# kshedden/muscato

Hardware: AMD Instinct MI355X
Metric: reads/sec (100 bp, multi-map) at 1/2/4/8 MI355X; confirm-kernel HBM GB/s vs peak (higher is better)
Workload: dtype u32

## Files before the change

### include/muscato_hip.h

```cpp
#ifndef MUSCATO_HIP_H
#define MUSCATO_HIP_H

#include <stdint.h>

#ifdef __cplusplus
extern "C" {
#endif

#define MUSC_ABI_VERSION 3
#define MUSC_MAX_WINDOWS 16

typedef struct musc_ctx musc_ctx;

typedef struct {
  uint32_t read_idx;
  uint32_t gene_idx;
  uint32_t pos;
  uint32_t nmiss;
} musc_hit;

typedef struct {
  int32_t n_windows;
  int32_t windows[MUSC_MAX_WINDOWS];
  int32_t window_width;
  double pmatch;
  int32_t min_dinuc;
  int32_t max_read_length;
  int32_t max_matches;
  int32_t match_mode;
  int32_t mmtol;
  int32_t apply_mmtol;
  int32_t max_mismatch_p1;
  int32_t skip_block_check;
  int32_t n_shards;
  int32_t reserved[2];
} musc_params;

typedef struct {
  uint64_t n_reads;
  uint64_t n_read_windows;
  uint64_t n_candidates;
  uint64_t n_pairs;
  uint64_t n_accepted;
  uint64_t n_hits;
  uint64_t n_overflow_blocks;
  uint64_t confirm_bytes;
  uint32_t confirm_launches;
  uint32_t n_batches;
  float ms_screen;
  float ms_scan;
  uint32_t match_variant;
  float ms_confirm;
  float ms_select;
  float ms_total;
  float ms_index_build;
  float ms_read_prep;
  uint64_t n_descriptors;
  uint32_t index_kind;
  uint32_t match_launches;
  uint64_t n_overflow_entries;
  uint64_t match_bytes;
  uint64_t match_bytes_strict;
  uint64_t index_bytes;
} musc_stats;

int musc_abi_version(void);

int musc_init(int device_ordinal, musc_ctx** out);
void musc_destroy(musc_ctx* ctx);
const char* musc_last_error(musc_ctx* ctx);
int musc_reload_env(musc_ctx* ctx);

int musc_db_load_ascii(musc_ctx* ctx, const char* seqs, const uint64_t* offsets, uint32_t nseq,
                       int on_device);
int musc_db_load_packed(musc_ctx* ctx, const uint8_t* bases2bit, const uint8_t* nmask,
                        const uint64_t* seq_offsets, uint32_t nseq);
int musc_db_build_index(musc_ctx* ctx, int32_t window_width);
int musc_db_build_index_for(musc_ctx* ctx, const musc_params* params, int32_t max_read_len);

int musc_db_set_partition_bases(musc_ctx* ctx, uint64_t max_bases);
int musc_db_partitions(musc_ctx* ctx, uint32_t* first_target, uint32_t cap, uint32_t* n);

int musc_reads_load_ascii(musc_ctx* ctx, const char* seqs, const uint64_t* offsets,
                          uint64_t nreads, int on_device);
int musc_reads_load_packed(musc_ctx* ctx, const uint8_t* bases2bit, const uint8_t* nmask,
                           const uint64_t* read_offsets, uint64_t nreads);
int musc_reads_load_packed32(musc_ctx* ctx, const uint8_t* bases2bit, const uint8_t* nmask,
                             const uint32_t* lengths, uint32_t fixed_len, uint64_t nreads, int async);

int musc_reads_sort_unique(musc_ctx* ctx, const char* seqs, const uint64_t* offsets, uint64_t nreads,
                           int on_device, uint32_t** order, uint32_t** ustart, uint64_t* nunique);

int musc_match_device(musc_ctx* ctx, const musc_params* params, uint64_t* nhits);
int musc_hits_copy(musc_ctx* ctx, musc_hit* dst, uint64_t capacity, int dst_on_device);
int musc_hits_copy_packed(musc_ctx* ctx, uint64_t* dst, uint64_t capacity, int dst_on_device,
                          uint64_t read_base, const int32_t* bits);
int musc_hits_unpack(musc_ctx* ctx, const uint64_t* src, uint64_t n, int on_device, const int32_t* bits,
                     musc_hit* dst);
int musc_hits_copy_compact(musc_ctx* ctx, uint32_t* words, uint64_t words_capacity, uint8_t* counts,
                           uint64_t counts_capacity, int dst_on_device, const int32_t* bits);
int musc_match(musc_ctx* ctx, const musc_params* params, musc_hit** hits, uint64_t* nhits);
void musc_free_hits(musc_hit* hits);

int musc_get_stats(musc_ctx* ctx, musc_stats* out);

#define MUSC_INSTANCE_WORDS 4
#define MUSC_INST_MATCH_T 1u
#define MUSC_INST_MATCH_G 2u
#define MUSC_INST_SCREEN 3u
#define MUSC_INST_SCREEN_T 4u
#define MUSC_INST_CONFIRM 5u
int musc_last_instance(const musc_ctx* ctx, uint32_t* out);
int musc_instances(uint32_t* out, uint32_t capacity, uint32_t* n);

int musc_overflow_probes(musc_ctx* ctx, uint32_t** read_idx, uint32_t** window, uint64_t* n);
void musc_free_u32(uint32_t* p);

int musc_gather(musc_ctx* const* ctxs, int n, const uint64_t* read_base, musc_hit** hits,
                uint64_t* nhits);
int musc_gather_rccl(musc_ctx* const* ctxs, int n, const uint64_t* read_base, musc_hit** hits,
                     uint64_t* nhits);
int musc_rccl_probe(char* msg, uint64_t cap);

#ifdef __cplusplus
}
#endif
#endif
```

### muscato_amd/_lib.py

```python
from __future__ import annotations

import ctypes
import os

HERE = os.path.dirname(os.path.abspath(__file__))
LIB_PATH = os.environ.get("MUSC_LIB_PATH") or os.path.join(HERE, "libmuscato_hip.so")

MUSC_MAX_WINDOWS = 16


class MuscHit(ctypes.Structure):
    _fields_ = [("read_idx", ctypes.c_uint32), ("gene_idx", ctypes.c_uint32),
                ("pos", ctypes.c_uint32), ("nmiss", ctypes.c_uint32)]


class MuscParams(ctypes.Structure):
    _fields_ = [
        ("n_windows", ctypes.c_int32),
        ("windows", ctypes.c_int32 * MUSC_MAX_WINDOWS),
        ("window_width", ctypes.c_int32),
        ("pmatch", ctypes.c_double),
        ("min_dinuc", ctypes.c_int32),
        ("max_read_length", ctypes.c_int32),
        ("max_matches", ctypes.c_int32),
        ("match_mode", ctypes.c_int32),
        ("mmtol", ctypes.c_int32),
        ("apply_mmtol", ctypes.c_int32),
        ("max_mismatch_p1", ctypes.c_int32),
        ("skip_block_check", ctypes.c_int32),
        ("n_shards", ctypes.c_int32),
        ("reserved", ctypes.c_int32 * 2),
    ]


class MuscStats(ctypes.Structure):
    _fields_ = [
        ("n_reads", ctypes.c_uint64), ("n_read_windows", ctypes.c_uint64),
        ("n_candidates", ctypes.c_uint64), ("n_pairs", ctypes.c_uint64), ("n_accepted", ctypes.c_uint64),
        ("n_hits", ctypes.c_uint64), ("n_overflow_blocks", ctypes.c_uint64),
        ("confirm_bytes", ctypes.c_uint64),
        ("confirm_launches", ctypes.c_uint32), ("n_batches", ctypes.c_uint32),
        ("ms_screen", ctypes.c_float), ("ms_scan", ctypes.c_float), ("match_variant", ctypes.c_uint32),
        ("ms_confirm", ctypes.c_float), ("ms_select", ctypes.c_float), ("ms_total", ctypes.c_float),
        ("ms_index_build", ctypes.c_float), ("ms_read_prep", ctypes.c_float),
        ("n_descriptors", ctypes.c_uint64),
        ("index_kind", ctypes.c_uint32), ("match_launches", ctypes.c_uint32),
        ("n_overflow_entries", ctypes.c_uint64), ("match_bytes", ctypes.c_uint64),
        ("match_bytes_strict", ctypes.c_uint64), ("index_bytes", ctypes.c_uint64),
    ]


SYMBOLS = [
    "musc_abi_version", "musc_init", "musc_destroy", "musc_last_error", "musc_reload_env",
    "musc_db_load_ascii", "musc_db_load_packed", "musc_db_build_index", "musc_db_build_index_for",
    "musc_db_set_partition_bases", "musc_db_partitions",
    "musc_reads_load_ascii", "musc_reads_load_packed", "musc_reads_load_packed32", "musc_reads_sort_unique",
    "musc_match_device", "musc_hits_copy", "musc_hits_copy_packed", "musc_hits_copy_compact", "musc_hits_unpack", "musc_match", "musc_free_hits",
    "musc_get_stats", "musc_last_instance", "musc_instances", "musc_gather", "musc_gather_rccl", "musc_rccl_probe", "musc_overflow_probes", "musc_free_u32",
]

_lib = None


def load() -> ctypes.CDLL:
    global _lib
    if _lib is not None:
        return _lib
    if not os.path.exists(LIB_PATH):
        raise ImportError(
            "muscato_amd: %s is missing -- build it with `python -m muscato_amd.build` "
            "(hipcc, gfx950).  There is no CPU fallback." % LIB_PATH)
    import sys
    torch = sys.modules.get("torch")
    if torch is not None:
        try:
            if torch.cuda.is_available():
                torch.cuda.init()
        except Exception:
            pass
    lib = ctypes.CDLL(LIB_PATH)
    for s in SYMBOLS:
        if not hasattr(lib, s):
            raise ImportError("muscato_amd: %s does not export %s" % (LIB_PATH, s))
    vp, u64, i32 = ctypes.c_void_p, ctypes.c_uint64, ctypes.c_int32
    lib.musc_abi_version.restype = ctypes.c_int
    lib.musc_init.argtypes = [ctypes.c_int, ctypes.POINTER(vp)]
    lib.musc_destroy.argtypes = [vp]
    lib.musc_destroy.restype = None
    lib.musc_last_error.argtypes = [vp]
    lib.musc_last_error.restype = ctypes.c_char_p
    lib.musc_reload_env.argtypes = [vp]
    lib.musc_db_load_ascii.argtypes = [vp, vp, vp, ctypes.c_uint32, ctypes.c_int]
    lib.musc_db_load_packed.argtypes = [vp, vp, vp, vp, ctypes.c_uint32]
    lib.musc_db_build_index.argtypes = [vp, i32]
    lib.musc_db_build_index_for.argtypes = [vp, ctypes.POINTER(MuscParams), i32]
    lib.musc_db_set_partition_bases.argtypes = [vp, u64]
    lib.musc_db_partitions.argtypes = [vp, vp, ctypes.c_uint32, ctypes.POINTER(ctypes.c_uint32)]
    lib.musc_reads_load_ascii.argtypes = [vp, vp, vp, u64, ctypes.c_int]
    lib.musc_reads_load_packed.argtypes = [vp, vp, vp, vp, u64]
    lib.musc_reads_load_packed32.argtypes = [vp, vp, vp, vp, ctypes.c_uint32, u64, ctypes.c_int]
    lib.musc_reads_sort_unique.argtypes = [vp, vp, vp, u64, ctypes.c_int, ctypes.POINTER(vp), ctypes.POINTER(vp),
                                           ctypes.POINTER(u64)]
    lib.musc_match_device.argtypes = [vp, ctypes.POINTER(MuscParams), ctypes.POINTER(u64)]
    lib.musc_hits_copy.argtypes = [vp, vp, u64, ctypes.c_int]
    lib.musc_hits_copy_packed.argtypes = [vp, vp, u64, ctypes.c_int, u64, ctypes.POINTER(i32)]
    lib.musc_hits_copy_compact.argtypes = [vp, vp, u64, vp, u64, ctypes.c_int, ctypes.POINTER(i32)]
    lib.musc_hits_unpack.argtypes = [vp, vp, u64, ctypes.c_int, ctypes.POINTER(i32), vp]
    lib.musc_match.argtypes = [vp, ctypes.POINTER(MuscParams), ctypes.POINTER(vp), ctypes.POINTER(u64)]
    lib.musc_free_hits.argtypes = [vp]
    lib.musc_free_hits.restype = None
    lib.musc_get_stats.argtypes = [vp, ctypes.POINTER(MuscStats)]
    lib.musc_last_instance.argtypes = [vp, ctypes.POINTER(ctypes.c_uint32)]
    lib.musc_instances.argtypes = [ctypes.POINTER(ctypes.c_uint32), ctypes.c_uint32, ctypes.POINTER(ctypes.c_uint32)]
    lib.musc_overflow_probes.argtypes = [vp, ctypes.POINTER(vp), ctypes.POINTER(vp), ctypes.POINTER(u64)]
    lib.musc_overflow_probes.restype = ctypes.c_int
    lib.musc_free_u32.argtypes = [vp]
    lib.musc_free_u32.restype = None
    lib.musc_gather.argtypes = [ctypes.POINTER(vp), ctypes.c_int, ctypes.POINTER(u64),
                                ctypes.POINTER(vp), ctypes.POINTER(u64)]
    lib.musc_gather_rccl.argtypes = lib.musc_gather.argtypes
    lib.musc_rccl_probe.argtypes = [ctypes.c_char_p, ctypes.c_uint64]
    for name in ("musc_init", "musc_reload_env", "musc_db_load_ascii", "musc_db_load_packed", "musc_db_build_index", "musc_db_build_index_for", "musc_db_build_index_for",
                 "musc_db_set_partition_bases", "musc_db_partitions",
                 "musc_reads_load_ascii", "musc_reads_load_packed", "musc_reads_load_packed32", "musc_reads_sort_unique", "musc_match_device",
                 "musc_hits_copy", "musc_hits_copy_packed", "musc_hits_copy_compact", "musc_hits_unpack", "musc_match", "musc_get_stats", "musc_last_instance", "musc_instances",
                 "musc_gather", "musc_gather_rccl", "musc_rccl_probe"):
        getattr(lib, name).restype = ctypes.c_int
    _lib = lib
    return lib
```

### muscato_amd/api.py

```python
from __future__ import annotations

import ctypes
import json
from dataclasses import dataclass, field, asdict
from typing import List, Optional, Sequence, Tuple

import numpy as np

from . import _lib


class MuscatoError(RuntimeError):
    pass


@dataclass
class Config:
    ReadFileName: str = ""
    GeneFileName: str = ""
    GeneIdFileName: str = ""
    ResultsFileName: str = ""
    Windows: List[int] = field(default_factory=list)
    WindowWidth: int = 0
    BloomSize: int = 0
    NumHash: int = 0
    PMatch: float = 0.0
    MinDinuc: int = 0
    TempDir: str = ""
    LogDir: str = ""
    MinReadLength: int = 0
    MaxReadLength: int = 0
    MaxMatches: int = 0
    MaxConfirmProcs: int = 0
    MMTol: int = 0
    MatchMode: str = ""
    SortPar: int = 0
    SortTemp: str = ""
    SortMem: str = ""
    NoCleanTemp: bool = False
    CPUProfile: bool = False
    MaxMismatch: int = -1
    DbPartitionBases: int = 0

    @classmethod
    def from_json(cls, text) -> "Config":
        d = json.loads(text) if isinstance(text, (str, bytes)) else dict(text)
        c = cls()
        for k, v in d.items():
            if hasattr(c, k) and v is not None:
                setattr(c, k, v)
        return c

    def to_json(self) -> str:
        return json.dumps(asdict(self))

    def with_defaults(self) -> "Config":
        c = Config(**asdict(self))
        if not c.Windows:
            raise MuscatoError("Windows not provided")
        if c.WindowWidth == 0:
            raise MuscatoError("WindowWidth not provided")
        if c.MaxReadLength == 0:
            raise MuscatoError("MaxReadLength not provided")
        if c.BloomSize == 0:
            c.BloomSize = 4 * 1000 * 1000 * 1000
        if c.NumHash == 0:
            c.NumHash = 20
        if c.PMatch == 0:
            c.PMatch = 1.0
        if c.MaxMatches == 0:
            c.MaxMatches = 1000 * 1000
        if c.MaxConfirmProcs == 0:
            c.MaxConfirmProcs = 3
        if c.MatchMode == "":
            c.MatchMode = "best"
        if c.MatchMode not in ("best", "first"):
            raise MuscatoError("MatchMode must be 'first' or 'best'")
        if c.ResultsFileName == "":
            c.ResultsFileName = "results.txt"
        if c.DbPartitionBases < 0:
            raise MuscatoError("DbPartitionBases must be >= 0")
        return c

    def to_params(self, apply_mmtol: bool, skip_block_check: bool = False, n_shards: int = 1) -> _lib.MuscParams:
        c = self.with_defaults()
        if len(c.Windows) > _lib.MUSC_MAX_WINDOWS:
            raise MuscatoError("at most %d windows are supported" % _lib.MUSC_MAX_WINDOWS)
        p = _lib.MuscParams()
        p.n_windows = len(c.Windows)
        for i, w in enumerate(c.Windows):
            p.windows[i] = int(w)
        p.window_width = int(c.WindowWidth)
        p.pmatch = float(c.PMatch)
        p.min_dinuc = int(c.MinDinuc)
        p.max_read_length = int(c.MaxReadLength)
        p.max_matches = int(c.MaxMatches)
        p.match_mode = 1 if c.MatchMode == "first" else 0
        p.mmtol = int(c.MMTol)
        p.apply_mmtol = 1 if apply_mmtol else 0
        p.max_mismatch_p1 = c.MaxMismatch + 1 if c.MaxMismatch >= 0 else 0
        p.skip_block_check = 1 if skip_block_check else 0
        p.n_shards = max(1, int(n_shards))
        return p


def concat(seqs: Sequence[bytes]) -> Tuple[np.ndarray, np.ndarray]:
    off = np.zeros(len(seqs) + 1, dtype=np.uint64)
    if len(seqs):
        off[1:] = np.cumsum([len(s) for s in seqs], dtype=np.uint64)
    buf = np.frombuffer(b"".join(seqs) + b"\0" * 8, dtype=np.uint8).copy()
    return buf, off


_CODE = np.full(256, 255, dtype=np.uint8)
for _i, _c in enumerate(b"ACGT"):
    _CODE[_c] = _i


def pack_2bit(buf: np.ndarray, nbases: int) -> Tuple[np.ndarray, Optional[np.ndarray]]:
    codes = _CODE[buf[:nbases]]
    isx = codes == 255
    codes = np.where(isx, 0, codes).astype(np.uint8)
    pad = (-nbases) % 4
    c4 = np.concatenate([codes, np.zeros(pad, np.uint8)]).reshape(-1, 4)
    packed = (c4[:, 0] | (c4[:, 1] << 2) | (c4[:, 2] << 4) | (c4[:, 3] << 6)).astype(np.uint8)
    mask = np.packbits(isx, bitorder="little") if isx.any() else None
    return packed, mask


class Engine:

    def __init__(self, device: int = 0):
        self._lib = _lib.load()
        h = ctypes.c_void_p()
        rc = self._lib.musc_init(int(device), ctypes.byref(h))
        if rc != 0:
            raise MuscatoError("musc_init failed: %s" % self._lib.musc_last_error(None).decode())
        self._h = h
        self.device = device
        self.n_targets = 0
        self.n_reads = 0

    def close(self) -> None:
        if getattr(self, "_h", None):
            self._lib.musc_destroy(self._h)
            self._h = None

    def __del__(self):
        try:
            self.close()
        except Exception:
            pass

    def __enter__(self):
        return self

    def __exit__(self, *a):
        self.close()

    def _check(self, rc: int, what: str) -> None:
        if rc != 0:
            raise MuscatoError("%s failed (%d): %s" % (what, rc, self._lib.musc_last_error(self._h).decode()))

    def reload_env(self) -> None:
        self._check(self._lib.musc_reload_env(self._h), "musc_reload_env")

    def load_targets(self, seqs: Sequence[bytes]) -> None:
        buf, off = concat(seqs)
        self.load_targets_arrays(buf, off)

    def load_targets_arrays(self, buf: np.ndarray, off: np.ndarray) -> None:
        self._check(self._lib.musc_db_load_ascii(self._h, buf.ctypes.data, off.ctypes.data, len(off) - 1, 0),
                    "musc_db_load_ascii")
        self.n_targets = len(off) - 1

    def load_targets_device(self, seqs_ptr: int, off_ptr: int, nseq: int) -> None:
        self._check(self._lib.musc_db_load_ascii(self._h, seqs_ptr, off_ptr, nseq, 1), "musc_db_load_ascii")
        self.n_targets = nseq

    def load_targets_packed(self, seqs: Sequence[bytes]) -> None:
        buf, off = concat(seqs)
        packed, mask = pack_2bit(buf, int(off[-1]))
        packed = np.concatenate([packed, np.zeros(8, np.uint8)])
        mp = mask.ctypes.data if mask is not None else None
        self._check(self._lib.musc_db_load_packed(self._h, packed.ctypes.data, mp, off.ctypes.data, len(off) - 1),
                    "musc_db_load_packed")
        self.n_targets = len(off) - 1

    def build_index(self, window_width: int) -> None:
        self._check(self._lib.musc_db_build_index(self._h, int(window_width)), "musc_db_build_index")

    def build_index_for(self, cfg: "Config", max_read_len: int = 0) -> None:
        p = cfg.to_params(True)
        self._apply_partition_bases(cfg)
        self._check(self._lib.musc_db_build_index_for(self._h, ctypes.byref(p), int(max_read_len)),
                    "musc_db_build_index_for")

    def set_partition_bases(self, max_bases: int) -> None:
        if max_bases < 0:
            raise MuscatoError("partition bases must be >= 0")
        self._check(self._lib.musc_db_set_partition_bases(self._h, int(max_bases)), "musc_db_set_partition_bases")

    def partitions(self) -> List[int]:
        n = ctypes.c_uint32()
        self._check(self._lib.musc_db_partitions(self._h, None, 0, ctypes.byref(n)), "musc_db_partitions")
        if not n.value:
            return []
        out = (ctypes.c_uint32 * (n.value + 1))()
        self._check(self._lib.musc_db_partitions(self._h, out, n.value + 1, ctypes.byref(n)), "musc_db_partitions")
        return list(out)

    def _apply_partition_bases(self, cfg: "Config") -> None:
        if cfg.DbPartitionBases:
            self.set_partition_bases(int(cfg.DbPartitionBases))

    def load_reads(self, seqs: Sequence[bytes]) -> None:
        buf, off = concat(seqs)
        self.load_reads_arrays(buf, off)

    def load_reads_arrays(self, buf: np.ndarray, off: np.ndarray) -> None:
        self._check(self._lib.musc_reads_load_ascii(self._h, buf.ctypes.data, off.ctypes.data, len(off) - 1, 0),
                    "musc_reads_load_ascii")
        self.n_reads = len(off) - 1

    def load_reads_device(self, seqs_ptr: int, off_ptr: int, nreads: int) -> None:
        self._check(self._lib.musc_reads_load_ascii(self._h, seqs_ptr, off_ptr, nreads, 1), "musc_reads_load_ascii")
        self.n_reads = nreads

    def sort_unique_reads(self, seqs: Sequence[bytes]):
        buf, off = concat(seqs)
        return self.sort_unique_reads_arrays(buf.ctypes.data, off.ctypes.data, len(off) - 1, False)

    def sort_unique_reads_arrays(self, seqs_ptr: int, off_ptr: int, nreads: int, on_device: bool):
        po, pu, nu = ctypes.c_void_p(), ctypes.c_void_p(), ctypes.c_uint64()
        self._check(self._lib.musc_reads_sort_unique(self._h, seqs_ptr, off_ptr, nreads, 1 if on_device else 0,
                                                     ctypes.byref(po), ctypes.byref(pu), ctypes.byref(nu)),
                    "musc_reads_sort_unique")
        try:
            order = np.ctypeslib.as_array(ctypes.cast(po, ctypes.POINTER(ctypes.c_uint32)), shape=(max(nreads, 1),))[:nreads].copy()
            ustart = np.ctypeslib.as_array(ctypes.cast(pu, ctypes.POINTER(ctypes.c_uint32)), shape=(nu.value + 1,)).copy()
        finally:
            self._lib.musc_free_u32(po)
            self._lib.musc_free_u32(pu)
        self.n_reads = int(nu.value)
        return order, ustart

    def load_reads_packed(self, seqs: Sequence[bytes]) -> None:
        buf, off = concat(seqs)
        packed, mask = pack_2bit(buf, int(off[-1]))
        packed = np.concatenate([packed, np.zeros(8, np.uint8)])
        mp = mask.ctypes.data if mask is not None else None
        self._check(self._lib.musc_reads_load_packed(self._h, packed.ctypes.data, mp, off.ctypes.data, len(off) - 1),
                    "musc_reads_load_packed")
        self.n_reads = len(off) - 1

    def load_reads_packed_ptr(self, bases_ptr: int, mask_ptr: int, off_ptr: int, nreads: int) -> None:
        self._check(self._lib.musc_reads_load_packed(self._h, bases_ptr, mask_ptr or None, off_ptr, nreads),
                    "musc_reads_load_packed")
        self.n_reads = nreads

    def load_reads_packed32_ptr(self, bases_ptr: int, mask_ptr: int, lengths_ptr: int, fixed_len: int, nreads: int,
                                async_upload: bool = False) -> None:
        self._check(self._lib.musc_reads_load_packed32(self._h, bases_ptr, mask_ptr or None, lengths_ptr or None,
                                                       fixed_len, nreads, 1 if async_upload else 0),
                    "musc_reads_load_packed32")
        self.n_reads = nreads

    def match_device(self, cfg: Config, apply_mmtol: bool = True, skip_block_check: bool = False,
                     n_shards: int = 1) -> int:
        p = cfg.to_params(apply_mmtol, skip_block_check, n_shards)
        self._apply_partition_bases(cfg)
        n = ctypes.c_uint64()
        self._check(self._lib.musc_match_device(self._h, ctypes.byref(p), ctypes.byref(n)), "musc_match_device")
        return int(n.value)

    def hits_to(self, ptr: int, capacity: int, on_device: bool) -> None:
        self._check(self._lib.musc_hits_copy(self._h, ptr, capacity, 1 if on_device else 0), "musc_hits_copy")

    def hits_to_packed(self, ptr: int, capacity: int, on_device: bool, bits: Sequence[int], read_base: int = 0) -> None:
        b = (ctypes.c_int32 * 4)(*bits)
        self._check(self._lib.musc_hits_copy_packed(self._h, ptr, capacity, 1 if on_device else 0, read_base, b),
                    "musc_hits_copy_packed")

    def hits_to_compact(self, words_ptr: int, words_cap: int, counts_ptr: int, counts_cap: int, on_device: bool,
                        bits: Sequence[int]) -> None:
        b = (ctypes.c_int32 * 3)(*bits)
        self._check(self._lib.musc_hits_copy_compact(self._h, words_ptr, words_cap, counts_ptr, counts_cap,
                                                     1 if on_device else 0, b), "musc_hits_copy_compact")

    def unpack_hits(self, src_ptr: int, n: int, on_device: bool, bits: Sequence[int], dst_ptr: int) -> None:
        b = (ctypes.c_int32 * 4)(*bits)
        self._check(self._lib.musc_hits_unpack(self._h, src_ptr, n, 1 if on_device else 0, b, dst_ptr), "musc_hits_unpack")

    def match(self, cfg: Config, apply_mmtol: bool = True, n_shards: int = 1) -> np.ndarray:
        n = self.match_device(cfg, apply_mmtol, n_shards=n_shards)
        out = np.zeros((n, 4), dtype=np.uint32)
        if n:
            self.hits_to(out.ctypes.data, n, False)
        return out

    def overflow_probes(self) -> np.ndarray:
        pr, pw, n = ctypes.c_void_p(), ctypes.c_void_p(), ctypes.c_uint64()
        self._check(self._lib.musc_overflow_probes(self._h, ctypes.byref(pr), ctypes.byref(pw), ctypes.byref(n)),
                    "musc_overflow_probes")
        out = np.zeros((n.value, 2), dtype=np.uint32)
        if n.value:
            out[:, 0] = np.ctypeslib.as_array(ctypes.cast(pr, ctypes.POINTER(ctypes.c_uint32)), shape=(n.value,))
            out[:, 1] = np.ctypeslib.as_array(ctypes.cast(pw, ctypes.POINTER(ctypes.c_uint32)), shape=(n.value,))
        self._lib.musc_free_u32(pr)
        self._lib.musc_free_u32(pw)
        return out

    def last_instance(self) -> dict:
        w = (ctypes.c_uint32 * 4)()
        self._check(self._lib.musc_last_instance(self._h, w), "musc_last_instance")
        return {"path": "fused" if w[0] else "two-kernel" if w[1] else "none",
                "match": decode_instance(w[0]), "screen": decode_instance(w[1]), "confirm": decode_instance(w[2]),
                "block_mode": w[3] & 0xFF, "exact_rerun": bool(w[3] & 0x100)}

    def stats(self) -> dict:
        s = _lib.MuscStats()
        self._check(self._lib.musc_get_stats(self._h, ctypes.byref(s)), "musc_get_stats")
        return {k: getattr(s, k) for k, _ in s._fields_}


_INST_FIELDS = {1: ("k_match_t", ("W", "XM", "WIDE", "SG")), 2: ("k_match_g", (None, None, None, "SG")),
                3: ("k_screen", ("mask", "one", "lines")), 4: ("k_screen_t", ()), 5: ("k_confirm", ("mask", "w2"))}


def decode_instance(word: int) -> Optional[dict]:
    if not word:
        return None
    name, fields = _INST_FIELDS[word & 0xFF]
    d = {"kernel": name, "RW": (word >> 8) & 0xFF}
    for i, f in enumerate(fields):
        if f:
            d[f] = (word >> (16 + 4 * i)) & 0xF
    return d


def instance_name(d: Optional[dict]) -> str:
    return "none" if d is None else "%s<%s>" % (d["kernel"], ", ".join(str(v) for k, v in d.items() if k != "kernel"))


def instances() -> List[dict]:
    lib = _lib.load()
    n = ctypes.c_uint32()
    if lib.musc_instances(None, 0, ctypes.byref(n)):
        raise RuntimeError("musc_instances failed")
    buf = (ctypes.c_uint32 * max(1, n.value))()
    lib.musc_instances(buf, n.value, ctypes.byref(n))
    return [decode_instance(w) for w in buf[:n.value]]


def gather(engines: Sequence["Engine"], read_bases: Sequence[int], rccl: bool = False) -> np.ndarray:
    lib = engines[0]._lib
    n = len(engines)
    arr = (ctypes.c_void_p * n)(*[e._h for e in engines])
    bases = (ctypes.c_uint64 * n)(*[int(b) for b in read_bases])
    ph, cnt = ctypes.c_void_p(), ctypes.c_uint64()
    rc = lib.musc_gather_rccl(arr, n, bases, ctypes.byref(ph), ctypes.byref(cnt)) if rccl else 1
    if rccl and rc == 2:
        raise MuscatoError("musc_gather_rccl failed (%d): %s" % (rc, lib.musc_last_error(engines[0]._h).decode()))
    if rc != 0:
        rc = lib.musc_gather(arr, n, bases, ctypes.byref(ph), ctypes.byref(cnt))
    if rc != 0:
        raise MuscatoError("musc_gather failed (%d): %s" % (rc, lib.musc_last_error(engines[0]._h).decode()))
    out = np.zeros((cnt.value, 4), dtype=np.uint32)
    if cnt.value:
        ctypes.memmove(out.ctypes.data, ph, cnt.value * 16)
    lib.musc_free_hits(ph)
    return out


def sorted_hits(a: np.ndarray) -> np.ndarray:
    if len(a) == 0:
        return a.reshape(0, 4)
    idx = np.lexsort((a[:, 3], a[:, 2], a[:, 1], a[:, 0]))
    return a[idx]
```

### muscato_amd/csrc/kernels_confirm.hpp

```cpp
#pragma once

template <int RW, bool MASK>
struct PairRegs {
  uint4 ds;
  uint32_t exact;
  uint32_t r[RW ? RW : 1], t[RW ? RW : 1], rm[(RW && MASK) ? RW : 1], tm[(RW && MASK) ? RW : 1];
};

template <int RW, bool MASK>
DEV void pair_issue(PairRegs<RW, MASK>& P, const uint4 ds, const uint32_t* __restrict__ rd,
                    const uint32_t* __restrict__ rdm, const uint32_t* __restrict__ db2,
                    const uint32_t* __restrict__ dbm2, const uint32_t* __restrict__ dbx, uint64_t r0,
                    const uint32_t* __restrict__ rvalid) {
  static_assert(RW != 0, "static stride only");
  P.ds = ds;
  const uint32_t ri = ds.x & 0xFFFFFFu;
  const uint64_t gpos = (uint64_t)ds.y | ((uint64_t)(ds.x >> 24) << 32);
  const uint32_t* __restrict__ rec = rd + (r0 + ri) * (uint64_t)RW;
  const uint64_t widx = gpos >> 4;
  P.exact = rvalid[ri];
  bool rx = false, tx = false;
  if constexpr (MASK) {
    rx = (ds.z & DESC_RX) != 0;
    tx = db_span_has_x(dbx, gpos, RW * 16);
  }
#pragma unroll
  for (int q = 0; q < RW / 4; q++) {
    const u32x4_v a = __builtin_nontemporal_load(reinterpret_cast<const u32x4_v*>(rec) + q);
    P.r[4 * q] = a.x; P.r[4 * q + 1] = a.y; P.r[4 * q + 2] = a.z; P.r[4 * q + 3] = a.w;
    const u32x4_u b = *reinterpret_cast<const u32x4_u*>(db2 + widx + 4 * q);
    P.t[4 * q] = b.x; P.t[4 * q + 1] = b.y; P.t[4 * q + 2] = b.z; P.t[4 * q + 3] = b.w;
    if constexpr (MASK) {
      uint4 c = make_uint4(0, 0, 0, 0);
      if (rx) c = *reinterpret_cast<const uint4*>(rdm + (r0 + ri) * (uint64_t)RW + 4 * q);
      P.rm[4 * q] = c.x; P.rm[4 * q + 1] = c.y; P.rm[4 * q + 2] = c.z; P.rm[4 * q + 3] = c.w;
      u32x4_u d = {0, 0, 0, 0};
      if (tx) d = *reinterpret_cast<const u32x4_u*>(dbm2 + widx + 4 * q);
      P.tm[4 * q] = d.x; P.tm[4 * q + 1] = d.y; P.tm[4 * q + 2] = d.z; P.tm[4 * q + 3] = d.w;
    }
  }
}

DEV uint32_t pair_code(const uint4 ds, uint32_t nx, uint32_t budget, uint32_t exact) {
  const uint32_t ri = ds.x & 0xFFFFFFu, k = ds.z & 15u;
  const bool within = nx <= budget;
  const bool a0 = within && ((exact >> k) & 1u);
  const bool a1 = within && (ds.z & DESC_TWO) && ((exact >> (k + 1)) & 1u);
  if (!(a0 || a1)) return NX_REJECT;
  const uint32_t kmin = (uint32_t)(__ffs(exact) - 1);
  const bool first = (a0 && kmin == k) || (a1 && kmin == k + 1);
  return (first ? nx : (nx | NX_DUP)) | (a0 ? NX_ACC0 : 0u) | (a1 ? NX_ACC1 : 0u) | (k << 20) | ((ri & (TILE - 1)) << 24);
}

template <int RW, bool MASK, bool W2, class BudgetOf>
DEV uint32_t pair_finish(const PairRegs<RW, MASK>& P, const PathParams& pp, BudgetOf budget_of) {
  const uint64_t gpos = (uint64_t)P.ds.y | ((uint64_t)(P.ds.x >> 24) << 32);
  const uint32_t sh = ((uint32_t)gpos & 15u) * 2u;
  uint32_t exact = P.exact;
  if ((P.ds.z >> 4) & 1u) exact &= ~pp.q1zero_mask;
  const uint32_t len = P.r[RW - 1] & 0xFFFFu;
  const int len2 = 2 * (int)len;
  uint32_t nx = 0;
#pragma unroll
  for (int j = 0; j < RW - 1; j++) {
    const uint32_t tj = __funnelshift_r(P.t[j], P.t[j + 1], sh);
    const uint32_t x = P.r[j] ^ tj;
    uint32_t d = (x | (x >> 1)) & 0x55555555u;
    if constexpr (MASK) d |= (P.rm[j] ^ __funnelshift_r(P.tm[j], P.tm[j + 1], sh)) & 0x55555555u;
    const int rem = len2 - 32 * j;
    d &= rem >= 32 ? 0xFFFFFFFFu : (rem <= 0 ? 0u : ((1u << rem) - 1u));
    nx += __popc(d);
    if constexpr (W2) {
#pragma unroll
      for (int kk = 0; kk < 2; kk++)
        if (kk < pp.W && (d & window_word_mask(pp.win[kk], pp.ww, j))) exact &= ~(1u << kk);
    } else {
      for (int kk = 0; kk < pp.W; kk++)
        if (d & window_word_mask(pp.win[kk], pp.ww, j)) exact &= ~(1u << kk);
    }
  }
  return pair_code(P.ds, nx, budget_of(len), exact);
}

template <int RW, bool MASK, bool W2, class BudgetOf>
DEV uint32_t confirm_pair(const uint4 ds, const uint32_t* __restrict__ rd, const uint32_t* __restrict__ rdm,
                          const uint32_t* __restrict__ db2, const uint32_t* __restrict__ dbm2,
                          const uint32_t* __restrict__ dbx, uint64_t r0, int rw_rt, const PathParams& pp,
                          BudgetOf budget_of, const uint32_t* __restrict__ rvalid) {
  if constexpr (RW != 0) {
    PairRegs<RW, MASK> P;
    pair_issue<RW, MASK>(P, ds, rd, rdm, db2, dbm2, dbx, r0, rvalid);
    return pair_finish<RW, MASK, W2>(P, pp, budget_of);
  } else {
    const uint32_t ri = ds.x & 0xFFFFFFu;
    const int rw = rw_rt;
    const uint64_t gpos = (uint64_t)ds.y | ((uint64_t)(ds.x >> 24) << 32);
    const uint32_t* __restrict__ rec = rd + (r0 + ri) * (uint64_t)rw;
    const uint64_t widx = gpos >> 4;
    const uint32_t sh = ((uint32_t)gpos & 15u) * 2u;
    uint32_t exact = rvalid[ri];
    if ((ds.z >> 4) & 1u) exact &= ~pp.q1zero_mask;
    uint32_t nx = 0;
    const uint32_t len = rec[rw - 1] & 0xFFFFu;
    const int len2 = 2 * (int)len;
    const uint32_t* __restrict__ recm = MASK ? rdm + (r0 + ri) * (uint64_t)rw : nullptr;
    uint32_t tlo = db2[widx], tmlo = MASK ? dbm2[widx] : 0u;
    for (int j = 0; j < rw - 1; j++) {
      const uint32_t thi = db2[widx + j + 1];
      const uint32_t x = rec[j] ^ __funnelshift_r(tlo, thi, sh);
      tlo = thi;
      uint32_t d = (x | (x >> 1)) & 0x55555555u;
      if (MASK) {
        const uint32_t tmhi = dbm2[widx + j + 1];
        d |= (recm[j] ^ __funnelshift_r(tmlo, tmhi, sh)) & 0x55555555u;
        tmlo = tmhi;
      }
      const int rem = len2 - 32 * j;
      d &= rem >= 32 ? 0xFFFFFFFFu : (rem <= 0 ? 0u : ((1u << rem) - 1u));
      nx += __popc(d);
      for (int kk = 0; kk < pp.W; kk++)
        if (d & window_word_mask(pp.win[kk], pp.ww, j)) exact &= ~(1u << kk);
    }
    return pair_code(ds, nx, budget_of(len), exact);
  }
}

#define BLOCK_LDS_BITS 11
#define CONF_TILES 32


#define CODE_CAP 1024

template <int RW, bool MASK, bool W2>
__global__ __launch_bounds__(TILE, (RW <= 8 && !(RW == 8 && MASK)) ? 8 : 4) void k_confirm(
    const uint32_t* __restrict__ rd, const uint32_t* __restrict__ rdm,
    const uint32_t* __restrict__ db2, const uint32_t* __restrict__ dbm2, const uint32_t* __restrict__ dbx,
    uint64_t r0, uint32_t n, int rw_rt,
    const PathParams* __restrict__ ppp, const uint16_t* __restrict__ nmiss_tab, const uint4* __restrict__ cdesc,
    const uint32_t* __restrict__ rvalid, uint32_t* __restrict__ p_nx,
    const uint32_t* __restrict__ tbase, const uint32_t* __restrict__ tcount,
    const uint32_t* __restrict__ wb, int block_mode, uint32_t block_thr, uint32_t* __restrict__ block_table,
    const uint64_t* __restrict__ seq_off, uint4* __restrict__ stage, uint32_t* __restrict__ tcount2,
    unsigned long long* __restrict__ counters) {
  const PathParams& pp = *ppp;
  extern __shared__ uint32_t s_wcnt[];
  __shared__ uint32_t s_best[TILE], s_cnt[TILE], s_base[TILE];
  __shared__ uint32_t s_code[CODE_CAP];
  __shared__ uint32_t s_sketch[1 << BLOCK_LDS_BITS];
  __shared__ uint32_t s_wsum[TILE / 64];
  __shared__ uint16_t s_nm[CONF_NM];
  __shared__ uint32_t s_tb[CONF_TILES], s_tn[CONF_TILES];
  const uint32_t ntiles = (n + TILE - 1) / TILE;
  const int lane = threadIdx.x & 63, wid = threadIdx.x >> 6;
  if (block_mode == 1)
    for (uint32_t t = threadIdx.x; t < (1u << BLOCK_LDS_BITS); t += TILE) s_sketch[t] = 0;
  for (uint32_t t = threadIdx.x; t < CONF_NM; t += TILE) s_nm[t] = t <= (uint32_t)pp.max_len ? nmiss_tab[t] : (uint16_t)0;
  const uint32_t my_tiles = blockIdx.x < ntiles ? (ntiles - 1 - blockIdx.x) / gridDim.x + 1 : 0;
  for (uint32_t j = threadIdx.x; j < my_tiles && j < CONF_TILES; j += TILE) {
    s_tb[j] = tbase[blockIdx.x + j * gridDim.x];
    s_tn[j] = tcount[blockIdx.x + j * gridDim.x];
  }
  if (blockIdx.x == 0 && threadIdx.x == 0) tcount2[ntiles] = 0;
  unsigned long long acc = 0;
  auto budget_of = [&](uint32_t len) -> uint32_t { return len < CONF_NM ? s_nm[len] : nmiss_tab[len]; };
  __syncthreads();

  for (uint32_t j = 0; j < my_tiles; j++) {
    const uint32_t tile = blockIdx.x + j * gridDim.x;
    lds_barrier();
    s_best[threadIdx.x] = 0xFFFFFFFFu;
    s_cnt[threadIdx.x] = 0;
    if (block_mode)
      for (uint32_t t = threadIdx.x; t < TILE * (uint32_t)pp.W; t += TILE) s_wcnt[t] = 0;
    lds_barrier();
    const uint32_t tn = s_tn[j];
    const uint64_t tb = s_tb[j];
    auto tally = [&](uint32_t w) {
      if (w == NX_REJECT) return;
      const uint32_t rl = w >> 24;
      if (block_mode) {
        const uint32_t k = (w >> 20) & 15u;
        if (w & NX_ACC0) atomicAdd(&s_wcnt[rl * pp.W + k], 1u);
        if (w & NX_ACC1) atomicAdd(&s_wcnt[rl * pp.W + k + 1], 1u);
      }
      if (w & NX_DUP) return;
      atomicMin(&s_best[rl], w & 0xFFFFu);
      acc++;
    };
    auto confirm_at = [&](uint32_t tj, uint32_t* gene, uint32_t* zword) -> uint32_t {
      const u32x4_v dsv = __builtin_nontemporal_load(reinterpret_cast<const u32x4_v*>(cdesc) + tb + tj);
      *gene = dsv.w;
      *zword = dsv.z;
      return confirm_pair<RW, MASK, W2>(make_uint4(dsv.x, dsv.y, dsv.z, dsv.w), rd, rdm, db2, dbm2, dbx, r0, rw_rt, pp,
                                    budget_of, rvalid);
    };
    uint32_t w0 = NX_REJECT, gene0 = 0, z0 = 0;
    if (threadIdx.x < tn) w0 = confirm_at(threadIdx.x, &gene0, &z0);
    tally(w0);
    for (uint32_t tj = threadIdx.x + TILE; tj < tn; tj += TILE) {
      uint32_t g, z;
      const uint32_t w = confirm_at(tj, &g, &z);
      if (tj - TILE < CODE_CAP) s_code[tj - TILE] = w; else p_nx[tb + tj] = w;
      tally(w);
    }
    lds_barrier();
    auto count = [&](uint32_t w) {
      if (w == NX_REJECT || (w & NX_DUP)) return;
      const uint32_t rl = w >> 24;
      const uint32_t thr = pp.apply_mmtol ? s_best[rl] + (uint32_t)pp.mmtol : 0xFFFFu;
      if ((w & 0xFFFFu) <= thr) atomicAdd(&s_cnt[rl], 1u);
    };
    count(w0);
    for (uint32_t tj = threadIdx.x + TILE; tj < tn; tj += TILE)
      count(tj - TILE < CODE_CAP ? s_code[tj - TILE] : p_nx[tb + tj]);
    if (block_mode) {
      for (uint32_t t = threadIdx.x; t < TILE * (uint32_t)pp.W; t += TILE) {
        const uint32_t cw = s_wcnt[t];
        if (!cw) continue;
        const uint32_t rl = t / pp.W, k = t % pp.W;
        const uint32_t h = block_hash32((uint32_t)k, wb[((uint64_t)tile * TILE + rl) * pp.W + k]);
        if (block_mode == 1) atomicAdd(&s_sketch[h >> (32 - BLOCK_LDS_BITS)], cw);
        else atomicAdd(&block_table[h >> (32 - BLOCK_TABLE_BITS)], cw);
      }
    }
    lds_barrier();
    const uint32_t c = s_cnt[threadIdx.x];
    uint32_t inc = c;
#pragma unroll
    for (int d = 1; d < 64; d <<= 1) {
      const uint32_t o = __shfl_up(inc, d);
      if (lane >= d) inc += o;
    }
    if (lane == 63) s_wsum[wid] = inc;
    lds_barrier();
    uint32_t woff = 0, total = 0;
#pragma unroll
    for (int q = 0; q < TILE / 64; q++) {
      if (q < wid) woff += s_wsum[q];
      total += s_wsum[q];
    }
    s_base[threadIdx.x] = woff + inc - c;
    s_cnt[threadIdx.x] = 0;
    if (threadIdx.x == 0) tcount2[tile] = total;
    lds_barrier();
    if (total == 0) continue;
    auto emit = [&](uint32_t w, uint32_t tj, uint32_t gene, uint32_t zword) {
      if (w == NX_REJECT || (w & NX_DUP)) return;
      const uint32_t rl = w >> 24, v = w & 0xFFFFu;
      const uint32_t thr = pp.apply_mmtol ? s_best[rl] + (uint32_t)pp.mmtol : 0xFFFFu;
      if (v > thr) return;
      const uint32_t ord = atomicAdd(&s_cnt[rl], 1u);
      uint32_t pos = (zword >> 6) & 0xFFFFu;
      if (!((zword >> 5) & 1u)) {
        const uint4 ds = cdesc[tb + tj];
        pos = (uint32_t)(((uint64_t)ds.y | ((uint64_t)(ds.x >> 24) << 32)) - seq_off[gene]);
      }
      stage[tb + s_base[rl] + ord] = make_uint4((uint32_t)(r0 + tile * TILE + rl), gene, pos, v);
    };
    emit(w0, threadIdx.x, gene0, z0);
    for (uint32_t tj = threadIdx.x + TILE; tj < tn; tj += TILE) {
      const uint32_t w = tj - TILE < CODE_CAP ? s_code[tj - TILE] : p_nx[tb + tj];
      if (w == NX_REJECT || (w & NX_DUP)) continue;
      const uint4 ds = cdesc[tb + tj];
      emit(w, tj, ds.w, ds.z);
    }
  }
  block_add_u64(acc, &counters[1]);
  if (block_mode == 1) {
    lds_barrier();
    uint32_t hot = 0;
    for (uint32_t t = threadIdx.x; t < (1u << BLOCK_LDS_BITS); t += TILE) hot |= s_sketch[t] >= block_thr;
    if (__any(hot) && (threadIdx.x & 63) == 0) atomicOr(&counters[6], 1ull);
  }
}

MUSC_KERNEL __launch_bounds__(256) void k_compact(uint32_t ntiles, const uint32_t* __restrict__ tbase,
                                                 const uint32_t* __restrict__ tcount2,
                                                 const uint32_t* __restrict__ tpre,
                                                 const uint4* __restrict__ stage, uint4* __restrict__ hits,
                                                 uint64_t hits_cap, unsigned long long* __restrict__ counters) {
  const unsigned long long base = counters[2];
  if (base + tpre[ntiles] > hits_cap) {
    if (blockIdx.x == 0 && threadIdx.x == 0) atomicOr(&counters[3], 2ull);
    return;
  }
  for (uint32_t tile = blockIdx.x; tile < ntiles; tile += gridDim.x) {
    const uint32_t m = tcount2[tile];
    const uint4* __restrict__ src = stage + tbase[tile];
    uint4* __restrict__ dst = hits + base + tpre[tile];
    for (uint32_t j = threadIdx.x; j < m; j += blockDim.x) dst[j] = src[j];
  }
}

template <int RW>
__global__ __launch_bounds__(256) void k_hot_probes(const uint32_t* __restrict__ rd,
                                                    const uint32_t* __restrict__ rdm, uint64_t nreads,
                                                    int rw_rt, const PathParams* __restrict__ ppp,
                                                    const uint32_t* __restrict__ block_table,
                                                    uint32_t max_matches, uint2* __restrict__ out,
                                                    uint64_t cap, unsigned long long* __restrict__ cursor) {
  const PathParams& pp = *ppp;
  const int rw = RW ? RW : rw_rt;
  const bool has_m = rdm != nullptr;
  for (uint64_t i = (uint64_t)blockIdx.x * blockDim.x + threadIdx.x; i < nreads; i += (uint64_t)gridDim.x * blockDim.x) {
    Rec<RW> rec;
    rec.load(rd + i * (uint64_t)rw, rw);
    Rec<RW> recm = rec;
    if (has_m) recm.load(rdm + i * (uint64_t)rw, rw);
    const uint32_t len = rec.len();
    for (int k = 0; k < pp.W; k++) {
      const uint32_t q1 = (uint32_t)pp.win[k], q2 = q1 + (uint32_t)pp.ww;
      if (len < q2) continue;
      if (pp.min_dinuc > 0 && rec_count_dinuc(rec, recm, has_m, q1, pp.ww) < pp.min_dinuc) continue;
      const uint32_t b = rec_bucket(rec, recm, has_m, q1, pp.ww, pp.bits, pp.direct);
      const uint32_t h = block_hash32((uint32_t)k, b);
      if (block_table[h >> (32 - BLOCK_TABLE_BITS)] > max_matches) {
        const unsigned long long slot = atomicAdd(cursor, 1ull);
        if (slot < cap) out[slot] = make_uint2((uint32_t)i, (uint32_t)k);
      }
    }
  }
}

MUSC_KERNEL void k_advance(const uint32_t* __restrict__ tpre, uint32_t ntiles, unsigned long long* counters) {
  if (threadIdx.x == 0 && blockIdx.x == 0) counters[2] += tpre[ntiles];
}

MUSC_KERNEL void k_block_overflow(const uint32_t* __restrict__ block_table, uint32_t max_matches,
                                 unsigned long long* __restrict__ counters) {
  unsigned long long c = 0;
  for (uint32_t i = blockIdx.x * blockDim.x + threadIdx.x; i < (1u << BLOCK_TABLE_BITS); i += gridDim.x * blockDim.x)
    c += block_table[i] > max_matches;
  block_add_u64(c, &counters[5]);
}

struct PackBits {
  int32_t read, gene, pos, nmiss;
};

MUSC_KERNEL __launch_bounds__(256) void k_pack_hits(const uint4* __restrict__ hits, uint64_t n, uint64_t read_base,
                                                   PackBits b, uint64_t* __restrict__ out, uint32_t* __restrict__ bad) {
  for (uint64_t i = (uint64_t)blockIdx.x * blockDim.x + threadIdx.x; i < n; i += (uint64_t)gridDim.x * blockDim.x) {
    const uint4 h = hits[i];
    const uint64_t r = (uint64_t)h.x + read_base;
    if ((b.read < 64 && (r >> b.read)) || ((uint64_t)h.y >> b.gene) || ((uint64_t)h.z >> b.pos) || ((uint64_t)h.w >> b.nmiss))
      atomicOr(bad, 1u);
    out[i] = (((((r << b.gene) | h.y) << b.pos) | h.z) << b.nmiss) | h.w;
  }
}

MUSC_KERNEL __launch_bounds__(256) void k_unpack_hits(const uint64_t* __restrict__ in, uint64_t n, PackBits b,
                                                     uint4* __restrict__ hits) {
  for (uint64_t i = (uint64_t)blockIdx.x * blockDim.x + threadIdx.x; i < n; i += (uint64_t)gridDim.x * blockDim.x) {
    uint64_t v = in[i];
    const uint32_t nm = (uint32_t)(v & ((1ull << b.nmiss) - 1ull));
    v >>= b.nmiss;
    const uint32_t pos = (uint32_t)(v & ((1ull << b.pos) - 1ull));
    v >>= b.pos;
    const uint32_t gene = (uint32_t)(v & ((1ull << b.gene) - 1ull));
    v >>= b.gene;
    hits[i] = make_uint4((uint32_t)v, gene, pos, nm);
  }
}

MUSC_KERNEL __launch_bounds__(256) void k_pack_compact(const uint4* __restrict__ hits, uint64_t n, PackBits b,
                                                      uint32_t* __restrict__ words, uint8_t* __restrict__ counts,
                                                      uint32_t* __restrict__ bad) {
  for (uint64_t i = (uint64_t)blockIdx.x * blockDim.x + threadIdx.x; i < n; i += (uint64_t)gridDim.x * blockDim.x) {
    const uint4 h = hits[i];
    if (((uint64_t)h.y >> b.gene) || ((uint64_t)h.z >> b.pos) || ((uint64_t)h.w >> b.nmiss)) atomicOr(bad, 1u);
    words[i] = (((h.y << b.pos) | h.z) << b.nmiss) | h.w;
    const uint32_t prev = i ? hits[i - 1].x : 0xFFFFFFFFu;
    if (i && prev > h.x) atomicOr(bad, 4u);
    if (i == 0 || prev != h.x) {
      uint32_t cnt = 1;
      while (i + cnt < n && cnt < 256 && hits[i + cnt].x == h.x) cnt++;
      if (cnt > 255) atomicOr(bad, 2u);
      counts[h.x] = (uint8_t)cnt;
    }
  }
}
```

### muscato_amd/csrc/muscato_hip.hip

```cpp

#include <hip/hip_runtime.h>
#include <rccl/rccl.h>
#include <dlfcn.h>

#include <algorithm>
#include <cstdarg>
#include <cstdio>
#include <cstdlib>
#include <cstring>
#include <map>
#include <mutex>
#include <string>
#include <type_traits>
#include <vector>

#include "../../include/muscato_hip.h"

#include "kernels_common.hpp"
#include "kernels_index.hpp"
#include "kernels_screen.hpp"
#include "kernels_confirm.hpp"
#include "kernels_match.hpp"
#include "kernels_match_lane_inst.hpp"
#include "kernels_screen_lane.hpp"
#include "kernels_partition.hpp"
MUSC_LANE_INSTANCES_4(extern)
MUSC_LANE_INSTANCES_8(extern)
MUSC_LANE_INSTANCES_12(extern)
MUSC_LANE_INSTANCES_8W(extern)
MUSC_LANE_INSTANCES_12W(extern)
MUSC_LANE_INSTANCES_16W(extern)
MUSC_LANE_INSTANCES_SPEC(extern)
MUSC_DMA_INSTANCES(extern)


namespace {

thread_local std::string g_init_error;

template <class T>
struct DevBuf {
  T* p = nullptr;
  uint64_t cap = 0;
  void release() {
    if (p) (void)hipFree(p);
    p = nullptr;
    cap = 0;
  }
};

struct Roctx {
  int (*push)(const char*) = nullptr;
  int (*pop)() = nullptr;
  Roctx() {
    for (const char* name : {"librocprofiler-sdk-roctx.so.1", "librocprofiler-sdk-roctx.so", "libroctx64.so.4", "libroctx64.so"}) {
      if (void* h = dlopen(name, RTLD_NOW | RTLD_LOCAL)) {
        push = reinterpret_cast<int (*)(const char*)>(dlsym(h, "roctxRangePushA"));
        pop = reinterpret_cast<int (*)()>(dlsym(h, "roctxRangePop"));
        if (push && pop) return;
        push = nullptr;
        pop = nullptr;
      }
    }
  }
};
const Roctx& roctx() {
  static const Roctx r;
  return r;
}
struct Range {
  bool on;
  explicit Range(const char* name) : on(roctx().push != nullptr) {
    if (on) (void)roctx().push(name);
  }
  ~Range() {
    if (on) (void)roctx().pop();
  }
};

struct CaptureGuard {
  hipStream_t st = nullptr;
  bool active = false;
  hipError_t begin(hipStream_t s) {
    const hipError_t e = hipStreamBeginCapture(s, hipStreamCaptureModeThreadLocal);
    if (e == hipSuccess) {
      st = s;
      active = true;
    }
    return e;
  }
  hipError_t end(hipGraph_t* g) {
    active = false;
    return hipStreamEndCapture(st, g);
  }
  ~CaptureGuard() {
    if (!active) return;
    hipGraph_t g = nullptr;
    (void)hipStreamEndCapture(st, &g);
    if (g) (void)hipGraphDestroy(g);
    (void)hipGetLastError();
  }
};

struct TmpBufs {
  void* p[16] = {};
  int n = 0;
  template <class T>
  hipError_t alloc(T** out, size_t bytes) {
    void* q = nullptr;
    *out = nullptr;
    if (n >= 16) return hipErrorOutOfMemory;
    const hipError_t e = hipMalloc(&q, bytes ? bytes : 16);
    if (e == hipSuccess) p[n++] = q;
    *out = (T*)q;
    return e;
  }
  void release() {
    for (int i = 0; i < n; i++) (void)hipFree(p[i]);
    n = 0;
  }
  ~TmpBufs() { release(); }
};

}

struct EnvKnobs {
  enum { IDX_AUTO = 0, IDX_CLASSIC, IDX_LINES, IDX_CLASSIC64 };
  int index = IDX_AUTO;
  bool match_dma = false;
  bool screen_wg = false;
  int context = 0;
  bool no_x_context = false;
  bool force_wide = false;
  int index_bits = 0;
  bool ctx_direct = false;
  int debug_grid = 0;
  bool debug_sync = false;
  int graph = -1;
  bool pipeline = false;
  bool no_spec = false;
  long batch_reads = 0;
  long index_budget_mb = 0;
  void read() {
    *this = EnvKnobs();
    auto is = [](const char* v, const char* w) { return v && !strcmp(v, w); };
    const char* e = getenv("MUSC_INDEX");
    index = is(e, "classic") ? IDX_CLASSIC : is(e, "lines") ? IDX_LINES : is(e, "classic64") ? IDX_CLASSIC64 : IDX_AUTO;
    e = getenv("MUSC_MATCH");
    match_dma = is(e, "dma");
    screen_wg = is(getenv("MUSC_SCREEN"), "wg");
    e = getenv("MUSC_CONTEXT");
    context = is(e, "narrow") ? 1 : is(e, "wide") ? 2 : 0;
    no_x_context = getenv("MUSC_NO_X_CONTEXT") != nullptr;
    force_wide = getenv("MUSC_DEBUG_FORCE_WIDE") != nullptr;
    if ((e = getenv("MUSC_DEBUG_INDEX_BITS"))) index_bits = atoi(e);
    ctx_direct = (e = getenv("MUSC_DEBUG_CTX_DIRECT")) && atoi(e) > 0;
    if ((e = getenv("MUSC_DEBUG_GRID"))) debug_grid = atoi(e);
    debug_sync = getenv("MUSC_DEBUG_SYNC") != nullptr;
    if ((e = getenv("MUSC_GRAPH"))) graph = atoi(e);
    if ((e = getenv("MUSC_PIPELINE"))) pipeline = atoi(e) > 0;
    no_spec = getenv("MUSC_NO_SPEC") != nullptr;
    if ((e = getenv("MUSC_BATCH_READS"))) batch_reads = atol(e);
    if ((e = getenv("MUSC_DEBUG_INDEX_BUDGET_MB"))) index_budget_mb = atol(e);
  }
};

struct musc_ctx {
  int device = 0;
  hipStream_t stream = nullptr;
  std::string err;
  EnvKnobs env;

  uint32_t* db2 = nullptr;
  uint32_t* dbm2 = nullptr;
  bool db_has_x = false;
  bool reads_have_x = false;
  DevBuf<uint32_t> rdx;
  uint64_t rdx_epoch = ~0ull;
  int rdx_wide = -1;
  uint64_t xok_epoch = ~0ull;
  double xok_pmatch = -1.0;
  int32_t xok_mmp1 = -1;
  bool xok = false;
  uint32_t* dbx = nullptr;
  uint64_t max_tlen = 0;
  uint64_t xokdb_epoch = ~0ull;
  int32_t xokdb_key[CTX_MAX_W + 3] = {0};
  bool xokdb = false;
  uint64_t* seq_off = nullptr;
  uint32_t nseq = 0;
  uint64_t nbases = 0;
  uint64_t db_words = 0;
  std::vector<uint64_t> h_seq_off;

  uint64_t part_bases = 0;
  std::vector<uint32_t> part_first;
  int part_kind = 0;
  uint64_t part_size = 0;
  uint32_t cur_part = 0;
  DevBuf<musc_hit> pacc;
  DevBuf<uint32_t> pbest;
  DevBuf<uint64_t> pcnt, padj;
  DevBuf<uint32_t> pflags, pflags_tmp;
  DevBuf<uint32_t> block_acc;

  int idx_ww = 0, idx_bits = 0, idx_direct = 0;
  uint32_t idx_g0 = 0, idx_g1 = 0;
  int wide = 0;
  Bucket* idx_T = nullptr;
  uint4* idx_E = nullptr;
  bool idx_lines = false;
  unsigned scrt_resident = 0;
  int scrt_rw = 0;
  uint64_t idx_T_bytes = 0, idx_E_cap = 0;
  uint64_t idx_n = 0;
  uint64_t idx_novf = 0;
  int idx_kind = 0;
  int idx_wide = 0;
  int idx_CL = 0;
  CtxBucket* ctx_T = nullptr;
  CtxEntry* ctx_E = nullptr;
  uint64_t ctx_T_cap = 0, ctx_E_cap = 0;
  PathParams* d_pp = nullptr;
  PathParams h_pp;
  bool h_pp_valid = false;
  MatchParams* d_mp = nullptr;
  MatchParams h_mp;
  bool h_mp_valid = false;
  int spec_geom = 0;
  DevBuf<uint4> spill;

  uint32_t* rd = nullptr;
  uint32_t* rdm = nullptr;
  uint64_t nreads = 0;
  int rw = 0;
  uint32_t max_len = 0;

  struct Upload {
    uint32_t* stage = nullptr;
    uint64_t stage_words = 0;
    hipStream_t s_up = nullptr;
    std::vector<hipEvent_t> ev;
    uint64_t piece = 0, n_pieces = 0;
    uint64_t packed_upto = 0;
    uint32_t L = 0;
    bool active = false;
  } up;

  struct BatchSet {
    DevBuf<uint32_t> wb, rvalid, tbase, tcount;
    DevBuf<uint4> cdesc;
  } bs[2];
  int cur = 0;
  hipStream_t stream2 = nullptr;
  hipStream_t s_confirm = nullptr;
  hipEvent_t ev_ready[2] = {nullptr, nullptr}, ev_free[2] = {nullptr, nullptr}, ev_join = nullptr;
  DevBuf<uint32_t> scan_tmp, tcount2, tpre;
  DevBuf<uint4> stage;
  DevBuf<uint32_t> p_nx;
  DevBuf<uint16_t> nmiss_tab;
  DevBuf<uint32_t> block_table;
  bool force_exact_blocks = false;
  uint64_t exact_epoch = 0;
  musc_params exact_params;
  int cur_block_mode = 0;
  uint32_t cur_block_thr = 0;
  PathParams last_pp;
  uint32_t last_max_matches = 0;
  uint32_t last_inst[MUSC_INSTANCE_WORDS] = {0, 0, 0, 0};
  bool last_exact_blocks = false;
  unsigned long long* counters = nullptr;
  uint64_t* h_pinned = nullptr;

  DevBuf<musc_hit> hits;
  uint64_t nhits = 0;
  DevBuf<uint64_t> packed;
  DevBuf<musc_hit> gathered;
  uint32_t* d_flag = nullptr;

  uint32_t batch_reads = 16u << 20;
  uint64_t data_epoch = 1;
  uint64_t sized_epoch = 0;
  musc_params sized_params;
  bool sized_exact_blocks = false;
  uint32_t sized_bsz = 0;
  musc_stats stats;
  hipGraphExec_t graph_exec = nullptr;
  bool graph_failed = false;
  uint64_t graph_epoch = 0;
  musc_params graph_params;
  int graph_block_mode = -1;
  uint32_t graph_batches = 0;
  std::vector<hipEvent_t> ev_pool;
  size_t ev_used = 0;
  double nm_pmatch = -1.0;
  int32_t nm_mmp1 = -1;
  uint32_t nm_maxlen = 0xFFFFFFFFu;
};

namespace {

int fail(musc_ctx* c, int code, const char* fmt, ...) {
  char buf[512];
  va_list ap;
  va_start(ap, fmt);
  vsnprintf(buf, sizeof buf, fmt, ap);
  va_end(ap);
  if (c) c->err = buf; else g_init_error = buf;
  return code;
}

#define HIPCHK(c, expr)                                                                 \
  do {                                                                                  \
    hipError_t e_ = (expr);                                                             \
    if (e_ != hipSuccess) {                                                             \
      (void)hipGetLastError();                                                          \
      return fail((c), 10, "%s failed: %s (%s:%d)", #expr, hipGetErrorString(e_), __FILE__, __LINE__); \
    }                                                                                   \
  } while (0)

template <class T>
int ensure(musc_ctx* c, DevBuf<T>& b, uint64_t n, bool keep = false) {
  if (n <= b.cap && b.p) return 0;
  uint64_t ncap = std::max<uint64_t>(n, b.cap + b.cap / 2);
  ncap = std::max<uint64_t>(ncap, 1024);
  T* np = nullptr;
  HIPCHK(c, hipMalloc((void**)&np, ncap * sizeof(T) + 64));
  if (keep && b.p && b.cap) {
    hipError_t e = hipMemcpyAsync(np, b.p, b.cap * sizeof(T), hipMemcpyDeviceToDevice, c->stream);
    if (e == hipSuccess) e = hipStreamSynchronize(c->stream);
    if (e != hipSuccess) {
      (void)hipFree(np);
      return fail(c, 10, "hit buffer grow failed: %s", hipGetErrorString(e));
    }
  }
  b.release();
  b.p = np;
  b.cap = ncap;
  return 0;
}

inline unsigned nblk(uint64_t n, unsigned b) { return (unsigned)((n + b - 1) / b); }

uint64_t scan_tmp_elems(uint64_t n) {
  uint64_t t = 0;
  while (n > SCAN_TILE) {
    n = (n + SCAN_TILE - 1) / SCAN_TILE;
    t += (n + 8 + 3) & ~3ull;
  }
  return t + 8;
}

int scan_u32(musc_ctx* c, const uint32_t* in, uint32_t* out, uint64_t n, bool inclusive, uint32_t* tmp,
             hipStream_t st = nullptr) {
  if (!st) st = c->stream;
  const uint64_t nb = (n + SCAN_TILE - 1) / SCAN_TILE;
  if (nb > 0x7FFFFFFFull) return fail(c, 11, "scan too large");
  if (nb <= 1) {
    if (inclusive) hipLaunchKernelGGL(k_scan_block<true>, dim3(1), dim3(SCAN_BLOCK), 0, st, in, out, (uint32_t*)nullptr, n);
    else hipLaunchKernelGGL(k_scan_block<false>, dim3(1), dim3(SCAN_BLOCK), 0, st, in, out, (uint32_t*)nullptr, n);
    HIPCHK(c, hipGetLastError());
    return 0;
  }
  uint32_t* sums = tmp;
  if (inclusive) hipLaunchKernelGGL(k_scan_block<true>, dim3((unsigned)nb), dim3(SCAN_BLOCK), 0, st, in, out, sums, n);
  else hipLaunchKernelGGL(k_scan_block<false>, dim3((unsigned)nb), dim3(SCAN_BLOCK), 0, st, in, out, sums, n);
  HIPCHK(c, hipGetLastError());
  int rc = scan_u32(c, sums, sums, nb, false, tmp + ((nb + 8 + 3) & ~3ull), st);
  if (rc) return rc;
  hipLaunchKernelGGL(k_scan_add, dim3((unsigned)nb), dim3(SCAN_BLOCK), 0, st, out, sums, n);
  HIPCHK(c, hipGetLastError());
  return 0;
}

int scan_u64(musc_ctx* c, const uint64_t* in, uint64_t* out, uint64_t n, uint64_t* tmp) {
  const uint64_t nb = (n + SCAN_TILE - 1) / SCAN_TILE;
  if (nb > 0x7FFFFFFFull) return fail(c, 11, "scan too large");
  if (nb <= 1) {
    hipLaunchKernelGGL(k_scan64_block, dim3(1), dim3(SCAN_BLOCK), 0, c->stream, in, out, (uint64_t*)nullptr, n);
    HIPCHK(c, hipGetLastError());
    return 0;
  }
  hipLaunchKernelGGL(k_scan64_block, dim3((unsigned)nb), dim3(SCAN_BLOCK), 0, c->stream, in, out, tmp, n);
  HIPCHK(c, hipGetLastError());
  int rc = scan_u64(c, tmp, tmp, nb, tmp + ((nb + 8 + 3) & ~3ull));
  if (rc) return rc;
  hipLaunchKernelGGL(k_scan64_add, dim3((unsigned)nb), dim3(SCAN_BLOCK), 0, c->stream, out, tmp, n);
  HIPCHK(c, hipGetLastError());
  return 0;
}

void free_index(musc_ctx* c) {
  c->idx_ww = 0;
  c->idx_n = 0;
  c->data_epoch++;
}

void drop_ctx_index(musc_ctx* c) {
  if (c->ctx_T) (void)hipFree(c->ctx_T);
  if (c->ctx_E) (void)hipFree(c->ctx_E);
  c->ctx_T = nullptr;
  c->ctx_E = nullptr;
  c->ctx_T_cap = c->ctx_E_cap = 0;
}

void free_db(musc_ctx* c) {
  free_index(c);
  if (c->db2) (void)hipFree(c->db2);
  if (c->dbm2) (void)hipFree(c->dbm2);
  if (c->dbx) (void)hipFree(c->dbx);
  if (c->seq_off) (void)hipFree(c->seq_off);
  c->db2 = c->dbm2 = c->dbx = nullptr;
  c->db_has_x = false;
  c->seq_off = nullptr;
  c->nseq = 0;
  c->nbases = 0;
  c->h_seq_off.clear();
  c->part_first.clear();
  c->data_epoch++;
}

void free_reads(musc_ctx* c) {
  if (c->up.active) {
    (void)hipStreamSynchronize(c->up.s_up);
    c->up.active = false;
  }
  if (c->rd) (void)hipFree(c->rd);
  if (c->rdm) (void)hipFree(c->rdm);
  c->rd = c->rdm = nullptr;
  c->reads_have_x = false;
  c->nreads = 0;
  c->rw = 0;
  c->data_epoch++;
}

struct EvPair {
  hipEvent_t a, b;
};

hipEvent_t pool_event(musc_ctx* c) {
  if (c->ev_used == c->ev_pool.size()) {
    hipEvent_t e = nullptr;
    if (hipEventCreate(&e) != hipSuccess) return nullptr;
    c->ev_pool.push_back(e);
  }
  return c->ev_pool[c->ev_used++];
}

struct Timer {
  musc_ctx* c;
  bool off = false;
  std::vector<EvPair> ev[5];
  explicit Timer(musc_ctx* ctx) : c(ctx) { c->ev_used = 0; }
  int begin(int fam, hipStream_t s = nullptr) {
    if (off) return 0;
    EvPair p;
    p.a = pool_event(c);
    p.b = pool_event(c);
    if (!p.a || !p.b) return 1;
    (void)hipEventRecord(p.a, s ? s : c->stream);
    ev[fam].push_back(p);
    return 0;
  }
  void end(int fam, hipStream_t s = nullptr) {
    if (!off && !ev[fam].empty()) (void)hipEventRecord(ev[fam].back().b, s ? s : c->stream);
  }
  float total(int fam) {
    float t = 0;
    for (auto& p : ev[fam]) {
      float ms = 0;
      if (hipEventElapsedTime(&ms, p.a, p.b) == hipSuccess) t += ms;
    }
    return t;
  }
};

int check_params(musc_ctx* c, const musc_params* P) {
  if (!P) return fail(c, 2, "params is NULL");
  if (P->n_windows < 1 || P->n_windows > MUSC_MAX_WINDOWS)
    return fail(c, 2, "n_windows=%d outside 1..%d", P->n_windows, MUSC_MAX_WINDOWS);
  if (P->window_width < 1 || P->window_width > 4096) return fail(c, 2, "bad window_width=%d", P->window_width);
  for (int k = 0; k < P->n_windows; k++)
    if (P->windows[k] < 0 || P->windows[k] > 60000) return fail(c, 2, "bad window start %d", P->windows[k]);
  if (!(P->pmatch >= 0.0 && P->pmatch <= 1.0)) return fail(c, 2, "PMatch=%g outside [0,1]", P->pmatch);
  if (P->match_mode != 0 && P->match_mode != 1) return fail(c, 2, "match_mode must be 0 (best) or 1 (first)");
  if (P->mmtol < 0) return fail(c, 2, "MMTol < 0");
  if (P->max_mismatch_p1 < 0) return fail(c, 2, "max_mismatch_p1 < 0");
  return 0;
}

bool screen_lane(const musc_ctx* c, bool mask) {
  return c->idx_lines && !mask && !c->rdm && (c->rw == 4 || c->rw == 8 || c->rw == 12 || c->rw == 16) && !c->env.screen_wg;
}

template <class F>
auto by_rw(int rw, F&& f) {
  switch (rw) {
    case 4: return f(std::integral_constant<int, 4>{});
    case 8: return f(std::integral_constant<int, 8>{});
    case 12: return f(std::integral_constant<int, 12>{});
    case 16: return f(std::integral_constant<int, 16>{});
    default: return f(std::integral_constant<int, 0>{});
  }
}

typedef decltype(&k_screen_t<8>) screen_t_fn;
typedef decltype(&k_screen<0, false, false, false>) screen_fn;
typedef decltype(&k_confirm<0, false, false>) confirm_fn;
template <class Fn>
struct Inst {
  Fn fn;
  uint32_t id;
};
constexpr uint32_t inst_id(uint32_t family, int rw, int a = 0, int b = 0, int c = 0, int d = 0) {
  return family | (uint32_t)rw << 8 | (uint32_t)a << 16 | (uint32_t)b << 20 | (uint32_t)c << 24 | (uint32_t)d << 28;
}
#define INST_SCREEN_T(RW) Inst<screen_t_fn>{k_screen_t<RW>, inst_id(MUSC_INST_SCREEN_T, RW)}
#define INST_SCREEN(RW, M, ONE, LN) Inst<screen_fn>{k_screen<RW, M, ONE, LN>, inst_id(MUSC_INST_SCREEN, RW, M, ONE, LN)}
#define INST_CONFIRM(RW, M, W2) Inst<confirm_fn>{k_confirm<RW, M, W2>, inst_id(MUSC_INST_CONFIRM, RW, M, W2)}

Inst<screen_t_fn> screen_t_instance(int rw) {
  return by_rw(rw, [](auto r) -> Inst<screen_t_fn> {
    if constexpr (decltype(r)::value != 0) return INST_SCREEN_T(decltype(r)::value);
    else return Inst<screen_t_fn>{nullptr, 0};
  });
}

Inst<screen_fn> screen_instance(int rw, bool mask, int W, bool lines) {
  const int m = mask, one = W <= 2, ln = lines;
  return by_rw(rw, [&](auto r) -> Inst<screen_fn> {
    constexpr int RW = decltype(r)::value;
    static const Inst<screen_fn> k[2][2][2] = {
        {{INST_SCREEN(RW, false, false, false), INST_SCREEN(RW, false, false, true)}, {INST_SCREEN(RW, false, true, false), INST_SCREEN(RW, false, true, true)}},
        {{INST_SCREEN(RW, true, false, false), INST_SCREEN(RW, true, false, true)}, {INST_SCREEN(RW, true, true, false), INST_SCREEN(RW, true, true, true)}}};
    return k[m][one][ln];
  });
}

Inst<confirm_fn> confirm_instance(int rw, bool mask, int W) {
  const int m = mask, w2 = W <= 2;
  return by_rw(rw, [&](auto r) -> Inst<confirm_fn> {
    constexpr int RW = decltype(r)::value;
    static const Inst<confirm_fn> k[2][2] = {{INST_CONFIRM(RW, false, false), INST_CONFIRM(RW, false, true)}, {INST_CONFIRM(RW, true, false), INST_CONFIRM(RW, true, true)}};
    return k[m][w2];
  });
}

Inst<screen_t_fn> screen_t_kernel(const musc_ctx* c) { return screen_t_instance(c->rw); }
Inst<screen_fn> screen_kernel(const musc_ctx* c, int W) { return screen_instance(c->rw, c->rdm != nullptr, W, c->idx_lines); }
Inst<confirm_fn> confirm_kernel(const musc_ctx* c, bool mask, int W) { return confirm_instance(c->rw, mask, W); }

unsigned screen_grid(musc_ctx* c, uint32_t n, bool mask) {
  unsigned g = std::min(nblk(n, TILE), MAX_GRID);
  if (screen_lane(c, mask)) {
    if (!c->scrt_resident) {
      int per_cu = 0, ncu = 0;
      const void* fn = reinterpret_cast<const void*>(screen_t_kernel(c).fn);
      if (hipOccupancyMaxActiveBlocksPerMultiprocessor(&per_cu, fn, 64, 0) != hipSuccess || per_cu < 1) { (void)hipGetLastError(); per_cu = 8; }
      if (hipDeviceGetAttribute(&ncu, hipDeviceAttributeMultiprocessorCount, c->device) != hipSuccess || ncu < 1) ncu = 256;
      c->scrt_resident = (unsigned)per_cu * (unsigned)ncu;
      c->scrt_rw = c->rw;
    }
    if (c->scrt_rw != c->rw) { c->scrt_resident = 0; return screen_grid(c, n, mask); }
    g = std::min(g, std::min(c->scrt_resident, MAX_GRID));
  }
  return g;
}

void launch_screen(musc_ctx* c, bool mask, uint64_t r0, uint32_t n, const PathParams& pp) {
  const dim3 sgrid(screen_grid(c, n, mask));
  auto& b = c->bs[c->cur];
  if (screen_lane(c, mask)) {
    const auto k = screen_t_kernel(c);
    c->last_inst[1] = k.id;
    hipLaunchKernelGGL(k.fn, sgrid, dim3(64), 0, c->stream, c->rd, r0, n, c->d_pp, c->nmiss_tab.p,
                       reinterpret_cast<const LineBucket*>(c->idx_T), c->idx_E, b.cdesc.p, b.cdesc.cap, b.rvalid.p, b.wb.p,
                       b.tbase.p, b.tcount.p, c->counters + 8, c->counters + 3);
  } else {
    const auto k = screen_kernel(c, pp.W);
    c->last_inst[1] = k.id;
    hipLaunchKernelGGL(k.fn, sgrid, dim3(TILE), 0, c->stream, c->rd, c->rdm, r0, n, c->rw, c->d_pp,
                       c->nmiss_tab.p, c->idx_T, c->idx_E, b.cdesc.p, b.cdesc.cap, b.rvalid.p, b.wb.p, b.tbase.p, b.tcount.p,
                       c->counters + 8, c->counters + 3);
  }
}

void launch_confirm(musc_ctx* c, bool mask, uint64_t r0, uint32_t n, const PathParams& pp) {
  const dim3 grid(std::min(nblk(n, TILE), MAX_GRID));
  static_assert((1u << 24) / TILE / MAX_GRID <= CONF_TILES, "a k_confirm workgroup keeps its tile list in LDS");
  const size_t lds = c->cur_block_mode ? (size_t)TILE * pp.W * 4 : 0;
  auto& b = c->bs[c->cur];
  const auto k = confirm_kernel(c, mask, pp.W);
  c->last_inst[2] = k.id;
  hipLaunchKernelGGL(k.fn, grid, dim3(TILE), lds, c->s_confirm, c->rd, c->rdm, c->db2, c->dbm2,
                     c->dbx, r0, n, c->rw, c->d_pp, c->nmiss_tab.p, b.cdesc.p, b.rvalid.p, c->p_nx.p, b.tbase.p, b.tcount.p,
                     b.wb.p, c->cur_block_mode, c->cur_block_thr, c->block_table.p, c->seq_off, c->stage.p, c->tcount2.p,
                     c->counters);
}

}

extern "C" {

int musc_abi_version(void) { return MUSC_ABI_VERSION; }

const char* musc_last_error(musc_ctx* ctx) { return ctx ? ctx->err.c_str() : g_init_error.c_str(); }

int musc_init(int device_ordinal, musc_ctx** out) {
  if (!out) return fail(nullptr, 2, "musc_init: out is NULL");
  *out = nullptr;
  int ndev = 0;
  hipError_t e = hipGetDeviceCount(&ndev);
  if (e != hipSuccess || ndev == 0)
    return fail(nullptr, 3, "musc_init: no HIP device (%s); this library has no CPU fallback",
                e == hipSuccess ? "device count 0" : hipGetErrorString(e));
  if (device_ordinal < 0 || device_ordinal >= ndev)
    return fail(nullptr, 2, "musc_init: device %d outside 0..%d", device_ordinal, ndev - 1);
  hipDeviceProp_t prop;
  if ((e = hipGetDeviceProperties(&prop, device_ordinal)) != hipSuccess)
    return fail(nullptr, 3, "musc_init: hipGetDeviceProperties: %s", hipGetErrorString(e));
  if (strncmp(prop.gcnArchName, "gfx950", 6) != 0)
    return fail(nullptr, 3, "musc_init: device %d is %s; this library is built for gfx950 only",
                device_ordinal, prop.gcnArchName);
  if ((e = hipSetDevice(device_ordinal)) != hipSuccess)
    return fail(nullptr, 3, "musc_init: hipSetDevice: %s", hipGetErrorString(e));
  musc_ctx* c = new musc_ctx();
  c->device = device_ordinal;
  memset(&c->stats, 0, sizeof c->stats);
  if ((e = hipStreamCreateWithFlags(&c->stream, hipStreamNonBlocking)) != hipSuccess ||
      (e = hipStreamCreateWithFlags(&c->stream2, hipStreamNonBlocking)) != hipSuccess ||
      (e = hipEventCreateWithFlags(&c->ev_ready[0], hipEventDisableTiming)) != hipSuccess ||
      (e = hipEventCreateWithFlags(&c->ev_ready[1], hipEventDisableTiming)) != hipSuccess ||
      (e = hipEventCreateWithFlags(&c->ev_free[0], hipEventDisableTiming)) != hipSuccess ||
      (e = hipEventCreateWithFlags(&c->ev_free[1], hipEventDisableTiming)) != hipSuccess ||
      (e = hipEventCreateWithFlags(&c->ev_join, hipEventDisableTiming)) != hipSuccess ||
      (e = hipMalloc((void**)&c->counters, 16 * sizeof(unsigned long long))) != hipSuccess ||
      (e = hipMalloc((void**)&c->d_flag, 4)) != hipSuccess ||
      (e = hipMalloc((void**)&c->d_mp, sizeof(MatchParams))) != hipSuccess ||
      (e = hipMalloc((void**)&c->d_pp, sizeof(PathParams))) != hipSuccess ||
      (e = hipHostMalloc((void**)&c->h_pinned, 16 * sizeof(uint64_t))) != hipSuccess) {
    fail(nullptr, 3, "musc_init: %s", hipGetErrorString(e));
    musc_destroy(c);
    return 3;
  }
  c->env.read();
  if (c->env.batch_reads >= 1 && c->env.batch_reads <= (16l << 20)) c->batch_reads = (uint32_t)c->env.batch_reads;
  *out = c;
  return 0;
}

int musc_reload_env(musc_ctx* c) {
  if (!c) return 1;
  c->env.read();
  c->sized_epoch = 0;
  return 0;
}

void musc_destroy(musc_ctx* c) {
  if (!c) return;
  (void)hipSetDevice(c->device);
  if (c->stream) (void)hipStreamSynchronize(c->stream);
  if (c->stream2) (void)hipStreamSynchronize(c->stream2);
  free_db(c);
  free_reads(c);
  if (c->idx_T) (void)hipFree(c->idx_T);
  if (c->idx_E) (void)hipFree(c->idx_E);
  if (c->ctx_T) (void)hipFree(c->ctx_T);
  if (c->ctx_E) (void)hipFree(c->ctx_E);
  if (c->d_mp) (void)hipFree(c->d_mp);
  if (c->d_pp) (void)hipFree(c->d_pp);
  c->spill.release();
  for (int i = 0; i < 2; i++) {
    c->bs[i].wb.release(); c->bs[i].tbase.release(); c->bs[i].rvalid.release(); c->bs[i].tcount.release();
    c->bs[i].cdesc.release();
  }
  c->scan_tmp.release(); c->tcount2.release(); c->tpre.release(); c->stage.release(); c->rdx.release();
  c->p_nx.release();
  c->nmiss_tab.release();
  c->block_table.release();
  c->pacc.release(); c->pbest.release(); c->pcnt.release(); c->padj.release(); c->pflags.release(); c->pflags_tmp.release();
  c->block_acc.release();
  c->hits.release();
  c->packed.release();
  c->gathered.release();
  if (c->d_flag) (void)hipFree(c->d_flag);
  if (c->counters) (void)hipFree(c->counters);
  if (c->h_pinned) (void)hipHostFree(c->h_pinned);
  for (hipEvent_t ev : {c->ev_ready[0], c->ev_ready[1], c->ev_free[0], c->ev_free[1], c->ev_join})
    if (ev) (void)hipEventDestroy(ev);
  for (hipEvent_t ev : c->ev_pool) (void)hipEventDestroy(ev);
  if (c->graph_exec) (void)hipGraphExecDestroy(c->graph_exec);
  for (hipEvent_t ev : c->up.ev) (void)hipEventDestroy(ev);
  if (c->up.stage) (void)hipFree(c->up.stage);
  if (c->up.s_up) (void)hipStreamDestroy(c->up.s_up);
  if (c->stream2) (void)hipStreamDestroy(c->stream2);
  if (c->stream) (void)hipStreamDestroy(c->stream);
  delete c;
}


static int db_xblocks(musc_ctx* c) {
  const uint64_t nblk64 = (c->db_words + 64 + 3) / 4;
  const uint64_t nw = nblk64 / 32 + 4;
  if (c->dbx) (void)hipFree(c->dbx);
  c->dbx = nullptr;
  HIPCHK(c, hipMalloc((void**)&c->dbx, nw * 4));
  HIPCHK(c, hipMemsetAsync(c->dbx, 0, nw * 4, c->stream));
  hipLaunchKernelGGL(k_db_xblocks, dim3(nblk(nblk64, 256)), dim3(256), 0, c->stream, c->dbm2, c->db_words, c->dbx);
  HIPCHK(c, hipGetLastError());
  HIPCHK(c, hipStreamSynchronize(c->stream));
  return 0;
}

static int db_finish(musc_ctx* c) {
  uint32_t hasx = 0;
  HIPCHK(c, hipMemcpyAsync(&hasx, c->d_flag, 4, hipMemcpyDeviceToHost, c->stream));
  unsigned long long tl = 0;
  HIPCHK(c, hipMemsetAsync(c->counters + 4, 0, 8, c->stream));
  hipLaunchKernelGGL(k_max_len, dim3(std::min(nblk(c->nseq, 256), MAX_GRID)), dim3(256), 0, c->stream, c->seq_off, (uint64_t)c->nseq, c->counters + 4);
  HIPCHK(c, hipGetLastError());
  HIPCHK(c, hipMemcpyAsync(&tl, c->counters + 4, 8, hipMemcpyDeviceToHost, c->stream));
  HIPCHK(c, hipStreamSynchronize(c->stream));
  c->max_tlen = tl;
  c->db_has_x = hasx != 0;
  if (!hasx) {
    (void)hipFree(c->dbm2);
    c->dbm2 = nullptr;
    return 0;
  }
  return db_xblocks(c);
}

static int db_alloc(musc_ctx* c, const uint64_t* offsets, uint32_t nseq, int on_device) {
  HIPCHK(c, hipSetDevice(c->device));
  free_db(c);
  if (nseq == 0) return fail(c, 2, "database has no sequences");
  uint64_t first = 0, last = 0;
  if (on_device) {
    HIPCHK(c, hipMemcpy(&first, offsets, 8, hipMemcpyDeviceToHost));
    HIPCHK(c, hipMemcpy(&last, offsets + nseq, 8, hipMemcpyDeviceToHost));
  } else {
    first = offsets[0];
    last = offsets[nseq];
  }
  if (first != 0) return fail(c, 2, "offsets[0] must be 0");
  if (last >= (1ull << 36)) return fail(c, 2, "database larger than 2^36 bases");
  c->nseq = nseq;
  c->nbases = last;
  c->db_words = (last + 15) / 16;
  c->h_seq_off.resize((size_t)nseq + 1);
  if (on_device) HIPCHK(c, hipMemcpy(c->h_seq_off.data(), offsets, ((uint64_t)nseq + 1) * 8, hipMemcpyDeviceToHost));
  else memcpy(c->h_seq_off.data(), offsets, ((uint64_t)nseq + 1) * 8);
  const uint64_t alloc_words = c->db_words + 64;
  HIPCHK(c, hipMalloc((void**)&c->db2, alloc_words * 4));
  HIPCHK(c, hipMalloc((void**)&c->dbm2, alloc_words * 4));
  HIPCHK(c, hipMemsetAsync(c->db2, 0, alloc_words * 4, c->stream));
  HIPCHK(c, hipMemsetAsync(c->dbm2, 0, alloc_words * 4, c->stream));
  HIPCHK(c, hipMalloc((void**)&c->seq_off, ((uint64_t)nseq + 1) * 8));
  HIPCHK(c, hipMemcpyAsync(c->seq_off, offsets, ((uint64_t)nseq + 1) * 8,
                           on_device ? hipMemcpyDeviceToDevice : hipMemcpyHostToDevice, c->stream));
  HIPCHK(c, hipMemsetAsync(c->d_flag, 0, 4, c->stream));
  return 0;
}

int musc_db_load_ascii(musc_ctx* c, const char* seqs, const uint64_t* offsets, uint32_t nseq, int on_device) {
  if (!c) return 1;
  if (!seqs || !offsets) return fail(c, 2, "musc_db_load_ascii: NULL input");
  int rc = db_alloc(c, offsets, nseq, on_device);
  if (rc) return rc;
  const unsigned char* src = (const unsigned char*)seqs;
  TmpBufs B;
  unsigned char* tmp = nullptr;
  if (!on_device && c->nbases) {
    HIPCHK(c, B.alloc(&tmp, c->nbases));
    HIPCHK(c, hipMemcpyAsync(tmp, seqs, c->nbases, hipMemcpyHostToDevice, c->stream));
    src = tmp;
  }
  if (c->db_words) {
    hipLaunchKernelGGL(k_pack_db_ascii, dim3(nblk(c->db_words, 256)), dim3(256), 0, c->stream, src, c->nbases,
                       c->db2, c->dbm2, c->db_words, c->d_flag);
    HIPCHK(c, hipGetLastError());
  }
  return db_finish(c);
}

int musc_db_load_packed(musc_ctx* c, const uint8_t* bases2bit, const uint8_t* nmask, const uint64_t* seq_offsets,
                        uint32_t nseq) {
  if (!c) return 1;
  if (!bases2bit || !seq_offsets) return fail(c, 2, "musc_db_load_packed: NULL input");
  int rc = db_alloc(c, seq_offsets, nseq, 0);
  if (rc) return rc;
  TmpBufs B;
  uint32_t* t2 = nullptr;
  uint16_t* tm = nullptr;
  const uint64_t w = c->db_words;
  if (w) {
    HIPCHK(c, B.alloc(&t2, w * 4));
    HIPCHK(c, hipMemsetAsync(t2, 0, w * 4, c->stream));
    HIPCHK(c, hipMemcpyAsync(t2, bases2bit, (c->nbases + 3) / 4, hipMemcpyHostToDevice, c->stream));
    if (nmask) {
      HIPCHK(c, B.alloc(&tm, w * 2));
      HIPCHK(c, hipMemsetAsync(tm, 0, w * 2, c->stream));
      HIPCHK(c, hipMemcpyAsync(tm, nmask, (c->nbases + 7) / 8, hipMemcpyHostToDevice, c->stream));
    }
    hipLaunchKernelGGL(k_pack_db_packed, dim3(nblk(w, 256)), dim3(256), 0, c->stream, t2, tm, c->db2, c->dbm2, w,
                       c->d_flag);
    HIPCHK(c, hipGetLastError());
  }
  return db_finish(c);
}

extern "C++" {
struct IdxRange {
  uint32_t g0, g1;
  uint64_t b0, b1, size;
};
static IdxRange whole_db(const musc_ctx* c) { return IdxRange{0, c->nseq, 0, c->nbases, c->nbases}; }

static uint64_t index_room(musc_ctx* c, uint64_t reserve) {
  size_t mfree = 0, mtotal = 0;
  if (hipMemGetInfo(&mfree, &mtotal) != hipSuccess) {
    (void)hipGetLastError();
    return 0;
  }
  const uint64_t have = (uint64_t)mfree + c->idx_T_bytes + c->idx_E_cap * sizeof(uint4) +
                        (c->ctx_T ? c->ctx_T_cap * sizeof(CtxBucket) : 0) + (c->ctx_E ? c->ctx_E_cap * sizeof(CtxEntry) : 0);
  uint64_t room = have > reserve ? have - reserve : 0;
  if (c->env.index_budget_mb > 0) room = std::min<uint64_t>(room, (uint64_t)c->env.index_budget_mb << 20);
  return room;
}

static uint64_t lines_need(uint64_t nb, uint64_t bases) {
  return (nb + 1) * (sizeof(LineBucket) + 8) + (bases > 7 * nb ? (bases - 7 * nb) * 16 : 0) + nb * 64;
}
static uint64_t classic64_need(uint64_t nb, uint64_t bases) { return (nb + 1) * (sizeof(Bucket) + 16) + bases * sizeof(uint4); }
static const uint64_t LINES_RESERVE = 12ull << 30, CLASSIC_RESERVE = 4ull << 30, CTX_RESERVE = 4ull << 30;

static bool want_line_buckets(musc_ctx* c, int32_t ww, int bits, int direct, uint64_t bases) {
  if (c->env.index == EnvKnobs::IDX_LINES) return true;
  if (c->env.index == EnvKnobs::IDX_CLASSIC64) return false;
  if (!direct) return false;
  (void)ww;
  const uint64_t nb = 1ull << bits;
  if (bases < 4 * nb) return false;
  return lines_need(nb, bases) <= index_room(c, LINES_RESERVE);
}

static void classic_table(const musc_ctx* c, int32_t ww, uint64_t bases, int* bits, int* direct) {
  *direct = 0;
  const uint64_t floor_bases = std::max<uint64_t>(bases, 1ull << 19);
  if (2 * ww <= 30 && (1ull << (2 * ww)) <= 32 * floor_bases) {
    *bits = 2 * ww;
    *direct = 1;
  } else {
    *bits = 10;
    while (*bits < 31 && (1ull << *bits) < bases) (*bits)++;
  }
  if (c->env.index_bits >= 8 && c->env.index_bits <= 31) { *bits = c->env.index_bits; *direct = 0; }
}

static void ctx_table(const musc_ctx* c, int32_t ww, uint64_t bases, int* bits, int* direct) {
  *direct = 0;
  const uint64_t floor_bases = std::max<uint64_t>(bases, 1ull << 9);
  if (2 * ww <= 30 && ((1ull << (2 * ww)) <= 2 * floor_bases || c->env.ctx_direct)) {
    *bits = 2 * ww;
    *direct = 1;
  } else {
    *bits = 10;
    while (*bits < 30 && (1ull << *bits) < bases) (*bits)++;
  }
  if (c->env.index_bits >= 8 && c->env.index_bits <= 30) { *bits = c->env.index_bits; *direct = 0; }
}
static uint64_t ctx_need(int bits, int wide, uint64_t bases) {
  const uint64_t esz = wide ? sizeof(CtxEntryW) : sizeof(CtxEntry);
  return ((1ull << bits) + 1) * (sizeof(CtxBucket) + 12) + bases / (wide ? 2 : 3) * esz;
}

template <class BT>
static int build_index_buckets(musc_ctx* c, int32_t ww, int bits, int direct, const IdxRange& R) {
  const uint64_t nb = 1ull << bits;
  c->ev_used = 0;
  hipEvent_t e0 = pool_event(c), e1 = pool_event(c), e2 = pool_event(c), e3 = pool_event(c);
  if (!e0 || !e1 || !e2 || !e3) return fail(c, 10, "hipEventCreate failed");
  if (c->idx_T_bytes < (nb + 1) * sizeof(BT)) {
    if (c->idx_T) (void)hipFree(c->idx_T);
    c->idx_T = nullptr;
    c->idx_T_bytes = 0;
    HIPCHK(c, hipMalloc((void**)&c->idx_T, (nb + 1) * sizeof(BT)));
    c->idx_T_bytes = (nb + 1) * sizeof(BT);
  }
  BT* const T = reinterpret_cast<BT*>(c->idx_T);
  TmpBufs B;
  uint64_t *tmp = nullptr, *stmp = nullptr;
  HIPCHK(c, B.alloc(&tmp, (nb + 1 + 16) * 8));
  HIPCHK(c, B.alloc(&stmp, scan_tmp_elems(nb + 1) * 8));
  HIPCHK(c, hipEventRecord(e0, c->stream));
  HIPCHK(c, hipMemsetAsync(T, 0, (nb + 1) * sizeof(BT), c->stream));
  const unsigned blocks = (unsigned)std::min<uint64_t>((R.b1 - R.b0 + 255) / 256, 1u << 22);
  if (R.b1 > R.b0) {
    hipLaunchKernelGGL((k_index<false, BT>), dim3(blocks), dim3(256), 0, c->stream, c->db2, c->dbm2, c->seq_off, c->nseq,
                       R.b0, R.b1, ww, bits, direct, c->wide, T, (uint4*)nullptr);
    HIPCHK(c, hipGetLastError());
  }
  hipLaunchKernelGGL((k_index_ovf_count<BT>), dim3(nblk(nb + 1, 256)), dim3(256), 0, c->stream, T, nb, tmp);
  HIPCHK(c, hipGetLastError());
  int rc = scan_u64(c, tmp, tmp, nb + 1, stmp);
  if (rc) return rc;
  uint64_t novf = 0;
  HIPCHK(c, hipMemcpyAsync(&novf, tmp + nb, 8, hipMemcpyDeviceToHost, c->stream));
  hipLaunchKernelGGL((k_index_ovf_set<BT>), dim3(nblk(nb, 256)), dim3(256), 0, c->stream, T, nb, tmp);
  HIPCHK(c, hipGetLastError());
  HIPCHK(c, hipEventRecord(e2, c->stream));
  HIPCHK(c, hipStreamSynchronize(c->stream));
  B.release();
  if (std::is_same<BT, LineBucket>::value) {
    if (novf >= 0xFFFFFFF0ull) return fail(c, 5, "internal: %llu overflow lines do not fit 32-bit numbers", (unsigned long long)novf);
    novf *= 8;
  }
  c->idx_novf = novf;
  if (c->idx_E_cap < novf + 16) {
    if (c->idx_E) (void)hipFree(c->idx_E);
    c->idx_E = nullptr;
    c->idx_E_cap = 0;
    HIPCHK(c, hipMalloc((void**)&c->idx_E, ((uint64_t)novf + 16) * sizeof(uint4)));
    c->idx_E_cap = novf + 16;
  }
  HIPCHK(c, hipEventRecord(e3, c->stream));
  if (R.b1 > R.b0) {
    hipLaunchKernelGGL((k_index<true, BT>), dim3(blocks), dim3(256), 0, c->stream, c->db2, c->dbm2, c->seq_off, c->nseq,
                       R.b0, R.b1, ww, bits, direct, c->wide, T, c->idx_E);
    HIPCHK(c, hipGetLastError());
  }
  HIPCHK(c, hipEventRecord(e1, c->stream));
  HIPCHK(c, hipStreamSynchronize(c->stream));
  float ms = 0, ms2 = 0;
  (void)hipEventElapsedTime(&ms, e0, e2);
  (void)hipEventElapsedTime(&ms2, e3, e1);
  c->stats.ms_index_build = ms + ms2;
  return 0;
}
}

static int build_index_classic(musc_ctx* c, int32_t ww, const IdxRange& R, int lines_kind) {
  c->wide = c->nbases >= 0xFFFFFFF0ull || c->env.force_wide;
  if (c->wide && c->nseq >= (1u << 24))
    return fail(c, 5, "a database of 2^32 bases or more may hold at most 2^24 targets (has %u)", c->nseq);
  int bits, direct;
  classic_table(c, ww, R.size, &bits, &direct);
  if (c->idx_ww == ww && c->idx_kind == 0 && c->idx_T && c->idx_bits == bits && c->idx_direct == direct &&
      c->idx_g0 == R.g0 && c->idx_g1 == R.g1 && (lines_kind < 0 || c->idx_lines == (lines_kind == 1)) &&
      !(c->env.index == EnvKnobs::IDX_LINES && !c->idx_lines) && !(c->env.index == EnvKnobs::IDX_CLASSIC64 && c->idx_lines))
    return 0;
  const bool lines = lines_kind >= 0 ? lines_kind == 1 : want_line_buckets(c, ww, bits, direct, R.size) && bits <= 30;
  free_index(c);
  drop_ctx_index(c);
  c->idx_kind = 0;
  c->idx_lines = lines;
  const int rc = lines ? build_index_buckets<LineBucket>(c, ww, bits, direct, R) : build_index_buckets<Bucket>(c, ww, bits, direct, R);
  if (rc) return rc;
  c->idx_ww = ww;
  c->idx_bits = bits;
  c->idx_direct = direct;
  c->idx_g0 = R.g0;
  c->idx_g1 = R.g1;
  return 0;
}

int musc_db_build_index(musc_ctx* c, int32_t ww) {
  if (!c) return 1;
  if (!c->db2) return fail(c, 4, "no database loaded");
  if (ww < 1 || ww > 4096) return fail(c, 2, "bad window width %d", ww);
  HIPCHK(c, hipSetDevice(c->device));
  return build_index_classic(c, ww, whole_db(c), -1);
}

static int build_index_ctx(musc_ctx* c, int32_t ww, int32_t CL, int wide, const IdxRange& R) {
  int bits, direct;
  ctx_table(c, ww, R.size, &bits, &direct);
  if (c->idx_kind == 1 && c->idx_ww == ww && c->idx_CL == CL && c->idx_wide == wide && c->idx_bits == bits &&
      c->idx_direct == direct && c->idx_g0 == R.g0 && c->idx_g1 == R.g1 && c->ctx_T)
    return 0;
  free_index(c);
  c->wide = 0;
  const uint64_t nb = 1ull << bits;
  if (ctx_need(bits, wide, R.size) > index_room(c, CTX_RESERVE)) return 100;
  if (c->idx_T) (void)hipFree(c->idx_T);
  if (c->idx_E) (void)hipFree(c->idx_E);
  c->idx_T = nullptr;
  c->idx_E = nullptr;
  c->idx_T_bytes = c->idx_E_cap = 0;
  c->ev_used = 0;
  hipEvent_t e0 = pool_event(c), e1 = pool_event(c), e2 = pool_event(c), e3 = pool_event(c);
  if (!e0 || !e1 || !e2 || !e3) return fail(c, 10, "hipEventCreate failed");
  if (c->ctx_T_cap < nb + 1) {
    if (c->ctx_T) (void)hipFree(c->ctx_T);
    c->ctx_T = nullptr;
    c->ctx_T_cap = 0;
    if (hipMalloc((void**)&c->ctx_T, (nb + 1) * sizeof(CtxBucket)) != hipSuccess) {
      (void)hipGetLastError();
      c->ctx_T = nullptr;
      return 100;
    }
    c->ctx_T_cap = nb + 1;
  }
  TmpBufs B;
  uint64_t *tmp = nullptr, *stmp = nullptr;
  uint32_t* cursor = nullptr;
  if (B.alloc(&tmp, (nb + 1 + 16) * 8) != hipSuccess || B.alloc(&stmp, scan_tmp_elems(nb + 1) * 8) != hipSuccess ||
      B.alloc(&cursor, (nb + 1) * 4) != hipSuccess) {
    (void)hipGetLastError();
    return 100;
  }
  HIPCHK(c, hipEventRecord(e0, c->stream));
  HIPCHK(c, hipMemsetAsync(c->ctx_T, 0, (nb + 1) * sizeof(CtxBucket), c->stream));
  HIPCHK(c, hipMemsetAsync(cursor, 0, (nb + 1) * 4, c->stream));
  const unsigned blocks = (unsigned)std::min<uint64_t>((R.b1 - R.b0 + 255) / 256, 1u << 22);
  const uint32_t* const xm2 = c->db_has_x ? c->dbm2 : nullptr;
  const uint32_t* const xbl = c->db_has_x ? c->dbx : nullptr;
  if (R.b1 > R.b0) {
    hipLaunchKernelGGL((k_index_ctx<false, false>), dim3(blocks), dim3(256), 0, c->stream, c->db2, xm2, xbl, c->seq_off, c->nseq, c->nbases,
                       R.b0, R.b1, ww, bits, direct, CL, c->ctx_T, (void*)nullptr, cursor);
    HIPCHK(c, hipGetLastError());
  }
  hipLaunchKernelGGL(k_ctx_ovf_count, dim3(nblk(nb + 1, 256)), dim3(256), 0, c->stream, c->ctx_T, nb,
                     (uint32_t)(wide ? CTXW_INLINE : CTX_INLINE), tmp);
  HIPCHK(c, hipGetLastError());
  int rc = scan_u64(c, tmp, tmp, nb + 1, stmp);
  if (rc) return rc;
  uint64_t novf = 0;
  HIPCHK(c, hipMemcpyAsync(&novf, tmp + nb, 8, hipMemcpyDeviceToHost, c->stream));
  hipLaunchKernelGGL(k_ctx_ovf_set, dim3(nblk(nb, 256)), dim3(256), 0, c->stream, c->ctx_T, nb, tmp);
  HIPCHK(c, hipGetLastError());
  HIPCHK(c, hipEventRecord(e2, c->stream));
  HIPCHK(c, hipStreamSynchronize(c->stream));
  if (novf >= 0xFFFFFFF0ull) return fail(c, 5, "internal: %llu overflow entries do not fit 32-bit offsets", (unsigned long long)novf);
  c->idx_novf = novf;
  const uint64_t ecap = (ctx_entries_bytes(novf + 16, wide) + sizeof(CtxEntry) - 1) / sizeof(CtxEntry);
  if (c->ctx_E_cap < ecap) {
    if (c->ctx_E) (void)hipFree(c->ctx_E);
    c->ctx_E = nullptr;
    c->ctx_E_cap = 0;
    if (hipMalloc((void**)&c->ctx_E, ecap * sizeof(CtxEntry)) != hipSuccess) {
      (void)hipGetLastError();
      c->ctx_E = nullptr;
      return 100;
    }
    c->ctx_E_cap = ecap;
  }
  HIPCHK(c, hipEventRecord(e3, c->stream));
  if (R.b1 > R.b0) {
    if (wide)
      hipLaunchKernelGGL((k_index_ctx<true, true>), dim3(blocks), dim3(256), 0, c->stream, c->db2, xm2, xbl, c->seq_off, c->nseq, c->nbases,
                         R.b0, R.b1, ww, bits, direct, CL, c->ctx_T, (void*)c->ctx_E, cursor);
    else
      hipLaunchKernelGGL((k_index_ctx<true, false>), dim3(blocks), dim3(256), 0, c->stream, c->db2, xm2, xbl, c->seq_off, c->nseq, c->nbases,
                         R.b0, R.b1, ww, bits, direct, CL, c->ctx_T, (void*)c->ctx_E, cursor);
    HIPCHK(c, hipGetLastError());
  }
  HIPCHK(c, hipEventRecord(e1, c->stream));
  HIPCHK(c, hipStreamSynchronize(c->stream));
  float ms = 0, ms2 = 0;
  (void)hipEventElapsedTime(&ms, e0, e2);
  (void)hipEventElapsedTime(&ms2, e3, e1);
  c->stats.ms_index_build = ms + ms2;
  c->idx_kind = 1;
  c->idx_wide = wide;
  c->idx_ww = ww;
  c->idx_CL = CL;
  c->idx_bits = bits;
  c->idx_direct = direct;
  c->idx_g0 = R.g0;
  c->idx_g1 = R.g1;
  return 0;
}

enum MatchKind { MK_LANE = 2, MK_DMA = 3 };
static int match_kind(const musc_ctx* c, int W) {
  if (c->env.match_dma && W == 2 && c->rw == 8 && c->idx_kind == 1 && !c->idx_wide && !c->db_has_x && !c->reads_have_x) return MK_DMA;
  return MK_LANE;
}

static bool reads_xpos(musc_ctx* c, int wide) {
  if (c->rdx_epoch == c->data_epoch && c->rdx_wide == wide) return true;
  if (ensure(c, c->rdx, c->nreads)) return false;
  if (wide)
    hipLaunchKernelGGL(k_read_xpos<true>, dim3(nblk(c->nreads, 256)), dim3(256), 0, c->stream, c->rd, c->rdm, c->nreads, c->rw, c->rdx.p);
  else
    hipLaunchKernelGGL(k_read_xpos<false>, dim3(nblk(c->nreads, 256)), dim3(256), 0, c->stream, c->rd, c->rdm, c->nreads, c->rw, c->rdx.p);
  if (hipGetLastError() != hipSuccess) return false;
  c->rdx_epoch = c->data_epoch;
  c->rdx_wide = wide;
  c->xok_epoch = ~0ull;
  c->xokdb_epoch = ~0ull;
  return true;
}

static bool reads_x_fit(musc_ctx* c, const musc_params* P, uint32_t max_len, int wide) {
  if (!c->rdm || !c->rd || !c->nreads) return false;
  if (c->env.no_x_context) return false;
  if (!reads_xpos(c, wide)) return false;
  max_len = std::max(max_len, c->max_len);
  if (c->xok_epoch == c->data_epoch && c->xok_pmatch == P->pmatch && c->xok_mmp1 == P->max_mismatch_p1) return c->xok;
  std::vector<uint16_t> tab((size_t)max_len + 2);
  for (uint32_t L = 0; L < tab.size(); L++) {
    volatile double a = 1.0 - P->pmatch;
    volatile double b = a * (double)L;
    long long v = (long long)b;
    if (P->max_mismatch_p1 > 0) v = P->max_mismatch_p1 - 1;
    if (v < 0) v = 0;
    if (v > 0xFFFE) v = 0xFFFE;
    tab[L] = (uint16_t)v;
  }
  TmpBufs B;
  uint16_t* d_tab = nullptr;
  uint32_t bad = 1;
  if (B.alloc(&d_tab, tab.size() * 2) != hipSuccess) return false;
  if (hipMemcpyAsync(d_tab, tab.data(), tab.size() * 2, hipMemcpyHostToDevice, c->stream) != hipSuccess) return false;
  if (hipMemsetAsync(c->d_flag, 0, 4, c->stream) != hipSuccess) return false;
  hipLaunchKernelGGL(k_xpos_check, dim3(nblk(c->nreads, 256)), dim3(256), 0, c->stream, c->rd, c->rdx.p, c->nreads, c->rw, d_tab,
                     max_len, wide ? XPos<true>::MAX : XPos<false>::MAX, c->d_flag);
  if (hipMemcpyAsync(&bad, c->d_flag, 4, hipMemcpyDeviceToHost, c->stream) != hipSuccess) return false;
  if (hipStreamSynchronize(c->stream) != hipSuccess) return false;
  c->xok = bad == 0;
  c->xok_epoch = c->data_epoch;
  c->xok_pmatch = P->pmatch;
  c->xok_mmp1 = P->max_mismatch_p1;
  return c->xok;
}

static bool reads_x_fit_db(musc_ctx* c, const musc_params* P, int wide) {
  if (!c->rdm || !c->rd || !c->nreads) return false;
  if (!reads_xpos(c, wide)) return false;
  int32_t key[CTX_MAX_W + 3] = {P->n_windows, P->window_width, wide};
  XWins wn;
  memset(&wn, 0, sizeof wn);
  wn.n = P->n_windows;
  wn.ww = P->window_width;
  for (int k = 0; k < P->n_windows && k < CTX_MAX_W; k++) key[3 + k] = wn.q1[k] = P->windows[k];
  if (c->xokdb_epoch == c->data_epoch && memcmp(key, c->xokdb_key, sizeof key) == 0) return c->xokdb;
  uint32_t bad = 1;
  if (hipMemsetAsync(c->d_flag, 0, 4, c->stream) != hipSuccess) return false;
  if (wide) hipLaunchKernelGGL(k_xpos_check_db<true>, dim3(nblk(c->nreads, 256)), dim3(256), 0, c->stream, c->rdx.p, c->nreads, wn, c->d_flag);
  else hipLaunchKernelGGL(k_xpos_check_db<false>, dim3(nblk(c->nreads, 256)), dim3(256), 0, c->stream, c->rdx.p, c->nreads, wn, c->d_flag);
  if (hipMemcpyAsync(&bad, c->d_flag, 4, hipMemcpyDeviceToHost, c->stream) != hipSuccess) return false;
  if (hipStreamSynchronize(c->stream) != hipSuccess) return false;
  c->xokdb = bad == 0;
  c->xokdb_epoch = c->data_epoch;
  memcpy(c->xokdb_key, key, sizeof key);
  return c->xokdb;
}

static bool ctx_eligible(musc_ctx* c, const musc_params* P, uint32_t max_len, int* CL, int* wide) {
  if (c->env.index != EnvKnobs::IDX_AUTO) return false;
  if (c->db_has_x && (c->max_tlen >= 0x80000000ull || c->nseq > (1u << 24) || c->env.no_x_context)) return false;
  if (c->nbases >= 0xFFFFFFF0ull || c->env.force_wide) return false;
  if (P->n_windows > CTX_MAX_W) return false;
  int q1min = P->windows[0], q1max = P->windows[0];
  for (int k = 1; k < P->n_windows; k++) {
    q1min = std::min(q1min, P->windows[k]);
    q1max = std::max(q1max, P->windows[k]);
  }
  const int64_t span = (int64_t)q1max - q1min + (int64_t)max_len;
  const int wenv = c->env.context;
  *CL = q1max;
  *wide = 0;
  if (span > CTX_BASES || q1max > CTX_BASES || wenv == 2) {
    if (wenv == 1) return false;
    if (span > CTXW_BASES || q1max > CTXW_BASES) return false;
    *wide = 1;
  }
  if (c->reads_have_x && !(c->db_has_x ? reads_x_fit_db(c, P, *wide) : reads_x_fit(c, P, max_len, *wide))) return false;
  return true;
}

enum { PK_CTX = 1, PK_LINES = 2, PK_CLASSIC64 = 3 };
static const uint32_t MAX_PARTITIONS = 4096;

static int index_kind_for(musc_ctx* c, int32_t ww, bool ctx_ok, int wide, uint64_t bases, bool fit, uint64_t extra) {
  int bits, direct;
  if (ctx_ok) {
    ctx_table(c, ww, bases, &bits, &direct);
    if (ctx_need(bits, wide, bases) <= index_room(c, CTX_RESERVE + extra)) return PK_CTX;
  }
  classic_table(c, ww, bases, &bits, &direct);
  const uint64_t nb = 1ull << bits;
  const bool lines = bits <= 30 && (c->env.index == EnvKnobs::IDX_LINES ||
                                    (c->env.index != EnvKnobs::IDX_CLASSIC64 && direct && bases >= 4 * nb &&
                                     lines_need(nb, bases) <= index_room(c, LINES_RESERVE + extra)));
  if (lines) return !fit || lines_need(nb, bases) <= index_room(c, LINES_RESERVE + extra) ? PK_LINES : 0;
  return !fit || classic64_need(nb, bases) <= index_room(c, CLASSIC_RESERVE + extra) ? PK_CLASSIC64 : 0;
}

static uint64_t merge_reserve(const musc_ctx* c) {
  const uint64_t tuples = std::max<uint64_t>(c->hits.cap, c->nreads);
  return 20 * (c->nreads + 1) + (4ull << BLOCK_TABLE_BITS) + 20 * tuples;
}

static bool cut_targets(const musc_ctx* c, uint64_t limit, std::vector<uint32_t>* first, uint64_t* largest) {
  const std::vector<uint64_t>& off = c->h_seq_off;
  limit = std::min(limit, c->nbases);
  first->assign(1, 0u);
  *largest = 0;
  uint32_t g = 0;
  while (g < c->nseq) {
    uint32_t g1 = (uint32_t)(std::upper_bound(off.begin() + g + 1, off.begin() + c->nseq + 1, off[g] + limit) - off.begin()) - 1;
    if (g1 <= g) g1 = g + 1;
    *largest = std::max<uint64_t>(*largest, off[g1] - off[g]);
    first->push_back(g1);
    if (first->size() > MAX_PARTITIONS + 1) return false;
    g = g1;
  }
  return true;
}

static int plan_partitions(musc_ctx* c, const musc_params* P, uint32_t max_len) {
  const int32_t ww = P->window_width;
  const std::vector<uint32_t> one = {0u, c->nseq};
  if (!c->part_bases && c->idx_ww == ww && c->idx_g0 == 0 && c->idx_g1 == c->nseq && c->nseq) {
    c->part_first = one;
    return 0;
  }
  int CL = 0, wide = 0;
  const bool ctx_ok = ctx_eligible(c, P, max_len, &CL, &wide);
  std::vector<uint32_t> first;
  uint64_t largest = 0;
  int kind = 0;
  if (c->part_bases) {
    if (!cut_targets(c, c->part_bases, &first, &largest))
      return fail(c, 5, "DbPartitionBases %llu cuts the database into more than %u partitions",
                  (unsigned long long)c->part_bases, MAX_PARTITIONS);
    const uint64_t extra = first.size() > 2 ? merge_reserve(c) : 0;
    kind = index_kind_for(c, ww, ctx_ok, wide, largest, true, extra);
    if (!kind) kind = index_kind_for(c, ww, false, wide, largest, false, 0);
  } else if (index_kind_for(c, ww, ctx_ok, wide, c->nbases, true, 0)) {
    first = one;
  } else {
    uint32_t lo = 2, hi = MAX_PARTITIONS;
    bool found = false;
    while (lo <= hi) {
      const uint32_t n = lo + (hi - lo) / 2;
      std::vector<uint32_t> f;
      uint64_t lg = 0;
      const bool ok = cut_targets(c, (c->nbases + n - 1) / n, &f, &lg);
      const int k = ok ? index_kind_for(c, ww, ctx_ok, wide, lg, true, merge_reserve(c)) : 0;
      if (k) {
        first.swap(f);
        largest = lg;
        kind = k;
        found = true;
        hi = n - 1;
      } else {
        lo = n + 1;
      }
    }
    if (!found)
      return fail(c, 5, "the index of this database does not fit the device even in %u partitions", MAX_PARTITIONS);
  }
  c->part_first = first;
  c->part_kind = first.size() > 2 ? kind : 0;
  c->part_size = first.size() > 2 ? largest : c->nbases;
  return 0;
}

static int ensure_index(musc_ctx* c, const musc_params* P, uint32_t max_len) {
  int CL = 0, wide = 0;
  if (c->part_first.size() > 2) {
    const uint32_t p = c->cur_part;
    const uint32_t g0 = c->part_first[p], g1 = c->part_first[p + 1];
    const IdxRange R{g0, g1, c->h_seq_off[g0], c->h_seq_off[g1], c->part_size};
    if (c->part_kind == PK_CTX) {
      if (!ctx_eligible(c, P, max_len, &CL, &wide)) return fail(c, 12, "internal: a partition lost context-bucket eligibility");
      const int rc = build_index_ctx(c, P->window_width, CL, wide, R);
      if (rc == 100)
        return fail(c, 5, "the context index of partition %u (%llu bases) does not fit the device", p,
                    (unsigned long long)(R.b1 - R.b0));
      return rc;
    }
    return build_index_classic(c, P->window_width, R, c->part_kind == PK_LINES ? 1 : 0);
  }
  if (ctx_eligible(c, P, max_len, &CL, &wide)) {
    const int rc = build_index_ctx(c, P->window_width, CL, wide, whole_db(c));
    if (rc != 100) return rc;
  }
  return musc_db_build_index(c, P->window_width);
}

int musc_db_build_index_for(musc_ctx* c, const musc_params* P, int32_t max_read_len) {
  if (!c) return 1;
  int rc = check_params(c, P);
  if (rc) return rc;
  if (!c->db2) return fail(c, 4, "no database loaded");
  HIPCHK(c, hipSetDevice(c->device));
  const uint32_t ml = max_read_len > 0 ? (uint32_t)max_read_len
                                       : (P->max_read_length > 0 ? (uint32_t)P->max_read_length : c->max_len);
  if ((rc = plan_partitions(c, P, ml))) return rc;
  c->cur_part = 0;
  return ensure_index(c, P, ml);
}

int musc_db_set_partition_bases(musc_ctx* c, uint64_t max_bases) {
  if (!c) return 1;
  c->part_bases = max_bases;
  return 0;
}

int musc_db_partitions(musc_ctx* c, uint32_t* first_target, uint32_t cap, uint32_t* n) {
  if (!c) return 1;
  if (!n) return fail(c, 2, "musc_db_partitions: n is NULL");
  *n = c->part_first.empty() ? 0u : (uint32_t)c->part_first.size() - 1;
  if (!first_target || !*n) return 0;
  if (cap < *n + 1) return fail(c, 2, "musc_db_partitions: room for %u boundaries < %u", cap, *n + 1);
  memcpy(first_target, c->part_first.data(), (*n + 1) * sizeof(uint32_t));
  return 0;
}


static int upload_prepare(musc_ctx* c, uint64_t r0, uint64_t n, hipStream_t st) {
  musc_ctx::Upload& u = c->up;
  if (!u.active) return 0;
  const uint64_t want = std::min<uint64_t>(r0 + n, c->nreads);
  while (u.packed_upto < want) {
    const uint64_t i = u.packed_upto / u.piece;
    const uint64_t first = i * u.piece, cnt = std::min<uint64_t>(u.piece, c->nreads - first);
    HIPCHK(c, hipStreamWaitEvent(st, u.ev[i], 0));
    hipLaunchKernelGGL(k_pack_reads_fixed, dim3(nblk(cnt * (uint64_t)c->rw, 256)), dim3(256), 0, st, u.stage, first, cnt, u.L, c->rw, c->rd);
    HIPCHK(c, hipGetLastError());
    u.packed_upto = first + cnt;
  }
  if (u.packed_upto >= c->nreads) u.active = false;
  return 0;
}

static int reads_load(musc_ctx* c, const unsigned char* ascii, const uint8_t* bases2bit, const uint8_t* nmask,
                      const uint64_t* offsets, uint64_t nreads, int on_device, bool packed) {
  HIPCHK(c, hipSetDevice(c->device));
  free_reads(c);
  if (nreads >= 0xFFFFFFF0ull) return fail(c, 2, "too many reads for 32-bit read_idx");
  c->nreads = nreads;
  if (nreads == 0) {
    c->rw = 4;
    return 0;
  }
  TmpBufs B;
  uint64_t* d_off = nullptr;
  const uint64_t* offp = offsets;
  if (!on_device) {
    HIPCHK(c, B.alloc(&d_off, (nreads + 1) * 8));
    HIPCHK(c, hipMemcpyAsync(d_off, offsets, (nreads + 1) * 8, hipMemcpyHostToDevice, c->stream));
    offp = d_off;
  }
  HIPCHK(c, hipMemsetAsync(c->counters + 4, 0, 8, c->stream));
  hipLaunchKernelGGL(k_max_len, dim3(std::min(nblk(nreads, 256), MAX_GRID)), dim3(256), 0, c->stream, offp, nreads, c->counters + 4);
  HIPCHK(c, hipGetLastError());
  HIPCHK(c, hipMemcpyAsync(c->h_pinned, c->counters + 4, 8, hipMemcpyDeviceToHost, c->stream));
  uint64_t first = 0, total = 0;
  HIPCHK(c, hipMemcpyAsync(&first, offp, 8, hipMemcpyDeviceToHost, c->stream));
  HIPCHK(c, hipMemcpyAsync(&total, offp + nreads, 8, hipMemcpyDeviceToHost, c->stream));
  HIPCHK(c, hipStreamSynchronize(c->stream));
  const uint64_t maxlen = c->h_pinned[0];
  if (first != 0) return fail(c, 2, "read offsets[0] must be 0");
  if (maxlen > 65535) return fail(c, 2, "read of %llu bases exceeds the 65535-base record limit", (unsigned long long)maxlen);
  c->max_len = (uint32_t)maxlen;
  int rw = (int)((2 * maxlen + 31) / 32) + 1;
  rw = (rw + 3) & ~3;
  if (rw < 4) rw = 4;
  c->rw = rw;
  const uint64_t words = nreads * (uint64_t)rw;
  if (words >= (1ull << 32)) return fail(c, 2, "too many read words for one dispatch (reads x record words >= 2^32)");
  HIPCHK(c, hipMalloc((void**)&c->rd, words * 4 + 256));
  HIPCHK(c, hipMemsetAsync(c->rd + words, 0, 256, c->stream));
  const bool may_have_x = !packed || nmask != nullptr;
  if (may_have_x) {
    HIPCHK(c, hipMalloc((void**)&c->rdm, words * 4 + 256));
    HIPCHK(c, hipMemsetAsync(c->rdm + words, 0, 256, c->stream));
  }
  uint32_t* d_hasx = c->d_flag;
  HIPCHK(c, hipMemsetAsync(d_hasx, 0, 4, c->stream));
  unsigned char *t1 = nullptr, *t2 = nullptr;
  if (!packed) {
    const unsigned char* src = ascii;
    if (!on_device && total) {
      HIPCHK(c, B.alloc(&t1, total));
      HIPCHK(c, hipMemcpyAsync(t1, ascii, total, hipMemcpyHostToDevice, c->stream));
      src = t1;
    }
    hipLaunchKernelGGL(k_pack_reads<false>, dim3(nblk(words, 256)), dim3(256), 0, c->stream, src,
                       (const uint32_t*)nullptr, (const uint32_t*)nullptr, offp, nreads, rw, c->rd, c->rdm, d_hasx);
  } else {
    const uint64_t b2 = ((total + 3) / 4 + 7) & ~3ull, bm = ((total + 7) / 8 + 7) & ~3ull;
    HIPCHK(c, B.alloc(&t1, b2 + 16));
    HIPCHK(c, hipMemsetAsync(t1, 0, b2 + 16, c->stream));
    HIPCHK(c, hipMemcpyAsync(t1, bases2bit, (total + 3) / 4, hipMemcpyHostToDevice, c->stream));
    if (nmask) {
      HIPCHK(c, B.alloc(&t2, bm + 16));
      HIPCHK(c, hipMemsetAsync(t2, 0, bm + 16, c->stream));
      HIPCHK(c, hipMemcpyAsync(t2, nmask, (total + 7) / 8, hipMemcpyHostToDevice, c->stream));
    }
    hipLaunchKernelGGL(k_pack_reads<true>, dim3(nblk(words, 256)), dim3(256), 0, c->stream,
                       (const unsigned char*)nullptr, (const uint32_t*)t1, (const uint32_t*)t2, offp, nreads, rw,
                       c->rd, c->rdm, d_hasx);
  }
  HIPCHK(c, hipGetLastError());
  uint32_t hasx = 0;
  HIPCHK(c, hipMemcpyAsync(&hasx, d_hasx, 4, hipMemcpyDeviceToHost, c->stream));
  HIPCHK(c, hipStreamSynchronize(c->stream));
  c->reads_have_x = hasx != 0;
  if (!hasx && c->rdm) {
    (void)hipFree(c->rdm);
    c->rdm = nullptr;
  }
  return 0;
}

static int reads_load_fixed(musc_ctx* c, const uint8_t* bases2bit, uint32_t L, uint64_t nreads, int async) {
  HIPCHK(c, hipSetDevice(c->device));
  free_reads(c);
  if (nreads >= 0xFFFFFFF0ull) return fail(c, 2, "too many reads for 32-bit read_idx");
  if (L > 65535) return fail(c, 2, "read of %u bases exceeds the 65535-base record limit", L);
  c->nreads = nreads;
  if (nreads == 0) {
    c->rw = 4;
    return 0;
  }
  c->max_len = L;
  int rw = (int)((2ull * L + 31) / 32) + 1;
  rw = (rw + 3) & ~3;
  if (rw < 4) rw = 4;
  c->rw = rw;
  const uint64_t words = nreads * (uint64_t)rw;
  if (words >= (1ull << 32)) return fail(c, 2, "too many read words for one dispatch (reads x record words >= 2^32)");
  HIPCHK(c, hipMalloc((void**)&c->rd, words * 4 + 256));
  HIPCHK(c, hipMemsetAsync(c->rd + words, 0, 256, c->stream));
  c->reads_have_x = false;
  musc_ctx::Upload& u = c->up;
  const uint64_t total_bytes = (nreads * (uint64_t)L + 3) / 4;
  const uint64_t need_words = (total_bytes + 3) / 4 + 4;
  if (u.stage_words < need_words) {
    if (u.stage) (void)hipFree(u.stage);
    u.stage = nullptr;
    u.stage_words = 0;
    HIPCHK(c, hipMalloc((void**)&u.stage, need_words * 4));
    u.stage_words = need_words;
  }
  if (!u.s_up) HIPCHK(c, hipStreamCreateWithFlags(&u.s_up, hipStreamNonBlocking));
  uint64_t piece = std::max<uint64_t>(c->batch_reads / 4, 64);
  piece = (piece + 63) & ~63ull;
  u.piece = piece;
  u.n_pieces = (nreads + piece - 1) / piece;
  u.L = L;
  u.packed_upto = 0;
  while (u.ev.size() < u.n_pieces) {
    hipEvent_t e = nullptr;
    HIPCHK(c, hipEventCreateWithFlags(&e, hipEventDisableTiming));
    u.ev.push_back(e);
  }
  HIPCHK(c, hipMemsetAsync(u.stage + (need_words - 4), 0, 16, u.s_up));
  for (uint64_t i = 0; i < u.n_pieces; i++) {
    const uint64_t b0 = i * piece * (uint64_t)L / 4;
    const uint64_t b1 = std::min<uint64_t>(((i + 1) * piece * (uint64_t)L + 3) / 4, total_bytes);
    HIPCHK(c, hipMemcpyAsync(reinterpret_cast<uint8_t*>(u.stage) + b0, bases2bit + b0, b1 - b0, hipMemcpyHostToDevice, u.s_up));
    HIPCHK(c, hipEventRecord(u.ev[i], u.s_up));
  }
  u.active = true;
  if (!async) {
    int rc = upload_prepare(c, 0, nreads, c->stream);
    if (rc) return rc;
    HIPCHK(c, hipStreamSynchronize(c->stream));
  }
  return 0;
}

int musc_reads_load_packed32(musc_ctx* c, const uint8_t* bases2bit, const uint8_t* nmask, const uint32_t* lengths,
                             uint32_t fixed_len, uint64_t nreads, int async) {
  if (!c) return 1;
  if (!bases2bit && nreads) return fail(c, 2, "musc_reads_load_packed32: NULL input");
  if (!lengths && !nmask) return reads_load_fixed(c, bases2bit, fixed_len, nreads, async);
  HIPCHK(c, hipSetDevice(c->device));
  TmpBufs B;
  uint64_t *d_off = nullptr, *stmp = nullptr;
  uint32_t* d_len = nullptr;
  HIPCHK(c, B.alloc(&d_off, (nreads + 2) * 8));
  if (lengths) {
    HIPCHK(c, B.alloc(&d_len, (nreads + 1) * 4));
    HIPCHK(c, B.alloc(&stmp, scan_tmp_elems(nreads + 1) * 8));
    HIPCHK(c, hipMemcpyAsync(d_len, lengths, nreads * 4, hipMemcpyHostToDevice, c->stream));
    hipLaunchKernelGGL(k_widen_u32, dim3(nblk(nreads + 1, 256)), dim3(256), 0, c->stream, d_len, nreads, d_off);
    HIPCHK(c, hipGetLastError());
    int rc = scan_u64(c, d_off, d_off, nreads + 1, stmp);
    if (rc) return rc;
  } else {
    hipLaunchKernelGGL(k_iota_mul, dim3(nblk(nreads + 1, 256)), dim3(256), 0, c->stream, d_off, nreads, (uint64_t)fixed_len);
    HIPCHK(c, hipGetLastError());
  }
  return reads_load(c, nullptr, bases2bit, nmask, d_off, nreads, 1, true);
}

int musc_reads_load_ascii(musc_ctx* c, const char* seqs, const uint64_t* offsets, uint64_t nreads, int on_device) {
  if (!c) return 1;
  if ((!seqs || !offsets) && nreads) return fail(c, 2, "musc_reads_load_ascii: NULL input");
  return reads_load(c, (const unsigned char*)seqs, nullptr, nullptr, offsets, nreads, on_device, false);
}

int musc_reads_load_packed(musc_ctx* c, const uint8_t* bases2bit, const uint8_t* nmask, const uint64_t* read_offsets,
                           uint64_t nreads) {
  if (!c) return 1;
  if ((!bases2bit || !read_offsets) && nreads) return fail(c, 2, "musc_reads_load_packed: NULL input");
  return reads_load(c, nullptr, bases2bit, nmask, read_offsets, nreads, 0, true);
}


extern "C++" {
static size_t match_dyn_lds(int kind, int W, int block_mode) {
  if (kind == MK_DMA) return block_mode == 1 ? (size_t)(4u << MATCHG_SKETCH_BITS) : 0u;
  const size_t wcnt = (size_t)TILE * W * 4 * (kind == MK_LANE ? 2 : 1);
  return block_mode ? wcnt + (block_mode == 1 ? (4u << MATCH_SKETCH_BITS) : 0u) : 0u;
}

typedef Inst<match_kernel_t> MatchInst;
#define INST_T(RW, W, XM, WD, SG) MatchInst{k_match_t<RW, W, XM, WD, SG>, inst_id(MUSC_INST_MATCH_T, RW, W, XM, WD, SG)}
#define INST_G(RW, SG) MatchInst{k_match_g<RW, SG>, inst_id(MUSC_INST_MATCH_G, RW, 0, 0, 0, SG)}
template <int RW, bool WD>
static MatchInst lane_instance(int W, int xm) {
  static const MatchInst k[4][3] = {
      {INST_T(RW, 1, 0, WD, 0), INST_T(RW, 1, 1, WD, 0), INST_T(RW, 1, 2, WD, 0)},
      {INST_T(RW, 2, 0, WD, 0), INST_T(RW, 2, 1, WD, 0), INST_T(RW, 2, 2, WD, 0)},
      {INST_T(RW, 3, 0, WD, 0), INST_T(RW, 3, 1, WD, 0), INST_T(RW, 3, 2, WD, 0)},
      {INST_T(RW, 4, 0, WD, 0), INST_T(RW, 4, 1, WD, 0), INST_T(RW, 4, 2, WD, 0)}};
  return k[(W >= 1 && W <= 3 ? W : 4) - 1][xm];
}

static MatchInst match_instance(int kind, int spec_geom, int rw, bool wide, int W, int xm) {
  if (kind == MK_DMA) return spec_geom == 1 ? INST_G(8, 1) : INST_G(8, 0);
  if (spec_geom == 1) return INST_T(8, 2, 0, false, 1);
  return by_rw(rw, [&](auto r) -> MatchInst {
    constexpr int RW = decltype(r)::value;
    if constexpr (RW == 0) return MatchInst{nullptr, 0};
    else if (wide) return lane_instance<RW, true>(W, xm);
    else if constexpr (RW <= 12) return lane_instance<RW, false>(W, xm);
    else return MatchInst{nullptr, 0};
  });
}

static MatchInst match_kernel(const musc_ctx* c, int W) {
  const int xm = c->db_has_x ? 2 : c->reads_have_x ? 1 : 0;
  return match_instance(match_kind(c, W), c->spec_geom, c->rw, c->idx_wide != 0, W, xm);
}

static unsigned match_resident(musc_ctx* c, match_kernel_t kern, int W, int block_mode) {
  int per_cu = 0, ncu = 0;
  const size_t lds = match_dyn_lds(match_kind(c, W), W, block_mode);
  const void* fn = reinterpret_cast<const void*>(kern);
  hipError_t e = hipOccupancyMaxActiveBlocksPerMultiprocessor(&per_cu, fn, TILE, lds);
  if (e != hipSuccess || per_cu < 1) { (void)hipGetLastError(); per_cu = 2; }
  {
    hipFuncAttributes fa;
    if (hipFuncGetAttributes(&fa, fn) == hipSuccess) {
      const size_t total = ((size_t)fa.sharedSizeBytes + lds + 2047) / 2048 * 2048;
      const int fit = total ? (int)((160u << 10) / total) : per_cu;
      if (fit >= 1 && fit < per_cu) per_cu = fit;
    } else {
      (void)hipGetLastError();
    }
  }
  if (hipDeviceGetAttribute(&ncu, hipDeviceAttributeMultiprocessorCount, c->device) != hipSuccess || ncu < 1) ncu = 256;
  unsigned resident = (unsigned)per_cu * (unsigned)ncu;
  if (c->env.debug_grid >= 1 && (unsigned)c->env.debug_grid < resident) resident = (unsigned)c->env.debug_grid;
  return resident;
}

static void launch_match(musc_ctx* c, match_kernel_t kern, uint64_t r0, uint32_t n, int W, int block_mode, uint32_t block_thr,
                         unsigned ngrid) {
  const size_t lds = match_dyn_lds(match_kind(c, W), W, block_mode);
  const uint32_t* const rdx = c->reads_have_x ? (const uint32_t*)c->rdx.p : (const uint32_t*)nullptr;
  hipLaunchKernelGGL(kern, dim3(ngrid), dim3(TILE), lds, c->stream, c->rd, r0, n, c->d_mp, c->nmiss_tab.p, c->ctx_T,
                     c->ctx_E, c->stage.p, c->stage.cap, c->spill.p, c->spill.cap, c->bs[0].tbase.p, c->tcount2.p,
                     block_mode, block_thr, c->block_table.p, c->counters, rdx);
}
}

static int match_device_impl(musc_ctx* c, const musc_params* P, uint64_t* nhits);
static int match_index_pass(musc_ctx* c, const musc_params* P, uint64_t* nhits);

extern "C++" {
template <int SG>
static bool spec_geom_equals(const MatchParams& mp) {
  typedef SpecGeom<SG> G;
  if (mp.W != G::nwin || mp.ww != G::ww || mp.CL != G::CL || mp.min_dinuc != G::min_dinuc || mp.direct != 1 || mp.bits != 2 * G::ww) return false;
  for (int k = 0; k < G::nwin; k++)
    if (mp.win[k] != G::win[k] || mp.need[k] != (1u << k) - 1u) return false;
  return true;
}
}
static int spec_geom_matches(const musc_ctx* c, const MatchParams& mp) {
  if (c->env.no_spec) return 0;
  if (c->rw != 8 || c->idx_wide || c->db_has_x || c->reads_have_x) return 0;
  if (spec_geom_equals<1>(mp)) return 1;
  return 0;
}

static int match_ctx_pass(musc_ctx* c, const musc_params* P, const PathParams& pp, int block_mode, uint64_t max_matches, uint64_t planned_batches, uint64_t* nhits) {
  int rc = 0;
  if (c->rw != 4 && c->rw != 8 && c->rw != 12 && !(c->rw == 16 && c->idx_wide))
    return fail(c, 12, "internal: record stride %d on the context path", c->rw);
  {
    static thread_local MatchParams mp;
    memset(&mp, 0, sizeof mp);
    mp.W = pp.W; mp.ww = pp.ww; mp.min_dinuc = pp.min_dinuc; mp.bits = pp.bits; mp.direct = pp.direct;
    mp.mmtol = pp.mmtol; mp.apply_mmtol = pp.apply_mmtol; mp.max_len = pp.max_len; mp.CL = c->idx_CL;
    mp.q1zero_mask = pp.q1zero_mask;
    mp.seq_off = c->db_has_x ? c->seq_off : nullptr;
    mp.dbm2 = c->db_has_x ? c->dbm2 : nullptr;
    for (int k = 0; k < pp.W && k < CTX_MAX_W; k++) mp.win[k] = pp.win[k];
    match_tables(mp);
    c->spec_geom = spec_geom_matches(c, mp);
    c->stats.match_variant = (match_kind(c, pp.W) == MK_DMA ? 4u : 2u) + (c->spec_geom ? 1u : 0u);
    if (!c->h_mp_valid || memcmp(&mp, &c->h_mp, sizeof mp) != 0) {
      c->h_mp = mp;
      HIPCHK(c, hipMemcpyAsync(c->d_mp, &c->h_mp, sizeof mp, hipMemcpyHostToDevice, c->stream));
      HIPCHK(c, hipStreamSynchronize(c->stream));
      c->h_mp_valid = true;
    }
  }
  const MatchInst inst = match_kernel(c, pp.W);
  const match_kernel_t kern = inst.fn;
  c->last_inst[0] = inst.id;
  if (!kern) return fail(c, 12, "internal: no fused kernel instance for record stride %d, %d windows", c->rw, pp.W);
  const unsigned resident = match_resident(c, kern, pp.W, block_mode);
  uint32_t block_thr = (uint32_t)std::min<uint64_t>(max_matches / (planned_batches * resident), 0x7FFFFFFFull);
  if (block_mode == 1 && block_thr < 2) block_mode = 2;
  c->last_inst[3] = (uint32_t)block_mode | (c->force_exact_blocks ? 0x100u : 0u);
  if (block_mode == 2 && !c->block_table.p) {
    if ((rc = ensure(c, c->block_table, 1ull << BLOCK_TABLE_BITS))) return rc;
  }
  const bool check_blocks = block_mode != 0;
  const bool sized = c->sized_epoch == c->data_epoch && c->sized_exact_blocks == (block_mode == 2) &&
                     memcmp(&c->sized_params, P, sizeof *P) == 0 && !c->env.debug_sync;
  uint32_t bsz = sized ? c->sized_bsz : c->batch_reads;
  const uint64_t L = c->max_len;
  const bool use_graph = sized && c->env.graph > 0 && !c->graph_failed;
  if (!sized && c->graph_exec) {
    (void)hipGraphExecDestroy(c->graph_exec);
    c->graph_exec = nullptr;
  }
  for (int attempt = 0;; attempt++) {
    if (attempt > 40) return fail(c, 12, "internal: the context pass did not converge on buffer sizes");
    Timer tm(c);
    hipEvent_t ev0 = pool_event(c), ev1 = pool_event(c);
    if (!ev0 || !ev1) return fail(c, 10, "hipEventCreate failed");
    const bool replay = use_graph && c->graph_exec && c->graph_epoch == c->data_epoch && c->graph_block_mode == block_mode &&
                        memcmp(&c->graph_params, P, sizeof *P) == 0;
    const bool capture = use_graph && !replay;
    if (capture && c->graph_exec) {
      (void)hipGraphExecDestroy(c->graph_exec);
      c->graph_exec = nullptr;
    }
    tm.off = capture || replay;
    CaptureGuard cap;
    if (!replay) {
      if (capture) {
        if (cap.begin(c->stream) != hipSuccess) {
          (void)hipGetLastError();
          c->graph_failed = true;
          return match_index_pass(c, P, nhits);
        }
      } else {
        HIPCHK(c, hipEventRecord(ev0, c->stream));
      }
    }
    uint64_t n_cand = 0, n_cmp = 0, n_windows = 0, n_ovf = 0, r0 = 0;
    c->stats.n_batches = 0;
    c->stats.match_launches = 0;
    bool again = false;
    if (!replay) {
      HIPCHK(c, hipMemsetAsync(c->counters, 0, 16 * sizeof(unsigned long long), c->stream));
      if (block_mode == 2) HIPCHK(c, hipMemsetAsync(c->block_table.p, 0, (1ull << BLOCK_TABLE_BITS) * 4, c->stream));
    }
    while (!replay && r0 < c->nreads) {
      const uint32_t n = (uint32_t)std::min<uint64_t>(bsz, c->nreads - r0);
      const uint32_t ntiles = nblk(n, WT);
      const uint64_t sgrid = std::min<uint64_t>(nblk(n, TILE), resident);
      const uint64_t swaves = sgrid * (TILE / 64);
      if (!sized) {
        if ((rc = ensure(c, c->bs[0].tbase, (uint64_t)ntiles + 1))) return rc;
        if ((rc = ensure(c, c->scan_tmp, scan_tmp_elems((uint64_t)ntiles + 1)))) return rc;
        if ((rc = ensure(c, c->tcount2, (uint64_t)ntiles + 1))) return rc;
        if ((rc = ensure(c, c->tpre, (uint64_t)ntiles + 1))) return rc;
        if ((rc = ensure(c, c->stage, std::max<uint64_t>(2ull * n, swaves * 64)))) return rc;
        if ((rc = ensure(c, c->spill, swaves * 32))) return rc;
        HIPCHK(c, hipMemsetAsync(c->counters + 8, 0, 8 * sizeof(unsigned long long), c->stream));
      }
      if ((rc = upload_prepare(c, r0, n, c->stream))) return rc;
      tm.begin(0);
      {
        Range rg("k_match");
        launch_match(c, kern, r0, n, pp.W, block_mode, block_thr, (unsigned)sgrid);
      }
      HIPCHK(c, hipGetLastError());
      tm.end(0);
      c->stats.match_launches++;
      c->stats.n_batches++;
      if (!sized) {
        HIPCHK(c, hipMemcpyAsync(&c->h_pinned[0], c->counters, 16 * 8, hipMemcpyDeviceToHost, c->stream));
        HIPCHK(c, hipStreamSynchronize(c->stream));
        const uint64_t need_stage = c->h_pinned[8 + 7] * swaves, need_spill = 2 * c->h_pinned[8 + 5] * swaves;
        if (need_stage > (1ull << 31)) {
          if (n == 1) return fail(c, 6, "one read has %llu tuples (> 2^31)", (unsigned long long)c->h_pinned[8 + 7]);
          bsz = n / 2;
          again = true;
          break;
        }
        if (c->h_pinned[3] & 8ull)
          return fail(c, 12, "internal: the kernel instance specialised for geometry %d refused this run's parameters", c->spec_geom);
        if (c->h_pinned[3] || need_stage > c->stage.cap || need_spill > c->spill.cap) {
          if (need_stage > c->stage.cap && (rc = ensure(c, c->stage, need_stage + need_stage / 4 + swaves))) return rc;
          if (need_spill > c->spill.cap && (rc = ensure(c, c->spill, need_spill + need_spill / 4 + swaves))) return rc;
          again = true;
          break;
        }
        n_windows += c->h_pinned[8 + 0];
        n_cmp += c->h_pinned[8 + 1];
        n_cand += c->h_pinned[8 + 3];
        n_ovf += c->h_pinned[8 + 4];
        if ((rc = ensure(c, c->hits, c->h_pinned[2] + c->h_pinned[8 + 6], true))) return rc;
      }
      Range rgc("scan + k_compact_w");
      tm.begin(4);
      tm.begin(1);
      rc = scan_u32(c, c->tcount2.p, c->tpre.p, (uint64_t)ntiles + 1, false, c->scan_tmp.p, c->stream);
      if (rc) return rc;
      tm.end(1);
      hipLaunchKernelGGL(k_compact_w, dim3(std::min(nblk(ntiles, 4), 4u * MAX_GRID)), dim3(256), 0, c->stream, ntiles,
                         c->bs[0].tbase.p, c->tcount2.p, c->tpre.p, c->stage.p, reinterpret_cast<uint4*>(c->hits.p),
                         c->hits.cap, c->counters);
      HIPCHK(c, hipGetLastError());
      hipLaunchKernelGGL(k_advance, dim3(1), dim3(64), 0, c->stream, c->tpre.p, ntiles, c->counters);
      HIPCHK(c, hipGetLastError());
      tm.end(4);
      r0 += n;
    }
    if (again) continue;
    c->last_pp = pp;
    c->last_max_matches = (uint32_t)max_matches;
    c->last_exact_blocks = block_mode == 2;
    if (!replay) {
      if (block_mode == 2) {
        hipLaunchKernelGGL(k_block_overflow, dim3(1024), dim3(256), 0, c->stream, c->block_table.p, (uint32_t)max_matches,
                           c->counters);
        HIPCHK(c, hipGetLastError());
      }
      if (!capture) HIPCHK(c, hipEventRecord(ev1, c->stream));
      HIPCHK(c, hipMemcpyAsync(c->h_pinned, c->counters, 16 * 8, hipMemcpyDeviceToHost, c->stream));
    }
    if (capture) {
      hipGraph_t g = nullptr;
      hipError_t ge = cap.end(&g);
      if (ge == hipSuccess) ge = hipGraphInstantiate(&c->graph_exec, g, nullptr, nullptr, 0);
      if (g) (void)hipGraphDestroy(g);
      if (ge != hipSuccess) {
        (void)hipGetLastError();
        c->graph_exec = nullptr;
        c->graph_failed = true;
        return match_index_pass(c, P, nhits);
      }
      c->graph_epoch = c->data_epoch;
      c->graph_params = *P;
      c->graph_block_mode = block_mode;
      c->graph_batches = c->stats.n_batches;
    }
    if (capture || replay) {
      c->stats.n_batches = c->stats.match_launches = c->graph_batches;
      HIPCHK(c, hipEventRecord(ev0, c->stream));
      HIPCHK(c, hipGraphLaunch(c->graph_exec, c->stream));
      HIPCHK(c, hipEventRecord(ev1, c->stream));
    }
    HIPCHK(c, hipStreamSynchronize(c->stream));
    if (c->h_pinned[3] & 8ull)
      return fail(c, 12, "internal: the kernel instance specialised for geometry %d refused this run's parameters", c->spec_geom);
    if (c->h_pinned[3]) {
      if (!sized) return fail(c, 12, "internal: a capacity guard fired although every batch was sized (flags %llu)",
                              (unsigned long long)c->h_pinned[3]);
      c->sized_epoch = 0;
      return match_index_pass(c, P, nhits);
    }
    if (sized) {
      n_windows = c->h_pinned[8 + 0];
      n_cmp = c->h_pinned[8 + 1];
      n_cand = c->h_pinned[8 + 3];
      n_ovf = c->h_pinned[8 + 4];
    }
    c->stats.n_read_windows = n_windows;
    c->stats.n_candidates = n_cand;
    c->stats.n_pairs = n_cmp;
    c->stats.n_descriptors = 0;
    c->stats.n_overflow_entries = n_ovf;
    c->stats.n_accepted = c->h_pinned[1];
    c->stats.n_hits = c->nhits = c->h_pinned[2];
    c->stats.n_overflow_blocks = check_blocks ? c->h_pinned[5] : ~0ull;
    if (block_mode == 1 && (c->h_pinned[6] || c->stats.n_batches > planned_batches)) {
      c->force_exact_blocks = true;
      c->exact_epoch = c->data_epoch;
      c->exact_params = *P;
      rc = match_index_pass(c, P, nhits);
      c->force_exact_blocks = false;
      return rc;
    }
    c->stats.ms_screen = tm.total(0);
    c->stats.ms_scan = tm.total(1);
    c->stats.ms_select = tm.total(4);
    (void)hipEventElapsedTime(&c->stats.ms_total, ev0, ev1);
    const uint64_t rec_b = (2 * L + 7) / 8;
    const uint64_t ent_b = c->idx_wide ? sizeof(CtxEntryW) : sizeof(CtxEntry);
    c->stats.match_bytes = c->nreads * rec_b + n_windows * sizeof(CtxBucket) + n_ovf * ent_b + 16 * c->stats.n_hits;
    c->stats.match_bytes_strict = c->nreads * rec_b + n_windows * 8 + n_cand * ent_b + 16 * c->stats.n_hits;
    if (nhits) *nhits = c->nhits;
    c->sized_epoch = c->data_epoch;
    c->sized_params = *P;
    c->sized_exact_blocks = block_mode == 2;
    c->sized_bsz = bsz;
    return 0;
  }
}

int musc_match_device(musc_ctx* c, const musc_params* P, uint64_t* nhits) {
  if (!c) return 1;
  const int rc = match_device_impl(c, P, nhits);
  if (rc != 0 && c->up.active && c->up.s_up) (void)hipStreamSynchronize(c->up.s_up);
  return rc;
}

static int match_partitioned(musc_ctx* c, const musc_params* P, uint64_t* nhits);

static int match_device_impl(musc_ctx* c, const musc_params* P, uint64_t* nhits) {
  Range rg_pass("musc_match_device");
  int rc = check_params(c, P);
  if (rc) return rc;
  if (!c->db2) return fail(c, 4, "no database loaded");
  if (!c->rd && c->nreads) return fail(c, 4, "no reads loaded");
  HIPCHK(c, hipSetDevice(c->device));
  if ((rc = plan_partitions(c, P, c->max_len))) return rc;
  c->cur_part = 0;
  if (c->part_first.size() > 2) return match_partitioned(c, P, nhits);
  return match_index_pass(c, P, nhits);
}

static int match_index_pass(musc_ctx* c, const musc_params* P, uint64_t* nhits) {
  int rc = ensure_index(c, P, c->max_len);
  if (rc) return rc;

  const float keep_index_ms = c->stats.ms_index_build;
  memset(&c->stats, 0, sizeof c->stats);
  c->stats.ms_index_build = keep_index_ms;
  c->stats.n_reads = c->nreads;
  c->nhits = 0;
  if (nhits) *nhits = 0;

  PathParams pp;
  memset(&pp, 0, sizeof pp);
  pp.W = P->n_windows;
  pp.ww = P->window_width;
  pp.min_dinuc = P->min_dinuc;
  pp.bits = c->idx_bits;
  pp.direct = c->idx_direct;
  pp.mmtol = P->mmtol > 0xFFFF ? 0xFFFF : P->mmtol;
  pp.apply_mmtol = P->apply_mmtol;
  pp.wide = c->wide;
  pp.max_len = (int32_t)c->max_len;
  for (int k = 0; k < pp.W; k++) {
    pp.win[k] = P->windows[k];
    if (P->windows[k] == 0) pp.q1zero_mask |= 1u << k;
  }

  if (c->nm_pmatch != P->pmatch || c->nm_mmp1 != P->max_mismatch_p1 || c->nm_maxlen != c->max_len || !c->nmiss_tab.p) {
    std::vector<uint16_t> tab((size_t)c->max_len + 2);
    for (uint32_t L = 0; L < tab.size(); L++) {
      volatile double a = 1.0 - P->pmatch;
      volatile double b = a * (double)L;
      long long v = (long long)b;
      if (P->max_mismatch_p1 > 0) v = P->max_mismatch_p1 - 1;
      if (v < 0) v = 0;
      if (v > 0xFFFE) v = 0xFFFE;
      tab[L] = (uint16_t)v;
    }
    rc = ensure(c, c->nmiss_tab, tab.size());
    if (rc) return rc;
    HIPCHK(c, hipMemcpyAsync(c->nmiss_tab.p, tab.data(), tab.size() * 2, hipMemcpyHostToDevice, c->stream));
    HIPCHK(c, hipStreamSynchronize(c->stream));
    c->nm_pmatch = P->pmatch;
    c->nm_mmp1 = P->max_mismatch_p1;
    c->nm_maxlen = c->max_len;
  }

  HIPCHK(c, hipMemsetAsync(c->counters, 0, 8 * sizeof(unsigned long long), c->stream));
  const uint64_t planned_batches = (c->nreads + c->batch_reads - 1) / c->batch_reads + 1;
  uint64_t max_matches = P->max_matches > 0 ? (uint64_t)P->max_matches : 0x7FFFFFFFull;
  if (P->n_shards > 1) max_matches /= (uint64_t)P->n_shards;
  const uint32_t block_thr = (uint32_t)std::min<uint64_t>(max_matches / (planned_batches * MAX_GRID), 0x7FFFFFFFull);
  const bool known_exact = c->exact_epoch == c->data_epoch && memcmp(&c->exact_params, P, sizeof *P) == 0;
  int block_mode = P->skip_block_check ? 0 : (c->force_exact_blocks || known_exact || block_thr < 2 ? 2 : 1);
  const bool check_blocks = block_mode != 0;
  c->cur_block_mode = block_mode;
  c->cur_block_thr = block_thr;
  if (block_mode == 2) {
    if ((rc = ensure(c, c->block_table, 1ull << BLOCK_TABLE_BITS))) return rc;
    HIPCHK(c, hipMemsetAsync(c->block_table.p, 0, (1ull << BLOCK_TABLE_BITS) * 4, c->stream));
  }
  if (!c->h_pp_valid || memcmp(&pp, &c->h_pp, sizeof pp) != 0) {
    c->h_pp = pp;
    HIPCHK(c, hipMemcpyAsync(c->d_pp, &c->h_pp, sizeof pp, hipMemcpyHostToDevice, c->stream));
    HIPCHK(c, hipStreamSynchronize(c->stream));
    c->h_pp_valid = true;
  }
  c->stats.index_kind = c->idx_kind == 1 ? (c->idx_wide ? 2u : 1u) : (c->idx_lines ? 3u : 0u);
  c->stats.match_variant = 0;
  c->last_inst[0] = c->last_inst[1] = c->last_inst[2] = 0;
  c->last_inst[3] = (uint32_t)block_mode | (c->force_exact_blocks ? 0x100u : 0u);
  c->stats.index_bytes = c->idx_kind == 1
                             ? ((1ull << c->idx_bits) + 1) * sizeof(CtxBucket) + ctx_entries_bytes(c->idx_novf + 16, c->idx_wide)
                             : ((1ull << c->idx_bits) + 1) * (c->idx_lines ? sizeof(LineBucket) : sizeof(Bucket)) + (c->idx_novf + 16) * sizeof(uint4);
  if (c->idx_kind == 1)
    return match_ctx_pass(c, P, pp, block_mode, max_matches, planned_batches, nhits);

  Timer tm(c);
  hipEvent_t ev0 = pool_event(c), ev1 = pool_event(c);
  if (!ev0 || !ev1) return fail(c, 10, "hipEventCreate failed");
  HIPCHK(c, hipEventRecord(ev0, c->stream));

  const bool mask = c->reads_have_x || c->db_has_x;
  if (mask && !c->rdm && c->nreads) {
    const uint64_t words = c->nreads * (uint64_t)c->rw;
    HIPCHK(c, hipMalloc((void**)&c->rdm, words * 4 + 256));
    HIPCHK(c, hipMemsetAsync(c->rdm, 0, words * 4 + 256, c->stream));
  }
  if (mask && !c->dbm2) {
    HIPCHK(c, hipMalloc((void**)&c->dbm2, (c->db_words + 64) * 4));
    HIPCHK(c, hipMemsetAsync(c->dbm2, 0, (c->db_words + 64) * 4, c->stream));
    if ((rc = db_xblocks(c))) return rc;
  }

  const bool sized = c->sized_epoch == c->data_epoch && c->sized_exact_blocks == (block_mode == 2) &&
                     memcmp(&c->sized_params, P, sizeof *P) == 0 && !c->env.debug_sync;
  uint64_t n_cand = 0, n_pairs = 0, n_windows = 0, n_two = 0;
  const uint64_t PAIR_CAP = 1ull << 31;
  uint64_t r0 = 0;
  uint32_t bsz = sized ? c->sized_bsz : c->batch_reads;
  if (sized) HIPCHK(c, hipMemsetAsync(c->counters + 8, 0, 8 * sizeof(unsigned long long), c->stream));
  const bool want_pipe = c->env.pipeline;
  const bool piped = sized && want_pipe && c->nreads > bsz && c->bs[1].cdesc.cap >= c->bs[0].cdesc.cap;
  hipStream_t sA = c->stream, sB = piped ? c->stream2 : c->stream;
  c->s_confirm = sB;
  c->cur = 0;
  if (piped) {
    HIPCHK(c, hipEventRecord(c->ev_join, sA));
    HIPCHK(c, hipStreamWaitEvent(sB, c->ev_join, 0));
  }
  uint32_t batch_no = 0;
  while (r0 < c->nreads) {
    const uint32_t n = (uint32_t)std::min<uint64_t>(bsz, c->nreads - r0);
    if (piped) {
      c->cur = (int)(batch_no & 1u);
      if (batch_no >= 2) HIPCHK(c, hipStreamWaitEvent(sA, c->ev_free[c->cur], 0));
    }
    const int W = pp.W;
    const uint32_t ntiles = nblk(n, TILE);
    uint64_t total = 1;
    if (!sized) {
      if ((rc = ensure(c, c->bs[c->cur].wb, (uint64_t)n * W))) return rc;
      if ((rc = ensure(c, c->bs[c->cur].rvalid, (uint64_t)n + 1))) return rc;
      if ((rc = ensure(c, c->bs[c->cur].tbase, (uint64_t)ntiles + 1))) return rc;
      if ((rc = ensure(c, c->bs[c->cur].tcount, (uint64_t)ntiles + 1))) return rc;
      if ((rc = ensure(c, c->scan_tmp, scan_tmp_elems((uint64_t)ntiles + 1)))) return rc;
      if ((rc = ensure(c, c->tcount2, (uint64_t)ntiles + 1))) return rc;
      if ((rc = ensure(c, c->tpre, (uint64_t)ntiles + 1))) return rc;
      if ((rc = ensure(c, c->bs[c->cur].cdesc, std::max<uint64_t>(4ull * n, 1024)))) return rc;
      HIPCHK(c, hipMemsetAsync(c->counters + 8, 0, 8 * sizeof(unsigned long long), c->stream));
    }

    if ((rc = upload_prepare(c, r0, n, c->stream))) return rc;
    tm.begin(0);
    {
      Range rg("k_screen");
      launch_screen(c, mask, r0, n, pp);
    }
    HIPCHK(c, hipGetLastError());
    tm.end(0);
    if (piped) {
      HIPCHK(c, hipEventRecord(c->ev_ready[c->cur], sA));
      HIPCHK(c, hipStreamWaitEvent(sB, c->ev_ready[c->cur], 0));
    }
    if (!sized) {
      HIPCHK(c, hipMemcpyAsync(&c->h_pinned[0], c->counters + 8, 8 * 8, hipMemcpyDeviceToHost, c->stream));
      HIPCHK(c, hipMemcpyAsync(&c->h_pinned[8], c->counters + 2, 8, hipMemcpyDeviceToHost, c->stream));
      HIPCHK(c, hipStreamSynchronize(c->stream));
      total = c->h_pinned[4];
      const uint64_t hits_so_far = c->h_pinned[8];
      const uint64_t sgrid = screen_grid(c, n, mask);
      const uint64_t need = c->h_pinned[7] * sgrid;
      if (need > PAIR_CAP) {
        if (n == 1) return fail(c, 6, "one read has %llu candidate pairs (> 2^31)", (unsigned long long)total);
        bsz = n / 2;
        HIPCHK(c, hipMemsetAsync(c->counters + 3, 0, 8, c->stream));
        continue;
      }
      if (c->h_pinned[7] > c->bs[c->cur].cdesc.cap / sgrid) {
        if ((rc = ensure(c, c->bs[c->cur].cdesc, need + need / 8 + sgrid))) return rc;
        HIPCHK(c, hipMemsetAsync(c->counters + 3, 0, 8, c->stream));
        continue;
      }
      n_windows += c->h_pinned[0];
      n_cand += c->h_pinned[3];
      n_pairs += c->h_pinned[4];
      n_two += c->h_pinned[5];
      if ((rc = ensure(c, c->p_nx, c->bs[c->cur].cdesc.cap))) return rc;
      if ((rc = ensure(c, c->stage, c->bs[c->cur].cdesc.cap))) return rc;
      if ((rc = ensure(c, c->hits, hits_so_far + total, true))) return rc;
    }
    c->stats.n_batches++;

    if (total) {
      const dim3 sg(std::min(nblk(n, TILE), MAX_GRID));

      tm.begin(3, sB);
      {
        Range rg("k_confirm");
        launch_confirm(c, mask, r0, n, pp);
      }
      HIPCHK(c, hipGetLastError());
      tm.end(3, sB);
      c->stats.confirm_launches++;

      Range rgc("scan + k_compact");
      tm.begin(4, sB);
      tm.begin(1, sB);
      rc = scan_u32(c, c->tcount2.p, c->tpre.p, (uint64_t)ntiles + 1, false, c->scan_tmp.p, sB);
      if (rc) return rc;
      tm.end(1, sB);
      hipLaunchKernelGGL(k_compact, sg, dim3(256), 0, sB, ntiles, c->bs[c->cur].tbase.p, c->tcount2.p, c->tpre.p,
                         c->stage.p, reinterpret_cast<uint4*>(c->hits.p), c->hits.cap, c->counters);
      HIPCHK(c, hipGetLastError());
      hipLaunchKernelGGL(k_advance, dim3(1), dim3(64), 0, sB, c->tpre.p, ntiles, c->counters);
      HIPCHK(c, hipGetLastError());
      tm.end(4, sB);
    }
    if (piped) HIPCHK(c, hipEventRecord(c->ev_free[c->cur], sB));
    r0 += n;
    batch_no++;
  }
  if (piped) {
    HIPCHK(c, hipEventRecord(c->ev_join, sB));
    HIPCHK(c, hipStreamWaitEvent(sA, c->ev_join, 0));
  }
  c->cur = 0;
  c->s_confirm = c->stream;
  c->last_pp = pp;
  c->last_max_matches = (uint32_t)max_matches;
  c->last_exact_blocks = block_mode == 2;
  if (block_mode == 2) {
    hipLaunchKernelGGL(k_block_overflow, dim3(1024), dim3(256), 0, c->stream, c->block_table.p,
                       (uint32_t)max_matches, c->counters);
    HIPCHK(c, hipGetLastError());
  }
  HIPCHK(c, hipEventRecord(ev1, c->stream));
  HIPCHK(c, hipMemcpyAsync(c->h_pinned, c->counters, 16 * 8, hipMemcpyDeviceToHost, c->stream));
  HIPCHK(c, hipStreamSynchronize(c->stream));
  if (sized) {
    if (c->h_pinned[3]) {
      c->sized_epoch = 0;
      return match_index_pass(c, P, nhits);
    }
    n_windows = c->h_pinned[8];
    n_cand = c->h_pinned[8 + 3];
    n_pairs = c->h_pinned[8 + 4];
    n_two = c->h_pinned[8 + 5];
  } else if (c->h_pinned[3]) {
    return fail(c, 12, "internal: a capacity guard fired although every batch was sized (flags %llu)",
                (unsigned long long)c->h_pinned[3]);
  }
  c->stats.n_read_windows = n_windows;
  c->stats.n_accepted = c->h_pinned[1];
  c->stats.n_hits = c->nhits = c->h_pinned[2];
  c->stats.n_descriptors = n_pairs;
  c->stats.n_pairs = n_pairs + n_two;
  c->stats.n_candidates = n_cand;
  c->stats.n_overflow_blocks = check_blocks ? c->h_pinned[5] : ~0ull;
  if (block_mode == 1 && (c->h_pinned[6] || c->stats.n_batches > planned_batches)) {
    c->force_exact_blocks = true;
    c->exact_epoch = c->data_epoch;
    c->exact_params = *P;
    rc = match_index_pass(c, P, nhits);
    c->force_exact_blocks = false;
    return rc;
  }
  c->stats.ms_screen = tm.total(0);
  c->stats.ms_scan = tm.total(1);
  c->stats.ms_confirm = tm.total(3);
  c->stats.ms_select = tm.total(4);
  (void)hipEventElapsedTime(&c->stats.ms_total, ev0, ev1);
  const uint64_t L = c->max_len;
  c->stats.confirm_bytes = c->stats.n_descriptors * (12 + (2 * L + 7) / 8 + (2 * L + 7) / 8 + 1) + 16 * c->stats.n_hits;
  if (nhits) *nhits = c->nhits;
  if (!sized && want_pipe) {
    if ((rc = ensure(c, c->bs[1].wb, c->bs[0].wb.cap)) || (rc = ensure(c, c->bs[1].rvalid, c->bs[0].rvalid.cap)) ||
        (rc = ensure(c, c->bs[1].tbase, c->bs[0].tbase.cap)) || (rc = ensure(c, c->bs[1].tcount, c->bs[0].tcount.cap)) ||
        (rc = ensure(c, c->bs[1].cdesc, c->bs[0].cdesc.cap)))
      return rc;
  }
  c->sized_epoch = c->data_epoch;
  c->sized_params = *P;
  c->sized_exact_blocks = block_mode == 2;
  c->sized_bsz = bsz;
  return 0;
}

static int match_partitions_run(musc_ctx* c, const musc_params* P, uint64_t* nhits) {
  const uint32_t np = (uint32_t)c->part_first.size() - 1;
  const uint64_t nr = c->nreads;
  const bool check_blocks = !P->skip_block_check;
  const uint32_t BT = 1u << BLOCK_TABLE_BITS;
  int rc = 0;
  if ((rc = ensure(c, c->pbest, nr + 1))) return rc;
  HIPCHK(c, hipMemsetAsync(c->pbest.p, 0xFF, (nr + 1) * 4, c->stream));
  if (check_blocks) {
    if ((rc = ensure(c, c->block_acc, BT))) return rc;
    HIPCHK(c, hipMemsetAsync(c->block_acc.p, 0, (uint64_t)BT * 4, c->stream));
  }
  musc_stats sum;
  memset(&sum, 0, sizeof sum);
  std::vector<uint64_t> seg(np + 1, 0);
  for (uint32_t p = 0; p < np && !rc; p++) {
    c->cur_part = p;
    uint64_t nh = 0;
    if ((rc = ensure_index(c, P, c->max_len))) break;
    const float build_ms = c->stats.ms_index_build;
    if ((rc = match_index_pass(c, P, &nh))) break;
    const musc_stats& s = c->stats;
    sum.n_read_windows += s.n_read_windows;
    sum.n_candidates += s.n_candidates;
    sum.n_pairs += s.n_pairs;
    sum.n_accepted += s.n_accepted;
    sum.confirm_bytes += s.confirm_bytes;
    sum.confirm_launches += s.confirm_launches;
    sum.n_batches += s.n_batches;
    sum.ms_screen += s.ms_screen;
    sum.ms_scan += s.ms_scan;
    sum.ms_confirm += s.ms_confirm;
    sum.ms_select += s.ms_select;
    sum.ms_total += s.ms_total;
    sum.ms_index_build += build_ms;
    sum.n_descriptors += s.n_descriptors;
    sum.match_launches += s.match_launches;
    sum.n_overflow_entries += s.n_overflow_entries;
    sum.match_bytes += s.match_bytes;
    sum.match_bytes_strict += s.match_bytes_strict;
    sum.index_kind = s.index_kind;
    sum.match_variant = s.match_variant;
    sum.index_bytes = s.index_bytes;
    if (nh) {
      if ((rc = ensure(c, c->pacc, seg[p] + nh, true))) break;
      HIPCHK(c, hipMemcpyAsync(c->pacc.p + seg[p], c->hits.p, nh * sizeof(musc_hit), hipMemcpyDeviceToDevice, c->stream));
      hipLaunchKernelGGL(k_part_best, dim3(std::min(nblk(nh, 256), 4u * MAX_GRID)), dim3(256), 0, c->stream,
                         reinterpret_cast<const uint4*>(c->pacc.p + seg[p]), nh, c->pbest.p);
      HIPCHK(c, hipGetLastError());
    }
    if (check_blocks) {
      hipLaunchKernelGGL(k_add_u32, dim3(nblk(BT, 256)), dim3(256), 0, c->stream, c->block_acc.p, c->block_table.p, (uint64_t)BT);
      HIPCHK(c, hipGetLastError());
    }
    seg[p + 1] = seg[p] + nh;
  }
  if (rc) return rc;

  Range rg("partition merge");
  hipEvent_t ev0 = pool_event(c), ev1 = pool_event(c);
  if (!ev0 || !ev1) return fail(c, 10, "hipEventCreate failed");
  HIPCHK(c, hipEventRecord(ev0, c->stream));
  const uint64_t total_in = seg[np];
  const uint32_t mmtol = P->mmtol > 0xFFFF ? 0xFFFFu : (uint32_t)P->mmtol;
  uint64_t max_seg = 0;
  for (uint32_t p = 0; p < np; p++) max_seg = std::max(max_seg, seg[p + 1] - seg[p]);
  if (max_seg >= 0xFFFFFFFFull) return fail(c, 6, "one partition returned %llu tuples (>= 2^32)", (unsigned long long)max_seg);
  if ((rc = ensure(c, c->pcnt, nr + 1)) || (rc = ensure(c, c->padj, nr + 1)) ||
      (rc = ensure(c, c->pflags, max_seg + 1)) || (rc = ensure(c, c->pflags_tmp, scan_tmp_elems(max_seg + 1))))
    return rc;
  if (scan_tmp_elems(nr + 1) * 2 > c->pflags_tmp.cap && (rc = ensure(c, c->pflags_tmp, scan_tmp_elems(nr + 1) * 2)))
    return rc;
  HIPCHK(c, hipMemsetAsync(c->pcnt.p, 0, (nr + 1) * 8, c->stream));
  if (total_in) {
    hipLaunchKernelGGL(k_part_count, dim3(std::min(nblk(total_in, 256), 4u * MAX_GRID)), dim3(256), 0, c->stream,
                       reinterpret_cast<const uint4*>(c->pacc.p), total_in, c->pbest.p, mmtol, P->apply_mmtol,
                       reinterpret_cast<unsigned long long*>(c->pcnt.p));
    HIPCHK(c, hipGetLastError());
  }
  if ((rc = scan_u64(c, c->pcnt.p, c->pcnt.p, nr + 1, reinterpret_cast<uint64_t*>(c->pflags_tmp.p)))) return rc;
  HIPCHK(c, hipMemcpyAsync(c->h_pinned, c->pcnt.p + nr, 8, hipMemcpyDeviceToHost, c->stream));
  HIPCHK(c, hipStreamSynchronize(c->stream));
  const uint64_t total = c->h_pinned[0];
  if ((rc = ensure(c, c->hits, total ? total : 1))) return rc;
  HIPCHK(c, hipMemsetAsync(c->d_flag, 0, 4, c->stream));
  for (uint32_t p = 0; p < np; p++) {
    const uint64_t n = seg[p + 1] - seg[p];
    if (!n) continue;
    const uint4* const h = reinterpret_cast<const uint4*>(c->pacc.p + seg[p]);
    const dim3 grid(std::min(nblk(n + 1, 256), 4u * MAX_GRID));
    hipLaunchKernelGGL(k_part_flags, grid, dim3(256), 0, c->stream, h, n, c->pbest.p, mmtol, P->apply_mmtol, c->pflags.p);
    HIPCHK(c, hipGetLastError());
    if ((rc = scan_u32(c, c->pflags.p, c->pflags.p, n + 1, false, c->pflags_tmp.p, c->stream))) return rc;
    hipLaunchKernelGGL(k_part_head, grid, dim3(256), 0, c->stream, h, n, c->pflags.p, c->pcnt.p, c->padj.p);
    HIPCHK(c, hipGetLastError());
    hipLaunchKernelGGL(k_part_scatter, grid, dim3(256), 0, c->stream, h, n, c->pflags.p, c->padj.p, c->pcnt.p,
                       reinterpret_cast<uint4*>(c->hits.p), total, c->d_flag);
    HIPCHK(c, hipGetLastError());
  }
  if (check_blocks) {
    HIPCHK(c, hipMemcpyAsync(c->block_table.p, c->block_acc.p, (uint64_t)BT * 4, hipMemcpyDeviceToDevice, c->stream));
    HIPCHK(c, hipMemsetAsync(c->counters + 5, 0, 8, c->stream));
    hipLaunchKernelGGL(k_block_overflow, dim3(1024), dim3(256), 0, c->stream, c->block_table.p, c->last_max_matches, c->counters);
    HIPCHK(c, hipGetLastError());
  }
  HIPCHK(c, hipEventRecord(ev1, c->stream));
  c->h_pinned[1] = 0;
  HIPCHK(c, hipMemcpyAsync(c->h_pinned, c->counters + 5, 8, hipMemcpyDeviceToHost, c->stream));
  HIPCHK(c, hipMemcpyAsync(c->h_pinned + 1, c->d_flag, 4, hipMemcpyDeviceToHost, c->stream));
  HIPCHK(c, hipStreamSynchronize(c->stream));
  if (c->h_pinned[1]) return fail(c, 12, "internal: the partition merge overran its %llu tuples", (unsigned long long)total);
  float merge_ms = 0;
  (void)hipEventElapsedTime(&merge_ms, ev0, ev1);
  sum.ms_select += merge_ms;
  sum.ms_total += merge_ms;
  sum.n_reads = nr;
  sum.n_hits = c->nhits = total;
  sum.n_overflow_blocks = check_blocks ? c->h_pinned[0] : ~0ull;
  c->stats = sum;
  c->last_exact_blocks = check_blocks;
  if (nhits) *nhits = total;
  return 0;
}

static int match_partitioned(musc_ctx* c, const musc_params* P, uint64_t* nhits) {
  const bool keep_force = c->force_exact_blocks;
  c->force_exact_blocks = true;
  const int rc = match_partitions_run(c, P, nhits);
  c->force_exact_blocks = keep_force;
  (void)hipStreamSynchronize(c->stream);
  c->pacc.release();
  c->pbest.release();
  c->pcnt.release();
  c->padj.release();
  c->pflags.release();
  c->pflags_tmp.release();
  c->block_acc.release();
  return rc;
}

int musc_hits_copy(musc_ctx* c, musc_hit* dst, uint64_t capacity, int dst_on_device) {
  if (!c) return 1;
  if (capacity < c->nhits) return fail(c, 2, "musc_hits_copy: capacity %llu < %llu hits",
                                       (unsigned long long)capacity, (unsigned long long)c->nhits);
  if (c->nhits == 0) return 0;
  if (!dst) return fail(c, 2, "musc_hits_copy: dst is NULL");
  HIPCHK(c, hipSetDevice(c->device));
  HIPCHK(c, hipMemcpyAsync(dst, c->hits.p, c->nhits * sizeof(musc_hit),
                           dst_on_device ? hipMemcpyDeviceToDevice : hipMemcpyDeviceToHost, c->stream));
  HIPCHK(c, hipStreamSynchronize(c->stream));
  return 0;
}

static int check_pack_bits(musc_ctx* c, const int32_t* bits, PackBits* b) {
  if (!bits) return fail(c, 2, "bits is NULL");
  int sum = 0;
  for (int i = 0; i < 4; i++) {
    if (bits[i] < 1 || bits[i] > 32) return fail(c, 2, "field width %d outside 1..32", bits[i]);
    sum += bits[i];
  }
  if (sum > 64) return fail(c, 2, "field widths add up to %d > 64 bits", sum);
  *b = PackBits{bits[0], bits[1], bits[2], bits[3]};
  return 0;
}

int musc_hits_copy_packed(musc_ctx* c, uint64_t* dst, uint64_t capacity, int dst_on_device, uint64_t read_base,
                          const int32_t* bits) {
  if (!c) return 1;
  PackBits b;
  int rc = check_pack_bits(c, bits, &b);
  if (rc) return rc;
  if (capacity < c->nhits) return fail(c, 2, "musc_hits_copy_packed: capacity %llu < %llu hits",
                                       (unsigned long long)capacity, (unsigned long long)c->nhits);
  if (c->nhits == 0) return 0;
  if (!dst) return fail(c, 2, "musc_hits_copy_packed: dst is NULL");
  HIPCHK(c, hipSetDevice(c->device));
  uint64_t* out = dst;
  if (!dst_on_device) {
    if ((rc = ensure(c, c->packed, c->nhits))) return rc;
    out = c->packed.p;
  }
  HIPCHK(c, hipMemsetAsync(c->d_flag, 0, 4, c->stream));
  hipLaunchKernelGGL(k_pack_hits, dim3(std::min(nblk(c->nhits, 256), MAX_GRID)), dim3(256), 0, c->stream,
                     reinterpret_cast<const uint4*>(c->hits.p), c->nhits, read_base, b, out, c->d_flag);
  HIPCHK(c, hipGetLastError());
  uint32_t bad = 0;
  HIPCHK(c, hipMemcpyAsync(&bad, c->d_flag, 4, hipMemcpyDeviceToHost, c->stream));
  if (!dst_on_device)
    HIPCHK(c, hipMemcpyAsync(dst, out, c->nhits * 8, hipMemcpyDeviceToHost, c->stream));
  HIPCHK(c, hipStreamSynchronize(c->stream));
  if (bad) return fail(c, 8, "musc_hits_copy_packed: a tuple field does not fit its width (%d/%d/%d/%d bits)",
                       b.read, b.gene, b.pos, b.nmiss);
  return 0;
}

int musc_hits_copy_compact(musc_ctx* c, uint32_t* words, uint64_t words_cap, uint8_t* counts, uint64_t counts_cap,
                           int dst_on_device, const int32_t* bits) {
  if (!c) return 1;
  if (!bits) return fail(c, 2, "bits is NULL");
  int sum = 0;
  for (int i = 0; i < 3; i++) {
    if (bits[i] < 1 || bits[i] > 30) return fail(c, 2, "field width %d outside 1..30", bits[i]);
    sum += bits[i];
  }
  if (sum > 32) return fail(c, 2, "field widths add up to %d > 32 bits", sum);
  if (words_cap < c->nhits) return fail(c, 2, "musc_hits_copy_compact: room for %llu tuples < %llu",
                                        (unsigned long long)words_cap, (unsigned long long)c->nhits);
  if (counts_cap < c->nreads) return fail(c, 2, "musc_hits_copy_compact: room for %llu reads < %llu",
                                          (unsigned long long)counts_cap, (unsigned long long)c->nreads);
  if ((c->nhits && !words) || (c->nreads && !counts)) return fail(c, 2, "musc_hits_copy_compact: NULL destination");
  HIPCHK(c, hipSetDevice(c->device));
  const PackBits b{0, bits[0], bits[1], bits[2]};
  uint32_t* dw = words;
  uint8_t* dc = counts;
  if (!dst_on_device) {
    int rc = ensure(c, c->packed, (c->nhits * 4 + c->nreads + 15) / 8 + 2);
    if (rc) return rc;
    dw = reinterpret_cast<uint32_t*>(c->packed.p);
    dc = reinterpret_cast<uint8_t*>(dw + c->nhits);
  }
  HIPCHK(c, hipMemsetAsync(c->d_flag, 0, 4, c->stream));
  if (c->nreads) HIPCHK(c, hipMemsetAsync(dc, 0, c->nreads, c->stream));
  if (c->nhits) {
    hipLaunchKernelGGL(k_pack_compact, dim3(std::min(nblk(c->nhits, 256), MAX_GRID)), dim3(256), 0, c->stream,
                       reinterpret_cast<const uint4*>(c->hits.p), c->nhits, b, dw, dc, c->d_flag);
    HIPCHK(c, hipGetLastError());
  }
  uint32_t bad = 0;
  HIPCHK(c, hipMemcpyAsync(&bad, c->d_flag, 4, hipMemcpyDeviceToHost, c->stream));
  if (!dst_on_device) {
    if (c->nhits) HIPCHK(c, hipMemcpyAsync(words, dw, c->nhits * 4, hipMemcpyDeviceToHost, c->stream));
    if (c->nreads) HIPCHK(c, hipMemcpyAsync(counts, dc, c->nreads, hipMemcpyDeviceToHost, c->stream));
  }
  HIPCHK(c, hipStreamSynchronize(c->stream));
  if (bad & 4u) return fail(c, 12, "internal: the hit list is not read-major");
  if (bad) return fail(c, 8, "musc_hits_copy_compact: %s", (bad & 1u) ? "a tuple field does not fit its width"
                                                                      : "a read has more than 255 tuples");
  return 0;
}

int musc_hits_unpack(musc_ctx* c, const uint64_t* src, uint64_t n, int on_device, const int32_t* bits, musc_hit* dst) {
  if (!c) return 1;
  PackBits b;
  int rc = check_pack_bits(c, bits, &b);
  if (rc) return rc;
  if (n == 0) return 0;
  if (!src || !dst) return fail(c, 2, "musc_hits_unpack: NULL pointer");
  if (!on_device) {
    for (uint64_t i = 0; i < n; i++) {
      uint64_t v = src[i];
      dst[i].nmiss = (uint32_t)(v & ((1ull << b.nmiss) - 1ull));
      v >>= b.nmiss;
      dst[i].pos = (uint32_t)(v & ((1ull << b.pos) - 1ull));
      v >>= b.pos;
      dst[i].gene_idx = (uint32_t)(v & ((1ull << b.gene) - 1ull));
      v >>= b.gene;
      dst[i].read_idx = (uint32_t)v;
    }
    return 0;
  }
  HIPCHK(c, hipSetDevice(c->device));
  hipLaunchKernelGGL(k_unpack_hits, dim3(std::min(nblk(n, 256), MAX_GRID)), dim3(256), 0, c->stream, src, n, b,
                     reinterpret_cast<uint4*>(dst));
  HIPCHK(c, hipGetLastError());
  HIPCHK(c, hipStreamSynchronize(c->stream));
  return 0;
}

int musc_match(musc_ctx* c, const musc_params* P, musc_hit** hits, uint64_t* nhits) {
  if (!c) return 1;
  if (!hits || !nhits) return fail(c, 2, "musc_match: NULL output pointer");
  *hits = nullptr;
  *nhits = 0;
  uint64_t n = 0;
  int rc = musc_match_device(c, P, &n);
  if (rc) return rc;
  musc_hit* h = (musc_hit*)malloc(sizeof(musc_hit) * (n ? n : 1));
  if (!h) return fail(c, 7, "out of host memory for %llu hits", (unsigned long long)n);
  rc = musc_hits_copy(c, h, n, 0);
  if (rc) {
    free(h);
    return rc;
  }
  *hits = h;
  *nhits = n;
  return 0;
}

void musc_free_hits(musc_hit* hits) { free(hits); }

int musc_overflow_probes(musc_ctx* c, uint32_t** read_idx, uint32_t** window, uint64_t* n) {
  if (!c) return 1;
  if (!read_idx || !window || !n) return fail(c, 2, "musc_overflow_probes: NULL output pointer");
  *read_idx = *window = nullptr;
  *n = 0;
  if (c->stats.n_overflow_blocks == 0 || c->stats.n_overflow_blocks == ~0ull) return 0;
  if (!c->last_exact_blocks || !c->block_table.p) return fail(c, 4, "no exact block counters from the last pass");
  HIPCHK(c, hipSetDevice(c->device));
  uint64_t cap = 1u << 20;
  for (;;) {
    TmpBufs B;
    uint2* d_out = nullptr;
    HIPCHK(c, B.alloc(&d_out, cap * sizeof(uint2)));
    HIPCHK(c, hipMemsetAsync(c->counters + 8, 0, 8, c->stream));
    const dim3 grid(std::min(nblk(c->nreads, 256), MAX_GRID)), block(256);
    switch (c->rw) {
      case 4: hipLaunchKernelGGL((k_hot_probes<4>), grid, block, 0, c->stream, c->rd, c->rdm, c->nreads, c->rw, c->d_pp, c->block_table.p, c->last_max_matches, d_out, cap, c->counters + 8); break;
      case 8: hipLaunchKernelGGL((k_hot_probes<8>), grid, block, 0, c->stream, c->rd, c->rdm, c->nreads, c->rw, c->d_pp, c->block_table.p, c->last_max_matches, d_out, cap, c->counters + 8); break;
      case 12: hipLaunchKernelGGL((k_hot_probes<12>), grid, block, 0, c->stream, c->rd, c->rdm, c->nreads, c->rw, c->d_pp, c->block_table.p, c->last_max_matches, d_out, cap, c->counters + 8); break;
      case 16: hipLaunchKernelGGL((k_hot_probes<16>), grid, block, 0, c->stream, c->rd, c->rdm, c->nreads, c->rw, c->d_pp, c->block_table.p, c->last_max_matches, d_out, cap, c->counters + 8); break;
      default: hipLaunchKernelGGL((k_hot_probes<0>), grid, block, 0, c->stream, c->rd, c->rdm, c->nreads, c->rw, c->d_pp, c->block_table.p, c->last_max_matches, d_out, cap, c->counters + 8); break;
    }
    hipError_t e = hipGetLastError();
    if (e == hipSuccess) e = hipMemcpyAsync(c->h_pinned, c->counters + 8, 8, hipMemcpyDeviceToHost, c->stream);
    if (e == hipSuccess) e = hipStreamSynchronize(c->stream);
    if (e != hipSuccess) return fail(c, 10, "musc_overflow_probes: %s", hipGetErrorString(e));
    const uint64_t found = c->h_pinned[0];
    if (found > cap) {
      cap = found + 16;
      continue;
    }
    std::vector<uint2> h(found ? found : 1);
    if (found) e = hipMemcpy(h.data(), d_out, found * sizeof(uint2), hipMemcpyDeviceToHost);
    if (e != hipSuccess) return fail(c, 10, "musc_overflow_probes: %s", hipGetErrorString(e));
    uint32_t* r = (uint32_t*)malloc(sizeof(uint32_t) * (found ? found : 1));
    uint32_t* w = (uint32_t*)malloc(sizeof(uint32_t) * (found ? found : 1));
    if (!r || !w) {
      free(r);
      free(w);
      return fail(c, 7, "musc_overflow_probes: out of host memory");
    }
    for (uint64_t j = 0; j < found; j++) {
      r[j] = h[j].x;
      w[j] = h[j].y;
    }
    *read_idx = r;
    *window = w;
    *n = found;
    return 0;
  }
}

void musc_free_u32(uint32_t* p) { free(p); }

int musc_get_stats(musc_ctx* c, musc_stats* out) {
  if (!c || !out) return 1;
  *out = c->stats;
  return 0;
}

int musc_last_instance(const musc_ctx* c, uint32_t* out) {
  if (!c || !out) return 1;
  for (int i = 0; i < MUSC_INSTANCE_WORDS; i++) out[i] = c->last_inst[i];
  return 0;
}

int musc_instances(uint32_t* out, uint32_t capacity, uint32_t* n) {
  if (!n) return 1;
  std::vector<uint32_t> ids;
  auto add = [&](uint32_t id) {
    if (id && std::find(ids.begin(), ids.end(), id) == ids.end()) ids.push_back(id);
  };
  static const int strides[] = {4, 8, 12, 16, 20};
  for (int rw : strides) {
    for (int kind : {MK_LANE, MK_DMA})
      for (int sg = 0; sg <= MUSC_SPEC_GEOMS; sg++)
        for (int wide = 0; wide < 2; wide++)
          for (int W = 1; W <= CTX_MAX_W; W++)
            for (int xm = 0; xm < 3; xm++) add(match_instance(kind, sg, rw, wide != 0, W, xm).id);
    add(screen_t_instance(rw).id);
    for (int mask = 0; mask < 2; mask++)
      for (int W = 2; W <= 3; W++) {
        for (int lines = 0; lines < 2; lines++) add(screen_instance(rw, mask != 0, W, lines != 0).id);
        add(confirm_instance(rw, mask != 0, W).id);
      }
  }
  *n = (uint32_t)ids.size();
  if (out)
    for (uint32_t i = 0; i < capacity && i < ids.size(); i++) out[i] = ids[i];
  return 0;
}

int musc_gather(musc_ctx* const* ctxs, int n, const uint64_t* read_base, musc_hit** hits, uint64_t* nhits) {
  if (!ctxs || n < 1 || !hits || !nhits) return 1;
  uint64_t total = 0;
  for (int i = 0; i < n; i++) {
    if (!ctxs[i]) return 1;
    total += ctxs[i]->nhits;
  }
  musc_hit* h = (musc_hit*)malloc(sizeof(musc_hit) * (total ? total : 1));
  if (!h) return fail(ctxs[0], 7, "musc_gather: out of host memory");
  uint64_t o = 0;
  for (int i = 0; i < n; i++) {
    musc_ctx* c = ctxs[i];
    int rc = musc_hits_copy(c, h + o, c->nhits, 0);
    if (rc) {
      free(h);
      return rc;
    }
    const uint64_t base = read_base ? read_base[i] : 0;
    for (uint64_t j = 0; j < c->nhits; j++) h[o + j].read_idx += (uint32_t)base;
    o += c->nhits;
  }
  *hits = h;
  *nhits = total;
  return 0;
}

namespace {
struct RcclApi {
  void* lib = nullptr;
  decltype(&ncclCommInitAll) CommInitAll = nullptr;
  decltype(&ncclCommDestroy) CommDestroy = nullptr;
  decltype(&ncclGroupStart) GroupStart = nullptr;
  decltype(&ncclGroupEnd) GroupEnd = nullptr;
  decltype(&ncclSend) Send = nullptr;
  decltype(&ncclRecv) Recv = nullptr;
  decltype(&ncclGetErrorString) GetErrorString = nullptr;
  std::string err;
  std::map<std::vector<int>, std::vector<ncclComm_t>> comms;
};
std::mutex g_rccl_mu;

RcclApi* rccl_api() {
  static RcclApi api;
  if (api.lib || !api.err.empty()) return &api;
  std::string first_err;
  std::vector<std::string> names;
  if (const char* e = getenv("MUSC_RCCL_LIB")) names.push_back(e);
  else names = {"/opt/rocm/lib/librccl.so.1", "librccl.so.1", "librccl.so"};
  for (const std::string& name : names) {
    (void)dlerror();
    api.lib = dlopen(name.c_str(), RTLD_NOW | RTLD_LOCAL);
    if (api.lib) break;
    const char* e = dlerror();
    if (first_err.empty()) first_err = e ? e : "not found";
  }
  if (!api.lib) {
    api.err = std::string("cannot load librccl: ") + first_err;
    return &api;
  }
#define MUSC_RCCL_SYM(FIELD, NAME)                                   \
  api.FIELD = reinterpret_cast<decltype(api.FIELD)>(dlsym(api.lib, NAME)); \
  if (!api.FIELD && api.err.empty()) api.err = std::string("librccl lacks ") + NAME;
  MUSC_RCCL_SYM(CommInitAll, "ncclCommInitAll")
  MUSC_RCCL_SYM(CommDestroy, "ncclCommDestroy")
  MUSC_RCCL_SYM(GroupStart, "ncclGroupStart")
  MUSC_RCCL_SYM(GroupEnd, "ncclGroupEnd")
  MUSC_RCCL_SYM(Send, "ncclSend")
  MUSC_RCCL_SYM(Recv, "ncclRecv")
  MUSC_RCCL_SYM(GetErrorString, "ncclGetErrorString")
#undef MUSC_RCCL_SYM
  return &api;
}
}

int musc_rccl_probe(char* msg, uint64_t cap) {
  std::lock_guard<std::mutex> lock(g_rccl_mu);
  RcclApi* api = rccl_api();
  if (msg && cap) {
    strncpy(msg, api->err.c_str(), cap - 1);
    msg[cap - 1] = 0;
  }
  return api->err.empty() ? 0 : 20;
}

__global__ void k_rebase_reads(uint4* __restrict__ h, uint64_t n, uint32_t base) {
  for (uint64_t i = (uint64_t)blockIdx.x * blockDim.x + threadIdx.x; i < n; i += (uint64_t)gridDim.x * blockDim.x) h[i].x += base;
}

int musc_gather_rccl(musc_ctx* const* ctxs, int n, const uint64_t* read_base, musc_hit** hits, uint64_t* nhits) {
  if (!ctxs || n < 1 || !hits || !nhits) return 1;
  *hits = nullptr;
  *nhits = 0;
  uint64_t total = 0;
  std::vector<uint64_t> off(n + 1, 0);
  std::vector<int> devs(n);
  for (int i = 0; i < n; i++) {
    if (!ctxs[i]) return 1;
    devs[i] = ctxs[i]->device;
    off[i] = total;
    total += ctxs[i]->nhits;
  }
  off[n] = total;
  musc_ctx* c0 = ctxs[0];
  for (int i = 0; i < n; i++)
    for (int j = i + 1; j < n; j++)
      if (devs[i] == devs[j]) return fail(c0, 2, "musc_gather_rccl: contexts %d and %d share device %d", i, j, devs[i]);
  std::lock_guard<std::mutex> lock(g_rccl_mu);
  std::vector<ncclComm_t>* comms = nullptr;
  RcclApi* api = nullptr;
  if (n > 1) {
    api = rccl_api();
    if (!api->err.empty()) return fail(c0, 20, "musc_gather_rccl: %s", api->err.c_str());
    auto it = api->comms.find(devs);
    if (it == api->comms.end()) {
      std::vector<ncclComm_t> cs(n);
      const ncclResult_t r = api->CommInitAll(cs.data(), n, devs.data());
      if (r != ncclSuccess) return fail(c0, 20, "musc_gather_rccl: ncclCommInitAll: %s", api->GetErrorString(r));
      it = api->comms.emplace(devs, cs).first;
    }
    comms = &it->second;
  }
  HIPCHK(c0, hipSetDevice(c0->device));
  int rc = ensure(c0, c0->gathered, total ? total : 1);
  if (rc) return rc;
  if (c0->nhits)
    HIPCHK(c0, hipMemcpyAsync(c0->gathered.p, c0->hits.p, c0->nhits * sizeof(musc_hit), hipMemcpyDeviceToDevice, c0->stream));
  if (n > 1) {
    ncclResult_t r = api->GroupStart();
    for (int i = 1; i < n && r == ncclSuccess; i++) {
      if (!ctxs[i]->nhits) continue;
      const size_t bytes = ctxs[i]->nhits * sizeof(musc_hit);
      (void)hipSetDevice(ctxs[i]->device);
      r = api->Send(ctxs[i]->hits.p, bytes, ncclUint8, 0, (*comms)[i], ctxs[i]->stream);
      if (r != ncclSuccess) break;
      (void)hipSetDevice(c0->device);
      r = api->Recv(c0->gathered.p + off[i], bytes, ncclUint8, i, (*comms)[0], c0->stream);
    }
    const ncclResult_t r2 = api->GroupEnd();
    if (r == ncclSuccess) r = r2;
    if (r != ncclSuccess) return fail(c0, 20, "musc_gather_rccl: %s", api->GetErrorString(r));
  }
  HIPCHK(c0, hipSetDevice(c0->device));
  for (int i = 0; i < n; i++) {
    const uint64_t base = read_base ? read_base[i] : 0;
    if (!base || !ctxs[i]->nhits) continue;
    hipLaunchKernelGGL(k_rebase_reads, dim3(std::min(nblk(ctxs[i]->nhits, 256), MAX_GRID)), dim3(256), 0, c0->stream,
                       reinterpret_cast<uint4*>(c0->gathered.p + off[i]), ctxs[i]->nhits, (uint32_t)base);
    HIPCHK(c0, hipGetLastError());
  }
  for (int i = 1; i < n; i++) {
    HIPCHK(ctxs[i], hipSetDevice(ctxs[i]->device));
    HIPCHK(ctxs[i], hipStreamSynchronize(ctxs[i]->stream));
  }
  HIPCHK(c0, hipSetDevice(c0->device));
  musc_hit* h = (musc_hit*)malloc(sizeof(musc_hit) * (total ? total : 1));
  if (!h) return fail(c0, 7, "musc_gather_rccl: out of host memory");
  hipError_t e = hipSuccess;
  if (total) e = hipMemcpyAsync(h, c0->gathered.p, total * sizeof(musc_hit), hipMemcpyDeviceToHost, c0->stream);
  if (e == hipSuccess) e = hipStreamSynchronize(c0->stream);
  if (e != hipSuccess) {
    free(h);
    return fail(c0, 10, "musc_gather_rccl: %s", hipGetErrorString(e));
  }
  *hits = h;
  *nhits = total;
  return 0;
}

}

#include "muscato_prep.hpp"
```

Measured before the change: 2.010 billion.

## Overlap read upload and hit download with compute via batch stream plan

Adds a stream plan that shapes read batches so the last batch is small (shrinking tail latency) and aligns upload pieces with batch boundaries, so matching on the first batch can start while later pieces are still uploading. Hit download for packed and compact formats now runs in geometrically growing chunks, packing on the compute stream and copying on the upload stream so device packing overlaps D2H transfer. The read buffer is reused across loads instead of being freed and reallocated each time. This adds event bookkeeping and a range-limited compact pack kernel, and it disables the sized/graph replay path whenever streaming is active.

```diff
diff --git a/include/muscato_hip.h b/include/muscato_hip.h
--- a/include/muscato_hip.h
+++ b/include/muscato_hip.h
@@ -113,6 +113,9 @@
 int musc_last_instance(const musc_ctx* ctx, uint32_t* out);
 int musc_instances(uint32_t* out, uint32_t capacity, uint32_t* n);
 
+int musc_stream_plan(uint64_t nreads, uint32_t fixed_len, uint32_t batch_reads, uint64_t* ends, uint8_t* is_batch_end,
+                     uint64_t capacity, uint64_t* n, uint64_t* planned_batches);
+
 int musc_overflow_probes(musc_ctx* ctx, uint32_t** read_idx, uint32_t** window, uint64_t* n);
 void musc_free_u32(uint32_t* p);
 
diff --git a/muscato_amd/_lib.py b/muscato_amd/_lib.py
--- a/muscato_amd/_lib.py
+++ b/muscato_amd/_lib.py
@@ -56,7 +56,7 @@
     "musc_db_set_partition_bases", "musc_db_partitions",
     "musc_reads_load_ascii", "musc_reads_load_packed", "musc_reads_load_packed32", "musc_reads_sort_unique",
     "musc_match_device", "musc_hits_copy", "musc_hits_copy_packed", "musc_hits_copy_compact", "musc_hits_unpack", "musc_match", "musc_free_hits",
-    "musc_get_stats", "musc_last_instance", "musc_instances", "musc_gather", "musc_gather_rccl", "musc_rccl_probe", "musc_overflow_probes", "musc_free_u32",
+    "musc_get_stats", "musc_last_instance", "musc_instances", "musc_stream_plan", "musc_gather", "musc_gather_rccl", "musc_rccl_probe", "musc_overflow_probes", "musc_free_u32",
 ]
 
 _lib = None
@@ -112,6 +112,7 @@
     lib.musc_get_stats.argtypes = [vp, ctypes.POINTER(MuscStats)]
     lib.musc_last_instance.argtypes = [vp, ctypes.POINTER(ctypes.c_uint32)]
     lib.musc_instances.argtypes = [ctypes.POINTER(ctypes.c_uint32), ctypes.c_uint32, ctypes.POINTER(ctypes.c_uint32)]
+    lib.musc_stream_plan.argtypes = [u64, ctypes.c_uint32, ctypes.c_uint32, vp, vp, u64, ctypes.POINTER(u64), ctypes.POINTER(u64)]
     lib.musc_overflow_probes.argtypes = [vp, ctypes.POINTER(vp), ctypes.POINTER(vp), ctypes.POINTER(u64)]
     lib.musc_overflow_probes.restype = ctypes.c_int
     lib.musc_free_u32.argtypes = [vp]
@@ -124,7 +125,7 @@
                  "musc_db_set_partition_bases", "musc_db_partitions",
                  "musc_reads_load_ascii", "musc_reads_load_packed", "musc_reads_load_packed32", "musc_reads_sort_unique", "musc_match_device",
                  "musc_hits_copy", "musc_hits_copy_packed", "musc_hits_copy_compact", "musc_hits_unpack", "musc_match", "musc_get_stats", "musc_last_instance", "musc_instances",
-                 "musc_gather", "musc_gather_rccl", "musc_rccl_probe"):
+                 "musc_stream_plan", "musc_gather", "musc_gather_rccl", "musc_rccl_probe"):
         getattr(lib, name).restype = ctypes.c_int
     _lib = lib
     return lib
diff --git a/muscato_amd/api.py b/muscato_amd/api.py
--- a/muscato_amd/api.py
+++ b/muscato_amd/api.py
@@ -353,6 +353,19 @@
     return [decode_instance(w) for w in buf[:n.value]]
 
 
+def stream_plan(nreads: int, fixed_len: int, batch_reads: int = 16 << 20) -> dict:
+    lib = _lib.load()
+    n, planned = ctypes.c_uint64(), ctypes.c_uint64()
+    if lib.musc_stream_plan(nreads, fixed_len, batch_reads, None, None, 0, ctypes.byref(n), ctypes.byref(planned)):
+        raise ValueError("musc_stream_plan: %d reads of %d bases is not a read set the loader takes" % (nreads, fixed_len))
+    ends = np.zeros(max(1, n.value), dtype=np.uint64)
+    flags = np.zeros(max(1, n.value), dtype=np.uint8)
+    lib.musc_stream_plan(nreads, fixed_len, batch_reads, ends.ctypes.data, flags.ctypes.data, n.value, ctypes.byref(n),
+                         ctypes.byref(planned))
+    ends, flags = ends[:n.value], flags[:n.value]
+    return {"piece_ends": ends, "batch_ends": ends[flags != 0], "planned_batches": int(planned.value)}
+
+
 def gather(engines: Sequence["Engine"], read_bases: Sequence[int], rccl: bool = False) -> np.ndarray:
     lib = engines[0]._lib
     n = len(engines)
diff --git a/muscato_amd/csrc/kernels_confirm.hpp b/muscato_amd/csrc/kernels_confirm.hpp
--- a/muscato_amd/csrc/kernels_confirm.hpp
+++ b/muscato_amd/csrc/kernels_confirm.hpp
@@ -380,3 +380,21 @@
     }
   }
 }
+
+MUSC_KERNEL __launch_bounds__(256) void k_pack_compact_range(const uint4* __restrict__ hits, uint64_t n, uint64_t t0, uint64_t t1,
+                                                            PackBits b, uint32_t* __restrict__ words, uint8_t* __restrict__ counts,
+                                                            uint32_t* __restrict__ bad) {
+  for (uint64_t i = t0 + (uint64_t)blockIdx.x * blockDim.x + threadIdx.x; i < t1; i += (uint64_t)gridDim.x * blockDim.x) {
+    const uint4 h = hits[i];
+    if (((uint64_t)h.y >> b.gene) || ((uint64_t)h.z >> b.pos) || ((uint64_t)h.w >> b.nmiss)) atomicOr(bad, 1u);
+    words[i] = (((h.y << b.pos) | h.z) << b.nmiss) | h.w;
+    const uint32_t prev = i ? hits[i - 1].x : 0xFFFFFFFFu;
+    if (i && prev > h.x) atomicOr(bad, 4u);
+    if (i == 0 || prev != h.x) {
+      uint32_t cnt = 1;
+      while (i + cnt < n && cnt < 256 && hits[i + cnt].x == h.x) cnt++;
+      if (cnt > 255) atomicOr(bad, 2u);
+      counts[h.x] = (uint8_t)cnt;
+    }
+  }
+}
diff --git a/muscato_amd/csrc/muscato_hip.hip b/muscato_amd/csrc/muscato_hip.hip
--- a/muscato_amd/csrc/muscato_hip.hip
+++ b/muscato_amd/csrc/muscato_hip.hip
@@ -122,6 +122,30 @@
   ~TmpBufs() { release(); }
 };
 
+}
+
+struct StreamPlan {
+  std::vector<uint64_t> piece_end, batch_end;
+};
+static void stream_plan(uint64_t nreads, uint64_t batch_reads, StreamPlan* sp) {
+  auto up64 = [](uint64_t x) { return (x + 63) & ~63ull; };
+  sp->piece_end.clear();
+  sp->batch_end.clear();
+  const uint64_t full = std::max<uint64_t>(up64(batch_reads), 64);
+  const uint64_t last_max = std::max<uint64_t>(up64(batch_reads / 16), 64);
+  const uint64_t piece = up64(std::max<uint64_t>(batch_reads / 4, 64));
+  for (uint64_t r0 = 0; r0 < nreads;) {
+    const uint64_t left = nreads - r0;
+    const uint64_t n = left >= 2 * full ? full : left <= last_max ? left : up64((left + 1) / 2);
+    for (uint64_t p = r0 + piece; p < r0 + n; p += piece) sp->piece_end.push_back(p);
+    r0 += n;
+    sp->piece_end.push_back(r0);
+    sp->batch_end.push_back(r0);
+  }
+}
+static uint64_t stream_plan_batch(const StreamPlan& sp, uint64_t r0) {
+  const auto it = std::upper_bound(sp.batch_end.begin(), sp.batch_end.end(), r0);
+  return it == sp.batch_end.end() ? 0 : *it - r0;
 }
 
 struct EnvKnobs {
@@ -231,6 +255,7 @@
   DevBuf<uint4> spill;
 
   uint32_t* rd = nullptr;
+  uint64_t rd_cap = 0;
   uint32_t* rdm = nullptr;
   uint64_t nreads = 0;
   int rw = 0;
@@ -241,7 +266,8 @@
     uint64_t stage_words = 0;
     hipStream_t s_up = nullptr;
     std::vector<hipEvent_t> ev;
-    uint64_t piece = 0, n_pieces = 0;
+    StreamPlan plan;
+    uint64_t next_piece = 0;
     uint64_t packed_upto = 0;
     uint32_t L = 0;
     bool active = false;
@@ -275,6 +301,7 @@
   DevBuf<musc_hit> hits;
   uint64_t nhits = 0;
   DevBuf<uint64_t> packed;
+  std::vector<hipEvent_t> dl_ev;
   DevBuf<musc_hit> gathered;
   uint32_t* d_flag = nullptr;
 
@@ -420,19 +447,24 @@
   c->data_epoch++;
 }
 
-void free_reads(musc_ctx* c) {
+void drop_reads(musc_ctx* c, bool keep_rd) {
   if (c->up.active) {
     (void)hipStreamSynchronize(c->up.s_up);
     c->up.active = false;
   }
-  if (c->rd) (void)hipFree(c->rd);
+  if (c->rd && !(keep_rd && c->rd_cap)) {
+    (void)hipFree(c->rd);
+    c->rd = nullptr;
+    c->rd_cap = 0;
+  }
   if (c->rdm) (void)hipFree(c->rdm);
-  c->rd = c->rdm = nullptr;
+  c->rdm = nullptr;
   c->reads_have_x = false;
   c->nreads = 0;
   c->rw = 0;
   c->data_epoch++;
 }
+void free_reads(musc_ctx* c) { drop_reads(c, false); }
 
 struct EvPair {
   hipEvent_t a, b;
@@ -691,6 +723,7 @@
   for (hipEvent_t ev : c->ev_pool) (void)hipEventDestroy(ev);
   if (c->graph_exec) (void)hipGraphExecDestroy(c->graph_exec);
   for (hipEvent_t ev : c->up.ev) (void)hipEventDestroy(ev);
+  for (hipEvent_t ev : c->dl_ev) (void)hipEventDestroy(ev);
   if (c->up.stage) (void)hipFree(c->up.stage);
   if (c->up.s_up) (void)hipStreamDestroy(c->up.s_up);
   if (c->stream2) (void)hipStreamDestroy(c->stream2);
@@ -1319,13 +1352,14 @@
   musc_ctx::Upload& u = c->up;
   if (!u.active) return 0;
   const uint64_t want = std::min<uint64_t>(r0 + n, c->nreads);
-  while (u.packed_upto < want) {
-    const uint64_t i = u.packed_upto / u.piece;
-    const uint64_t first = i * u.piece, cnt = std::min<uint64_t>(u.piece, c->nreads - first);
+  while (u.packed_upto < want && u.next_piece < u.plan.piece_end.size()) {
+    const uint64_t i = u.next_piece;
+    const uint64_t first = u.packed_upto, cnt = u.plan.piece_end[i] - first;
     HIPCHK(c, hipStreamWaitEvent(st, u.ev[i], 0));
     hipLaunchKernelGGL(k_pack_reads_fixed, dim3(nblk(cnt * (uint64_t)c->rw, 256)), dim3(256), 0, st, u.stage, first, cnt, u.L, c->rw, c->rd);
     HIPCHK(c, hipGetLastError());
     u.packed_upto = first + cnt;
+    u.next_piece = i + 1;
   }
   if (u.packed_upto >= c->nreads) u.active = false;
   return 0;
@@ -1414,23 +1448,26 @@
 
 static int reads_load_fixed(musc_ctx* c, const uint8_t* bases2bit, uint32_t L, uint64_t nreads, int async) {
   HIPCHK(c, hipSetDevice(c->device));
-  free_reads(c);
-  if (nreads >= 0xFFFFFFF0ull) return fail(c, 2, "too many reads for 32-bit read_idx");
-  if (L > 65535) return fail(c, 2, "read of %u bases exceeds the 65535-base record limit", L);
+  drop_reads(c, true);
+  int rw = (int)((2ull * L + 31) / 32) + 1;
+  rw = (rw + 3) & ~3;
+  if (rw < 4) rw = 4;
+  const uint64_t words = nreads * (uint64_t)rw;
+  const char* refuse = nreads >= 0xFFFFFFF0ull ? "too many reads for 32-bit read_idx"
+                       : L > 65535             ? "read length exceeds the 65535-base record limit"
+                       : words >= (1ull << 32) ? "too many read words for one dispatch (reads x record words >= 2^32)"
+                                               : nullptr;
+  if (refuse) {
+    free_reads(c);
+    return fail(c, 2, "%s", refuse);
+  }
   c->nreads = nreads;
   if (nreads == 0) {
     c->rw = 4;
     return 0;
   }
   c->max_len = L;
-  int rw = (int)((2ull * L + 31) / 32) + 1;
-  rw = (rw + 3) & ~3;
-  if (rw < 4) rw = 4;
   c->rw = rw;
-  const uint64_t words = nreads * (uint64_t)rw;
-  if (words >= (1ull << 32)) return fail(c, 2, "too many read words for one dispatch (reads x record words >= 2^32)");
-  HIPCHK(c, hipMalloc((void**)&c->rd, words * 4 + 256));
-  HIPCHK(c, hipMemsetAsync(c->rd + words, 0, 256, c->stream));
   c->reads_have_x = false;
   musc_ctx::Upload& u = c->up;
   const uint64_t total_bytes = (nreads * (uint64_t)L + 3) / 4;
@@ -1443,25 +1480,32 @@
     u.stage_words = need_words;
   }
   if (!u.s_up) HIPCHK(c, hipStreamCreateWithFlags(&u.s_up, hipStreamNonBlocking));
-  uint64_t piece = std::max<uint64_t>(c->batch_reads / 4, 64);
-  piece = (piece + 63) & ~63ull;
-  u.piece = piece;
-  u.n_pieces = (nreads + piece - 1) / piece;
+  stream_plan(nreads, c->batch_reads, &u.plan);
+  const std::vector<uint64_t>& ends = u.plan.piece_end;
   u.L = L;
   u.packed_upto = 0;
-  while (u.ev.size() < u.n_pieces) {
+  u.next_piece = 0;
+  while (u.ev.size() < ends.size()) {
     hipEvent_t e = nullptr;
     HIPCHK(c, hipEventCreateWithFlags(&e, hipEventDisableTiming));
     u.ev.push_back(e);
   }
   HIPCHK(c, hipMemsetAsync(u.stage + (need_words - 4), 0, 16, u.s_up));
-  for (uint64_t i = 0; i < u.n_pieces; i++) {
-    const uint64_t b0 = i * piece * (uint64_t)L / 4;
-    const uint64_t b1 = std::min<uint64_t>(((i + 1) * piece * (uint64_t)L + 3) / 4, total_bytes);
+  for (size_t i = 0; i < ends.size(); i++) {
+    const uint64_t b0 = (i ? ends[i - 1] : 0) * (uint64_t)L / 4;
+    const uint64_t b1 = std::min<uint64_t>((ends[i] * (uint64_t)L + 3) / 4, total_bytes);
     HIPCHK(c, hipMemcpyAsync(reinterpret_cast<uint8_t*>(u.stage) + b0, bases2bit + b0, b1 - b0, hipMemcpyHostToDevice, u.s_up));
     HIPCHK(c, hipEventRecord(u.ev[i], u.s_up));
   }
   u.active = true;
+  if (c->rd_cap < words * 4 + 256) {
+    if (c->rd) (void)hipFree(c->rd);
+    c->rd = nullptr;
+    c->rd_cap = 0;
+    HIPCHK(c, hipMalloc((void**)&c->rd, words * 4 + 256));
+    c->rd_cap = words * 4 + 256;
+  }
+  HIPCHK(c, hipMemsetAsync(c->rd + words, 0, 256, c->stream));
   if (!async) {
     int rc = upload_prepare(c, 0, nreads, c->stream);
     if (rc) return rc;
@@ -1636,6 +1680,7 @@
   const bool sized = c->sized_epoch == c->data_epoch && c->sized_exact_blocks == (block_mode == 2) &&
                      memcmp(&c->sized_params, P, sizeof *P) == 0 && !c->env.debug_sync;
   uint32_t bsz = sized ? c->sized_bsz : c->batch_reads;
+  bool streamed = c->up.active && !sized;
   const uint64_t L = c->max_len;
   const bool use_graph = sized && c->env.graph > 0 && !c->graph_failed;
   if (!sized && c->graph_exec) {
@@ -1676,7 +1721,7 @@
       if (block_mode == 2) HIPCHK(c, hipMemsetAsync(c->block_table.p, 0, (1ull << BLOCK_TABLE_BITS) * 4, c->stream));
     }
     while (!replay && r0 < c->nreads) {
-      const uint32_t n = (uint32_t)std::min<uint64_t>(bsz, c->nreads - r0);
+      const uint32_t n = (uint32_t)(streamed ? stream_plan_batch(c->up.plan, r0) : std::min<uint64_t>(bsz, c->nreads - r0));
       const uint32_t ntiles = nblk(n, WT);
       const uint64_t sgrid = std::min<uint64_t>(nblk(n, TILE), resident);
       const uint64_t swaves = sgrid * (TILE / 64);
@@ -1706,6 +1751,7 @@
         if (need_stage > (1ull << 31)) {
           if (n == 1) return fail(c, 6, "one read has %llu tuples (> 2^31)", (unsigned long long)c->h_pinned[8 + 7]);
           bsz = n / 2;
+          streamed = false;
           again = true;
           break;
         }
@@ -1813,7 +1859,7 @@
     c->stats.match_bytes = c->nreads * rec_b + n_windows * sizeof(CtxBucket) + n_ovf * ent_b + 16 * c->stats.n_hits;
     c->stats.match_bytes_strict = c->nreads * rec_b + n_windows * 8 + n_cand * ent_b + 16 * c->stats.n_hits;
     if (nhits) *nhits = c->nhits;
-    c->sized_epoch = c->data_epoch;
+    c->sized_epoch = streamed ? 0 : c->data_epoch;
     c->sized_params = *P;
     c->sized_exact_blocks = block_mode == 2;
     c->sized_bsz = bsz;
@@ -1891,7 +1937,8 @@
   }
 
   HIPCHK(c, hipMemsetAsync(c->counters, 0, 8 * sizeof(unsigned long long), c->stream));
-  const uint64_t planned_batches = (c->nreads + c->batch_reads - 1) / c->batch_reads + 1;
+  const uint64_t planned_batches = c->up.active ? std::max<uint64_t>(c->up.plan.batch_end.size(), 1)
+                                                : (c->nreads + c->batch_reads - 1) / c->batch_reads + 1;
   uint64_t max_matches = P->max_matches > 0 ? (uint64_t)P->max_matches : 0x7FFFFFFFull;
   if (P->n_shards > 1) max_matches /= (uint64_t)P->n_shards;
   const uint32_t block_thr = (uint32_t)std::min<uint64_t>(max_matches / (planned_batches * MAX_GRID), 0x7FFFFFFFull);
@@ -1943,6 +1990,7 @@
   const uint64_t PAIR_CAP = 1ull << 31;
   uint64_t r0 = 0;
   uint32_t bsz = sized ? c->sized_bsz : c->batch_reads;
+  bool streamed = c->up.active && !sized;
   if (sized) HIPCHK(c, hipMemsetAsync(c->counters + 8, 0, 8 * sizeof(unsigned long long), c->stream));
   const bool want_pipe = c->env.pipeline;
   const bool piped = sized && want_pipe && c->nreads > bsz && c->bs[1].cdesc.cap >= c->bs[0].cdesc.cap;
@@ -1955,7 +2003,7 @@
   }
   uint32_t batch_no = 0;
   while (r0 < c->nreads) {
-    const uint32_t n = (uint32_t)std::min<uint64_t>(bsz, c->nreads - r0);
+    const uint32_t n = (uint32_t)(streamed ? stream_plan_batch(c->up.plan, r0) : std::min<uint64_t>(bsz, c->nreads - r0));
     if (piped) {
       c->cur = (int)(batch_no & 1u);
       if (batch_no >= 2) HIPCHK(c, hipStreamWaitEvent(sA, c->ev_free[c->cur], 0));
@@ -1998,6 +2046,7 @@
       if (need > PAIR_CAP) {
         if (n == 1) return fail(c, 6, "one read has %llu candidate pairs (> 2^31)", (unsigned long long)total);
         bsz = n / 2;
+        streamed = false;
         HIPCHK(c, hipMemsetAsync(c->counters + 3, 0, 8, c->stream));
         continue;
       }
@@ -2104,7 +2153,7 @@
         (rc = ensure(c, c->bs[1].cdesc, c->bs[0].cdesc.cap)))
       return rc;
   }
-  c->sized_epoch = c->data_epoch;
+  c->sized_epoch = streamed ? 0 : c->data_epoch;
   c->sized_params = *P;
   c->sized_exact_blocks = block_mode == 2;
   c->sized_bsz = bsz;
@@ -2264,6 +2313,48 @@
   return 0;
 }
 
+extern "C++" {
+template <class Pack>
+static int download_chunks(musc_ctx* c, uint64_t n, size_t elem, const void* src, void* dst, Pack pack) {
+  if (!c->up.s_up) HIPCHK(c, hipStreamCreateWithFlags(&c->up.s_up, hipStreamNonBlocking));
+  const uint64_t smallest = std::min<uint64_t>(c->batch_reads, 1u << 18);
+  uint64_t sz = std::max<uint64_t>(n / 32, smallest);
+  size_t k = 0;
+  for (uint64_t t0 = 0; t0 < n; k++, sz *= 4) {
+    const uint64_t t1 = n - t0 <= sz + sz / 2 ? n : t0 + sz;
+    if (k == c->dl_ev.size()) {
+      hipEvent_t e = nullptr;
+      HIPCHK(c, hipEventCreateWithFlags(&e, hipEventDisableTiming));
+      c->dl_ev.push_back(e);
+    }
+    pack(t0, t1);
+    HIPCHK(c, hipGetLastError());
+    HIPCHK(c, hipEventRecord(c->dl_ev[k], c->stream));
+    HIPCHK(c, hipStreamWaitEvent(c->up.s_up, c->dl_ev[k], 0));
+    HIPCHK(c, hipMemcpyAsync((char*)dst + t0 * elem, (const char*)src + t0 * elem, (t1 - t0) * elem, hipMemcpyDeviceToHost, c->up.s_up));
+    t0 = t1;
+  }
+  return 0;
+}
+}
+
+static int download_end(musc_ctx* c, uint32_t* h_bad, void* tail_dst, const void* tail_src, uint64_t tail_bytes) {
+  hipError_t e = hipMemcpyAsync(h_bad, c->d_flag, 4, hipMemcpyDeviceToHost, c->stream);
+  if (e == hipSuccess && tail_bytes) {
+    hipStream_t st = c->up.s_up ? c->up.s_up : c->stream;
+    if (st != c->stream && (e = hipEventRecord(c->ev_join, c->stream)) == hipSuccess) e = hipStreamWaitEvent(st, c->ev_join, 0);
+    if (e == hipSuccess) e = hipMemcpyAsync(tail_dst, tail_src, tail_bytes, hipMemcpyDeviceToHost, st);
+  }
+  const hipError_t e1 = hipStreamSynchronize(c->stream);
+  const hipError_t e2 = c->up.s_up ? hipStreamSynchronize(c->up.s_up) : hipSuccess;
+  if (e == hipSuccess) e = e1 != hipSuccess ? e1 : e2;
+  if (e != hipSuccess) {
+    (void)hipGetLastError();
+    return fail(c, 10, "copying the tuples to the host failed: %s", hipGetErrorString(e));
+  }
+  return 0;
+}
+
 static int check_pack_bits(musc_ctx* c, const int32_t* bits, PackBits* b) {
   if (!bits) return fail(c, 2, "bits is NULL");
   int sum = 0;
@@ -2293,14 +2384,23 @@
     out = c->packed.p;
   }
   HIPCHK(c, hipMemsetAsync(c->d_flag, 0, 4, c->stream));
-  hipLaunchKernelGGL(k_pack_hits, dim3(std::min(nblk(c->nhits, 256), MAX_GRID)), dim3(256), 0, c->stream,
-                     reinterpret_cast<const uint4*>(c->hits.p), c->nhits, read_base, b, out, c->d_flag);
-  HIPCHK(c, hipGetLastError());
-  uint32_t bad = 0;
-  HIPCHK(c, hipMemcpyAsync(&bad, c->d_flag, 4, hipMemcpyDeviceToHost, c->stream));
-  if (!dst_on_device)
-    HIPCHK(c, hipMemcpyAsync(dst, out, c->nhits * 8, hipMemcpyDeviceToHost, c->stream));
-  HIPCHK(c, hipStreamSynchronize(c->stream));
+  const uint4* const hits = reinterpret_cast<const uint4*>(c->hits.p);
+  auto pack = [&](uint64_t t0, uint64_t t1) {
+    hipLaunchKernelGGL(k_pack_hits, dim3(std::min(nblk(t1 - t0, 256), MAX_GRID)), dim3(256), 0, c->stream, hits + t0, t1 - t0,
+                       read_base, b, out + t0, c->d_flag);
+  };
+  uint32_t* const h_bad = reinterpret_cast<uint32_t*>(c->h_pinned);
+  if (dst_on_device) {
+    pack(0, c->nhits);
+    HIPCHK(c, hipGetLastError());
+    HIPCHK(c, hipMemcpyAsync(h_bad, c->d_flag, 4, hipMemcpyDeviceToHost, c->stream));
+    HIPCHK(c, hipStreamSynchronize(c->stream));
+  } else {
+    rc = download_chunks(c, c->nhits, 8, out, dst, pack);
+    const int rc_end = download_end(c, h_bad, nullptr, nullptr, 0);
+    if (rc || rc_end) return rc ? rc : rc_end;
+  }
+  const uint32_t bad = *h_bad;
   if (bad) return fail(c, 8, "musc_hits_copy_packed: a tuple field does not fit its width (%d/%d/%d/%d bits)",
                        b.read, b.gene, b.pos, b.nmiss);
   return 0;
@@ -2333,18 +2433,25 @@
   }
   HIPCHK(c, hipMemsetAsync(c->d_flag, 0, 4, c->stream));
   if (c->nreads) HIPCHK(c, hipMemsetAsync(dc, 0, c->nreads, c->stream));
-  if (c->nhits) {
-    hipLaunchKernelGGL(k_pack_compact, dim3(std::min(nblk(c->nhits, 256), MAX_GRID)), dim3(256), 0, c->stream,
-                       reinterpret_cast<const uint4*>(c->hits.p), c->nhits, b, dw, dc, c->d_flag);
-    HIPCHK(c, hipGetLastError());
-  }
-  uint32_t bad = 0;
-  HIPCHK(c, hipMemcpyAsync(&bad, c->d_flag, 4, hipMemcpyDeviceToHost, c->stream));
-  if (!dst_on_device) {
-    if (c->nhits) HIPCHK(c, hipMemcpyAsync(words, dw, c->nhits * 4, hipMemcpyDeviceToHost, c->stream));
-    if (c->nreads) HIPCHK(c, hipMemcpyAsync(counts, dc, c->nreads, hipMemcpyDeviceToHost, c->stream));
-  }
-  HIPCHK(c, hipStreamSynchronize(c->stream));
+  const uint4* const hits = reinterpret_cast<const uint4*>(c->hits.p);
+  uint32_t* const h_bad = reinterpret_cast<uint32_t*>(c->h_pinned);
+  if (dst_on_device) {
+    if (c->nhits) {
+      hipLaunchKernelGGL(k_pack_compact, dim3(std::min(nblk(c->nhits, 256), MAX_GRID)), dim3(256), 0, c->stream, hits, c->nhits,
+                         b, dw, dc, c->d_flag);
+      HIPCHK(c, hipGetLastError());
+    }
+    HIPCHK(c, hipMemcpyAsync(h_bad, c->d_flag, 4, hipMemcpyDeviceToHost, c->stream));
+    HIPCHK(c, hipStreamSynchronize(c->stream));
+  } else {
+    int rc = download_chunks(c, c->nhits, 4, dw, words, [&](uint64_t t0, uint64_t t1) {
+      hipLaunchKernelGGL(k_pack_compact_range, dim3(std::min(nblk(t1 - t0, 256), MAX_GRID)), dim3(256), 0, c->stream, hits,
+                         c->nhits, t0, t1, b, dw, dc, c->d_flag);
+    });
+    const int rc_end = download_end(c, h_bad, counts, dc, c->nreads);
+    if (rc || rc_end) return rc ? rc : rc_end;
+  }
+  const uint32_t bad = *h_bad;
   if (bad & 4u) return fail(c, 12, "internal: the hit list is not read-major");
   if (bad) return fail(c, 8, "musc_hits_copy_compact: %s", (bad & 1u) ? "a tuple field does not fit its width"
                                                                       : "a read has more than 255 tuples");
@@ -2493,6 +2600,23 @@
   return 0;
 }
 
+int musc_stream_plan(uint64_t nreads, uint32_t fixed_len, uint32_t batch_reads, uint64_t* ends, uint8_t* is_batch_end,
+                     uint64_t capacity, uint64_t* n, uint64_t* planned_batches) {
+  if (!n || fixed_len > 65535 || nreads >= 0xFFFFFFF0ull) return 1;
+  if (batch_reads < 1 || batch_reads > (16u << 20)) batch_reads = 16u << 20;
+  StreamPlan sp;
+  stream_plan(nreads, batch_reads, &sp);
+  *n = sp.piece_end.size();
+  if (planned_batches) *planned_batches = std::max<uint64_t>(sp.batch_end.size(), 1);
+  size_t b = 0;
+  for (size_t i = 0; i < sp.piece_end.size() && i < capacity; i++) {
+    if (ends) ends[i] = sp.piece_end[i];
+    while (b < sp.batch_end.size() && sp.batch_end[b] < sp.piece_end[i]) b++;
+    if (is_batch_end) is_batch_end[i] = b < sp.batch_end.size() && sp.batch_end[b] == sp.piece_end[i];
+  }
+  return 0;
+}
+
 int musc_gather(musc_ctx* const* ctxs, int n, const uint64_t* read_base, musc_hit** hits, uint64_t* nhits) {
   if (!ctxs || n < 1 || !hits || !nhits) return 1;
   uint64_t total = 0;
```

New measurement: 2.104 billion (median of 6 runs). +4.7%, better.
